# crmorton/Turbo-Whisper-Workspace

Hardware: AMD Instinct MI355X
Metric: real-time factor (audio-sec/wall-sec) Whisper-v3-turbo, 30s chunks, 1/2/4/8 GPU (higher is better)
Workload: dtype bf16; 1 GPU; whisper-large-v3-turbo bf16, batch=24 x 30s windows per GPU, greedy, 128 new tokens/window (EOS suppressed, one seek pass), timestamps on, language detected; collectives=none, global_batch=24, seq_len=3000, parallelism=chunk-dp1

## Files before the change

include/tw_whisper.h:

```cpp
#ifndef TW_WHISPER_H
#define TW_WHISPER_H
#include <stdint.h>

#ifdef __cplusplus
extern "C" {
#endif

#define TW_ABI_VERSION 1

#define TW_EPI_BF16 0
#define TW_EPI_GELU_BF16 1
#define TW_EPI_RESID_F32 2
#define TW_EPI_GELU_POS_F32 3
#define TW_EPI_F32 4
#define TW_EPI_CROSSKV 5
#define TW_EPI_GELU_PACKED 6
#define TW_EPI_GELU_MX 7
#define TW_EPI_GELU_F32 8
#define TW_EPI_PARTIAL_F32 100

#define TW_STATE_STRIDE 8
#define TW_ST_NGEN 0
#define TW_ST_LAST 1
#define TW_ST_PENULT 2
#define TW_ST_LASTTS 3
#define TW_ST_FINISHED 4
#define TW_ST_LANG 5
#define TW_ST_SUMLP 6
#define TW_ST_NOSPEECH 7

#define TW_SELECT_CHUNKS 16
#define TW_SELECT_WS_PER_ROW 128

typedef struct TwSelectParams {
  int32_t V;
  int32_t eos;
  int32_t pad;
  int32_t ts_begin;
  int32_t no_timestamps;
  int32_t max_initial_ts;
  int32_t use_timestamps;
  int32_t max_new;
  int32_t mode;
  int32_t lo, hi;
  int32_t n_begin_suppress;
  int32_t begin_suppress[8];
} TwSelectParams;

int tw_version(void);
const char* tw_last_error(void);

int tw_fill_synth(void* out, long n, uint64_t seed, uint32_t tensor_id, float scale, float offset, int as_f32,
                  void* stream);
int tw_f32_to_bf16(const float* in, uint16_t* out, long n, float scale, void* stream);

int tw_logmel(const float* wave, int n_chunks, const float* basis_cos, const float* basis_sin, const float* mel_fb,
              int n_mels, float* feats, uint32_t* maxkeys, void* stream);

int tw_logmel_long(const float* wave, long n_samples, const float* basis_cos, const float* basis_sin,
                   const float* mel_fb, int n_mels, float* feats, long feats_ld, uint32_t* maxkey, void* stream);

int tw_im2col_conv1(const float* feats, int n_mels, const int* row_map, const int* seek, int R, int kpad,
                    uint16_t* out, void* stream);
int tw_im2col_conv1_long(const float* feats, int n_mels, long ld, const int* max_frames, const int* row_map,
                         const int* seek, int R, int kpad, uint16_t* out, void* stream);
int tw_im2col_conv2(const uint16_t* h1, int R, int D, uint16_t* out, void* stream);
int tw_conv2_gemm(const uint16_t* h1, int R, int D, const uint16_t* W, const float* bias, const float* pos, float* out,
                  void* stream);

int tw_gemm_bf16(const uint16_t* A, const uint16_t* W, int M, int N, int K, int lda, int ldw, int epi, void* out,
                 int ldo, const float* bias, const float* aux, int aux_rows, const int* kv_geom, void* stream);
int tw_gemm_set_variant(int v);
int tw_gemm_bf16_partial(const uint16_t* A, const uint16_t* W, int M, int N, int K, int lda, int ldw, int splits,
                         float* part, int ldp, void* stream);
int tw_resid_layernorm(float* x, const float* parts, int nparts, const float* bias, const float* gamma,
                       const float* beta, int M, int D, float eps, uint16_t* out, void* stream);
int tw_layernorm(const float* x, const float* gamma, const float* beta, int M, int D, float eps, uint16_t* out,
                 void* stream);
int tw_layernorm_set_lds_pad(int kib);

int tw_gemm_mx(const uint8_t* A, const uint8_t* Sa, const uint8_t* W, const uint8_t* Sw, int M, int N, int K, int lda,
               int ldw, int Mp, int Np, int epi, void* out, int ldo, const float* bias, uint8_t* sout, int sout_rows,
               void* stream);
int tw_gemm_mx_set_variant(int v);
int tw_quant_mx(const uint16_t* src, int rows, int K, int ld, uint8_t* dst, uint8_t* scales, int rows_pad,
                void* stream);
int tw_layernorm_mx(const float* x, const float* gamma, const float* beta, int M, int D, float eps, uint8_t* out,
                    uint8_t* scales, int rows_pad, void* stream);

int tw_attn_encoder(const uint16_t* qkv, int B, int S, int H, uint16_t* out, void* stream);
int tw_attn_encoder_mx(const uint16_t* qkv, int B, int S, int H, uint8_t* out, uint8_t* scales, int rows_pad,
                       void* stream);
int tw_attn_set_variant(int variant);
int tw_attn_set_lds_pad(int units);

typedef struct TwBeamParams {
  int32_t num_beams;
  int32_t max_new;
  float length_penalty;
  int32_t ld_tokens;
  int32_t scores_are_logprobs;
} TwBeamParams;
typedef struct TwBeamState {
  float* run_score;
  float* fin_score;
  int32_t* fin_flag;
  int32_t* fin_len;
  int32_t* fin_tokens;
  int32_t* win;
  int32_t* src_rows;
  int32_t* kv_tab;
  int32_t* fin_tab;
  float* run_lp;
  float* fin_lp;
} TwBeamState;
size_t tw_beam_workspace_bytes(int rows);
int tw_beam_step(const float* logits, int W, int ld_logits, const uint32_t* suppress_bits,
                 const TwSelectParams* params, const TwBeamParams* beam, const TwBeamState* bstate, int* state,
                 int* tokens, int* ids, int* pos, void* workspace, void* stream);
int tw_kv_reorder(uint16_t* k_cache, uint16_t* v_cache, uint16_t* k_scratch, uint16_t* v_scratch, int layers,
                  int rows_cap, int H, int T, int R, const int* src_rows, const int* pos, void* stream);

int tw_pack_weight(const uint16_t* W, int N, int K, int ldw, uint16_t* Wp, void* stream);
int tw_gemv_packed(const uint16_t* A, int a_packed, int lda, const uint16_t* Wp, int M, int N, int K, int epi,
                   void* out, int ldo, const float* bias, int splits, void* stream);
int tw_gemv_set_wide_slices(int kw);
int tw_gemv_set_variant(int v);
int tw_gemm_set_epilogue(int tr);
int tw_gemm_set_persistent_grid(int n);
typedef struct TwDecLayerW {
  const uint16_t *wqkv, *wo, *wq_x, *wo_x, *w1, *w2;
  const float *bqkv, *bo, *bq_x, *bo_x, *b1, *b2;
  const float *ln1_g, *ln1_b, *ln2_g, *ln2_b, *ln3_g, *ln3_b;
} TwDecLayerW;
size_t tw_dec_fused_sync_bytes(void);
int tw_dec_fused_supported(int d_model, int heads, int ffn, int rows);
int tw_dec_fused_set_grid(int n);
int tw_dec_fused_set_acquire(int on);
int tw_dec_fused_set_probe(void* buf);
int tw_dec_fused_grid(void);
int tw_dec_fused(const TwDecLayerW* layers, int n_layers, int R, const int* pos, float* x, uint16_t* kc,
                 uint16_t* vc, long kv_layer_stride, int max_pos, const uint16_t* xkv, long xkv_layer_stride,
                 long xkv_v_off, int S, uint16_t* qb, uint16_t* ab, uint16_t* fb, float* slab, float* xpart,
                 const float* lnf_g, const float* lnf_b, uint16_t* hp, float eps, unsigned* sync, unsigned* err,
                 void* stream);
size_t tw_dec_fused_xpart_bytes(int rows);
int tw_resid_layernorm_packed(float* x, const float* parts, int nparts, const float* bias, const float* gamma,
                              const float* beta, int M, int D, float eps, uint16_t* out, void* stream);
int tw_resid_layernorm_packed_to(const float* x, float* x_out, const float* parts, int nparts, const float* bias,
                                 const float* gamma, const float* beta, int M, int D, float eps, uint16_t* out,
                                 void* stream);

int tw_attn_decode_self(const uint16_t* qkv, int B, int H, int max_pos, const int* pos, uint16_t* k_cache,
                        uint16_t* v_cache, uint16_t* out, void* stream);
int tw_attn_decode_self_tab(const uint16_t* qkv, int B, int H, int max_pos, const int* pos, uint16_t* k_cache,
                            uint16_t* v_cache, const int* kv_tab, int row0, uint16_t* out, void* stream);
int tw_attn_decode_self_masked(const uint16_t* qkv, int B, int H, int max_pos, const int* pos, uint16_t* k_cache,
                               uint16_t* v_cache, const int* kv_start, uint16_t* out, void* stream);
int tw_attn_decode_self_tab_masked(const uint16_t* qkv, int B, int H, int max_pos, const int* pos, uint16_t* k_cache,
                                   uint16_t* v_cache, const int* kv_tab, int row0, const int* kv_start, uint16_t* out,
                                   void* stream);
int tw_kv_tab_check(const int* kv_tab, const int* pos, int row0, int B, int max_pos, int* bad, void* stream);
int tw_debug_build(void);
int tw_attn_decode_cross(const uint16_t* q, int B, int H, int S, int Bt, const int* row_map, const uint16_t* cross_kv,
                         uint16_t* out, void* stream);
size_t tw_attn_decode_cross_grouped_ws_bytes(int B, int H);
int tw_attn_decode_cross_grouped(const uint16_t* q, int B, int H, int S, int Bt, const int* row_map, int group,
                                 int first, const uint16_t* cross_kv, float* ws, uint16_t* out, void* stream);
int tw_attn_decode_cross_probs(const uint16_t* q, int B, int H, int S, int Bt, const int* row_map,
                               const uint16_t* cross_kv, uint16_t* out, float* probs, uint32_t head_mask, int slot0,
                               int n_slots, const int* pos, int pos0, int n_steps, void* stream);
int tw_dtw(const double* matrix, int n, int m, int* text_idx, int* time_idx, int* path_len);

int tw_gemm_f32(const float* A, const float* W, int M, int N, int K, int lda, int ldw, int epi, float* out, int ldo,
                const float* bias, const float* aux, int aux_rows, const int* kv_geom, void* stream);
int tw_layernorm_f32(const float* x, const float* gamma, const float* beta, int M, int D, float eps, float* out,
                     void* stream);
int tw_im2col_conv1_f32(const float* feats, int n_mels, long ld, const int* max_frames, const int* row_map,
                        const int* seek, int R, int kpad, float* out, void* stream);
int tw_im2col_conv2_f32(const float* h1, int R, int D, float* out, void* stream);
int tw_embed_decoder_f32(const float* tok_emb, const float* pos_emb, const int* ids, const int* pos, int B, int D,
                         float* x, void* stream);
int tw_attn_encoder_f32(const float* qkv, int B, int S, int H, float* out, void* stream);
int tw_attn_decode_self_f32(const float* qkv, int B, int H, int max_pos, const int* pos, float* k_cache,
                            float* v_cache, const int* kv_tab, int row0, const int* kv_start, float* out,
                            void* stream);
int tw_attn_decode_cross_f32(const float* q, int B, int H, int S, int Bt, const int* row_map, const float* cross_kv,
                             float* out, float* probs, unsigned head_mask, int slot0, int n_slots, const int* pos,
                             int pos0, int n_steps, void* stream);

int tw_embed_decoder(const uint16_t* tok_emb, const uint16_t* pos_emb, const int* ids, const int* pos, int B, int D,
                     float* x, void* stream);
int tw_logits_select(const float* logits, int B, int ld_logits, const uint32_t* suppress_bits,
                     const TwSelectParams* params, int* state, int* tokens_out, int ld_tokens, int* next_ids,
                     int* pos, float* workspace, void* stream);
int tw_logits_select_embed(const float* logits, int B, int ld_logits, const uint32_t* suppress_bits,
                           const TwSelectParams* params, int* state, int* tokens_out, int ld_tokens, int* next_ids,
                           int* pos, float* workspace, const uint16_t* tok_emb, const uint16_t* pos_emb, int D,
                           int max_pos, float* x, const float* gamma, const float* beta, float eps, uint16_t* out,
                           int packed, void* stream);

int tw_logits_sample(const float* logits, int B, int ld_logits, const uint32_t* suppress_bits,
                     const TwSelectParams* params, float temperature, int top_k, uint64_t seed, const int* row_key,
                     int* state, int* tokens_out, int ld_tokens, int* next_ids, int* pos, void* stream);
int tw_token_prob(const float* logits, int B, int ld_logits, int V, int token, int* state, void* stream);

#define TW_HIST_MAX 448
#define TW_HIST_LANG (-1)
int tw_logits_history(float* logits, int R, int ld_logits, int V, const int* prefix, int ld_prefix,
                      const int* prefix_len, const int* tokens, int ld_tokens, const int* state,
                      float repetition_penalty, int no_repeat_ngram, int to_logprobs, void* stream);

#ifdef __cplusplus
}
#endif
#endif
```

turbo-whisper-workspace_amd/csrc/decode.hip:

```cpp
#include "tw_common.h"
#include "../../include/tw_whisper.h"

struct Best {
  float v;
  int i;
};
__device__ inline Best best_of(Best a, Best b) {
  if (b.v > a.v || (b.v == a.v && b.i < a.i)) return b;
  return a;
}
__device__ inline void lse_merge(float& m, float& s, float m2, float s2) {
  if (m2 == -INFINITY) return;
  if (m == -INFINITY) { m = m2; s = s2; return; }
  if (m2 > m) { s = s * __expf(m - m2) + s2; m = m2; }
  else s = s + s2 * __expf(m2 - m);
}

__device__ inline void lse_add1(float& m, float& s, float x) {
  const float d = x - m;
  const float e = (x == -INFINITY) ? 0.f : __expf(-fabsf(d));
  s = (d > 0.f) ? s * e + 1.f : s + e;
  m = fmaxf(m, x);
}

struct SelPart {
  float bt_v; int bt_i;
  float bs_v; int bs_i;
  float m_ts, s_ts;
  float pad0, pad1;
};

struct RowMask {
  int init_step, mask_ts_all, mask_text_lt_eos, ts_hi_block;
};
__device__ inline RowMask row_mask(const int* st, const TwSelectParams& p) {
  const int n_gen = st[TW_ST_NGEN], last = st[TW_ST_LAST], penult = st[TW_ST_PENULT], last_ts = st[TW_ST_LASTTS];
  const int tsb = p.ts_begin;
  RowMask r{n_gen == 0, 0, 0, tsb};
  if (p.mode == 0 && p.use_timestamps) {
    const bool last_was_ts = n_gen >= 1 && last >= tsb;
    const bool penult_was_ts = n_gen < 2 || penult >= tsb;
    if (last_was_ts) {
      if (penult_was_ts) r.mask_ts_all = 1;
      else r.mask_text_lt_eos = 1;
    }
    if (last_ts >= 0) r.ts_hi_block = (last_was_ts && !penult_was_ts) ? last_ts : last_ts + 1;
  }
  return r;
}

template <bool TX>
__device__ inline void sel_chunk(const float* __restrict__ row, const uint32_t* __restrict__ suppress_bits,
                                 const TwSelectParams& p, const RowMask& rm, int v0, int v1, SelPart* sp,
                                 SelPart& out, float& m_tx, float& s_tx) {
  const int tid = threadIdx.x, lane = tid & 63, wid = tid >> 6;
  const int tsb = p.ts_begin;
  Best bt{-INFINITY, 0x7fffffff}, bs{-INFINITY, 0x7fffffff};
  float m_ts = -INFINITY, s_ts = 0.f;
  for (int base = v0 + tid; base < v1; base += 4 * 256) {
    float xs[4];
    uint32_t sb[4];
#pragma unroll
    for (int u = 0; u < 4; ++u) {
      const int v = min(base + 256 * u, v1 - 1);
      xs[u] = row[v];
      sb[u] = suppress_bits ? suppress_bits[v >> 5] : 0u;
    }
#pragma unroll
    for (int u = 0; u < 4; ++u) {
      const int v = base + 256 * u;
      const bool ok = v < v1;
      float x = xs[u];
      bool masked;
      if (p.mode == 1) {
        masked = (v < p.lo || v >= p.hi);
      } else {
        masked = (sb[u] >> (v & 31)) & 1u;
        if (rm.init_step)
          for (int i = 0; i < p.n_begin_suppress; ++i) masked |= (v == p.begin_suppress[i]);
        if (p.use_timestamps) {
          masked |= (v == p.no_timestamps);
          if (v >= tsb) {
            masked |= rm.mask_ts_all || (v < rm.ts_hi_block);
            if (rm.init_step && p.max_initial_ts >= 0) masked |= (v > tsb + p.max_initial_ts);
          } else {
            masked |= (rm.mask_text_lt_eos && v < p.eos) || rm.init_step;
          }
        }
      }
      if (masked) x = -INFINITY;
      if (!ok) continue;
      if (v < tsb || !p.use_timestamps || p.mode == 1) {
        bt = best_of(bt, Best{x, v});
        if (TX && x != -INFINITY) lse_merge(m_tx, s_tx, x, 1.f);
      } else {
        bs = best_of(bs, Best{x, v});
        if (x != -INFINITY) lse_merge(m_ts, s_ts, x, 1.f);
      }
    }
  }
#pragma unroll
  for (int o = 32; o > 0; o >>= 1) {
    Best ot{__shfl_xor(bt.v, o, 64), __shfl_xor(bt.i, o, 64)};
    Best os{__shfl_xor(bs.v, o, 64), __shfl_xor(bs.i, o, 64)};
    bt = best_of(bt, ot);
    bs = best_of(bs, os);
    float m2 = __shfl_xor(m_ts, o, 64), s2 = __shfl_xor(s_ts, o, 64);
    lse_merge(m_ts, s_ts, m2, s2);
  }
  if (lane == 0) sp[wid] = SelPart{bt.v, bt.i, bs.v, bs.i, m_ts, s_ts, 0.f, 0.f};
  __syncthreads();
  if (tid == 0) {
    for (int w = 1; w < 4; ++w) {
      bt = best_of(bt, Best{sp[w].bt_v, sp[w].bt_i});
      bs = best_of(bs, Best{sp[w].bs_v, sp[w].bs_i});
      lse_merge(m_ts, s_ts, sp[w].m_ts, sp[w].s_ts);
    }
    out = SelPart{bt.v, bt.i, bs.v, bs.i, m_ts, s_ts, 0.f, 0.f};
  }
}

__global__ TW_DEC_LB(256, 1) void k_select_partial(const float* __restrict__ logits, int ld_logits,
                                                        const uint32_t* __restrict__ suppress_bits, TwSelectParams p,
                                                        const int* __restrict__ state, SelPart* __restrict__ ws) {
  TW_DEC_PRIO();
  __shared__ SelPart sp[4];
  const int b = blockIdx.x, c = blockIdx.y, NC = gridDim.y;
  const RowMask rm = row_mask(state + b * TW_STATE_STRIDE, p);
  const int V = p.V;
  const int v0 = (int)((long)c * V / NC), v1 = (int)((long)(c + 1) * V / NC);
  SelPart out;
  float m_tx = -INFINITY, s_tx = 0.f;
  sel_chunk<false>(logits + (size_t)b * ld_logits, suppress_bits, p, rm, v0, v1, sp, out, m_tx, s_tx);
  if (threadIdx.x == 0) ws[b * NC + c] = out;
}

__device__ inline void sel_merge(const SelPart* __restrict__ ws, int NC, int b, int lane, Best& bt, Best& bs,
                                 float& m_ts, float& s_ts) {
  bt = Best{-INFINITY, 0x7fffffff};
  bs = Best{-INFINITY, 0x7fffffff};
  m_ts = -INFINITY;
  s_ts = 0.f;
  for (int c = lane; c < NC; c += 64) {
    const SelPart r = ws[b * NC + c];
    bt = best_of(bt, Best{r.bt_v, r.bt_i});
    bs = best_of(bs, Best{r.bs_v, r.bs_i});
    lse_merge(m_ts, s_ts, r.m_ts, r.s_ts);
  }
#pragma unroll
  for (int o = 32; o > 0; o >>= 1) {
    Best ot{__shfl_xor(bt.v, o, 64), __shfl_xor(bt.i, o, 64)};
    Best os{__shfl_xor(bs.v, o, 64), __shfl_xor(bs.i, o, 64)};
    bt = best_of(bt, ot);
    bs = best_of(bs, os);
    float m2 = __shfl_xor(m_ts, o, 64), s2 = __shfl_xor(s_ts, o, 64);
    lse_merge(m_ts, s_ts, m2, s2);
  }
}
__device__ inline bool sel_rule_fires(const TwSelectParams& p, Best bt, float m_ts, float s_ts) {
  if (!p.use_timestamps) return false;
  const float lse_ts = (m_ts == -INFINITY) ? -INFINITY : m_ts + __logf(s_ts);
  return lse_ts > bt.v;
}
__device__ inline int sel_greedy(const TwSelectParams& p, Best bt, Best bs, float m_ts, float s_ts) {
  if (!p.use_timestamps) return bt.i;
  return sel_rule_fires(p, bt, m_ts, s_ts) ? bs.i : best_of(bt, bs).i;
}
__device__ inline int sel_commit(const TwSelectParams& p, int* __restrict__ st, int sel, int* __restrict__ tokens_out,
                                 int ld_tokens, int* __restrict__ next_ids, int b) {
  const int n_gen = st[TW_ST_NGEN], last = st[TW_ST_LAST];
  const int finished = st[TW_ST_FINISHED];
  const int tok = finished ? p.pad : sel;
  if (tokens_out) tokens_out[(size_t)b * ld_tokens + n_gen] = tok;
  if (next_ids) next_ids[b] = tok;
  st[TW_ST_PENULT] = last;
  st[TW_ST_LAST] = tok;
  if (tok >= p.ts_begin && p.use_timestamps) st[TW_ST_LASTTS] = tok;
  st[TW_ST_NGEN] = n_gen + 1;
  if (!finished && (tok == p.eos || n_gen + 1 >= p.max_new)) st[TW_ST_FINISHED] = 1;
  return tok;
}

__device__ inline void select_final_row(const SelPart* __restrict__ ws, int NC, const TwSelectParams& p,
                                        int* __restrict__ state, int* __restrict__ tokens_out, int ld_tokens,
                                        int* __restrict__ next_ids, int* __restrict__ pos, int b, int lane,
                                        int& tok_out, int& npos) {
  Best bt, bs;
  float m_ts, s_ts;
  sel_merge(ws, NC, b, lane, bt, bs, m_ts, s_ts);
  if (lane != 0) return;
  int* st = state + b * TW_STATE_STRIDE;
  npos = 0;
  if (pos) npos = pos[b] += 1;
  if (p.mode == 1) {
    const int sel = bt.i;
    st[TW_ST_LANG] = sel;
    if (next_ids) next_ids[b] = sel;
    tok_out = sel;
    return;
  }
  tok_out = sel_commit(p, st, sel_greedy(p, bt, bs, m_ts, s_ts), tokens_out, ld_tokens, next_ids, b);
}

__global__ __launch_bounds__(64) void k_select_final(const SelPart* __restrict__ ws, int NC, TwSelectParams p,
                                                     int* __restrict__ state, int* __restrict__ tokens_out,
                                                     int ld_tokens, int* __restrict__ next_ids,
                                                     int* __restrict__ pos) {
  TW_DEC_PRIO();
  int tok, npos;
  select_final_row(ws, NC, p, state, tokens_out, ld_tokens, next_ids, pos, blockIdx.x, threadIdx.x, tok, npos);
}

#define SFE_MAXV 4
template <bool PACKED>
__global__ TW_DEC_LB(256, 1) void k_select_final_embed(const SelPart* __restrict__ ws, int NC, TwSelectParams p,
                                                            int* __restrict__ state, int* __restrict__ tokens_out,
                                                            int ld_tokens, int* __restrict__ next_ids,
                                                            int* __restrict__ pos, const bf16_t* __restrict__ tok_emb,
                                                            const bf16_t* __restrict__ pos_emb, int D, int max_pos,
                                                            float* __restrict__ x, const float* __restrict__ g,
                                                            const float* __restrict__ bta, float eps,
                                                            bf16_t* __restrict__ out) {
  TW_DEC_PRIO();
  __shared__ float red[8];
  __shared__ int sh[2];
  const int b = blockIdx.x, tid = threadIdx.x;
  if (tid < 64) {
    int tok = 0, npos = 0;
    select_final_row(ws, NC, p, state, tokens_out, ld_tokens, next_ids, pos, b, tid, tok, npos);
    if (tid == 0) {
      sh[0] = tok;
      sh[1] = min(npos, max_pos - 1);
    }
  }
  __syncthreads();
  const bf16_t* te = tok_emb + (size_t)sh[0] * D;
  const bf16_t* pe = pos_emb + (size_t)sh[1] * D;
  float* xr = x + (size_t)b * D;
  const int nc = D >> 2;
  float4 v[SFE_MAXV];
  float s = 0.f;
#pragma unroll
  for (int i = 0; i < SFE_MAXV; ++i) {
    const int c = min(tid + 256 * i, nc - 1);
    const uint2 t = ((const uint2*)te)[c], q = ((const uint2*)pe)[c];
    float4 a;
    a.x = bf16_to_f32((bf16_t)(t.x & 0xffff)) + bf16_to_f32((bf16_t)(q.x & 0xffff));
    a.y = bf16_to_f32((bf16_t)(t.x >> 16)) + bf16_to_f32((bf16_t)(q.x >> 16));
    a.z = bf16_to_f32((bf16_t)(t.y & 0xffff)) + bf16_to_f32((bf16_t)(q.y & 0xffff));
    a.w = bf16_to_f32((bf16_t)(t.y >> 16)) + bf16_to_f32((bf16_t)(q.y >> 16));
    v[i] = a;
    if (tid + 256 * i < nc) {
      ((float4*)xr)[tid + 256 * i] = a;
      s += (a.x + a.y) + (a.z + a.w);
    }
  }
  tw_row_ln_store<PACKED>(v, s, b, D, eps, g, bta, out, red);
}

extern "C" int tw_logits_select(const float* logits, int B, int ld_logits, const uint32_t* suppress_bits,
                                const TwSelectParams* params, int* state, int* tokens_out, int ld_tokens,
                                int* next_ids, int* pos, float* workspace, void* stream) {
  TW_REQUIRE(logits && params && state && workspace && B > 0, "tw_logits_select: bad args");
  TW_REQUIRE(params->V > 0 && params->V <= ld_logits, "tw_logits_select: V=%d ld=%d", params->V, ld_logits);
  TW_REQUIRE(params->n_begin_suppress >= 0 && params->n_begin_suppress <= 8, "tw_logits_select: begin_suppress");
  static_assert(sizeof(SelPart) * TW_SELECT_CHUNKS == sizeof(float) * TW_SELECT_WS_PER_ROW, "workspace size");
  hipStream_t s = (hipStream_t)stream;
  SelPart* ws = (SelPart*)workspace;
  hipLaunchKernelGGL(k_select_partial, dim3(B, TW_SELECT_CHUNKS), dim3(256), 0, s, logits, ld_logits, suppress_bits,
                     *params, state, ws);
  hipLaunchKernelGGL(k_select_final, dim3(B), dim3(64), 0, s, ws, TW_SELECT_CHUNKS, *params, state, tokens_out,
                     ld_tokens, next_ids, pos);
  return tw_check_launch("tw_logits_select");
}

extern "C" int tw_logits_select_embed(const float* logits, int B, int ld_logits, const uint32_t* suppress_bits,
                                      const TwSelectParams* params, int* state, int* tokens_out, int ld_tokens,
                                      int* next_ids, int* pos, float* workspace, const uint16_t* tok_emb,
                                      const uint16_t* pos_emb, int D, int max_pos, float* x, const float* gamma,
                                      const float* beta, float eps, uint16_t* out, int packed, void* stream) {
  TW_REQUIRE(logits && params && state && workspace && next_ids && pos && B > 0, "tw_logits_select_embed: bad args");
  TW_REQUIRE(params->mode == 0, "tw_logits_select_embed: greedy token selection (mode 0) only");
  TW_REQUIRE(params->V > 0 && params->V <= ld_logits, "tw_logits_select_embed: V=%d ld=%d", params->V, ld_logits);
  TW_REQUIRE(params->n_begin_suppress >= 0 && params->n_begin_suppress <= 8, "tw_logits_select_embed: begin_suppress");
  TW_REQUIRE(tok_emb && pos_emb && x && gamma && beta && out && max_pos > 0, "tw_logits_select_embed: embed/LN args");
  TW_REQUIRE(D > 0 && D % 4 == 0 && D <= 1024 * SFE_MAXV && (!packed || (B <= 64 && D % 32 == 0)),
             "tw_logits_select_embed: D=%d B=%d packed=%d", D, B, packed);
  hipStream_t s = (hipStream_t)stream;
  SelPart* ws = (SelPart*)workspace;
  hipLaunchKernelGGL(k_select_partial, dim3(B, TW_SELECT_CHUNKS), dim3(256), 0, s, logits, ld_logits, suppress_bits,
                     *params, state, ws);
  if (packed)
    hipLaunchKernelGGL(k_select_final_embed<true>, dim3(B), dim3(256), 0, s, ws, TW_SELECT_CHUNKS, *params, state,
                       tokens_out, ld_tokens, next_ids, pos, tok_emb, pos_emb, D, max_pos, x, gamma, beta, eps, out);
  else
    hipLaunchKernelGGL(k_select_final_embed<false>, dim3(B), dim3(256), 0, s, ws, TW_SELECT_CHUNKS, *params, state,
                       tokens_out, ld_tokens, next_ids, pos, tok_emb, pos_emb, D, max_pos, x, gamma, beta, eps, out);
  return tw_check_launch("tw_logits_select_embed");
}

__device__ inline uint64_t tw_mix64(uint64_t z) {
  z += 0x9e3779b97f4a7c15ull;
  z = (z ^ (z >> 30)) * 0xbf58476d1ce4e5b9ull;
  z = (z ^ (z >> 27)) * 0x94d049bb133111ebull;
  return z ^ (z >> 31);
}
__device__ inline float tw_gumbel(uint64_t seed, uint32_t key, uint32_t step, uint32_t v) {
  const uint64_t h = tw_mix64(seed ^ tw_mix64(((uint64_t)key << 32) ^ ((uint64_t)step << 20) ^ (uint64_t)v));
  const float u = ((float)(h >> 40) + 0.5f) * (1.0f / 16777216.0f);
  return -logf(-logf(u));
}
__device__ inline float sel_processed(const float* __restrict__ row, const uint32_t* __restrict__ suppress_bits,
                                      const TwSelectParams& p, const RowMask& rm, int v) {
  const int tsb = p.ts_begin;
  bool masked = suppress_bits ? (suppress_bits[v >> 5] >> (v & 31)) & 1u : false;
  if (rm.init_step)
    for (int i = 0; i < p.n_begin_suppress; ++i) masked |= (v == p.begin_suppress[i]);
  if (p.use_timestamps) {
    masked |= (v == p.no_timestamps);
    if (v >= tsb) {
      masked |= rm.mask_ts_all || (v < rm.ts_hi_block);
      if (rm.init_step && p.max_initial_ts >= 0) masked |= (v > tsb + p.max_initial_ts);
    } else {
      masked |= (rm.mask_text_lt_eos && v < p.eos) || rm.init_step;
    }
  }
  return masked ? -INFINITY : row[v];
}
__device__ inline float block_sum256(float v, float* red) {
  v = wave_sum(v);
  __syncthreads();
  if ((threadIdx.x & 63) == 0) red[threadIdx.x >> 6] = v;
  __syncthreads();
  return (red[0] + red[1]) + (red[2] + red[3]);
}
__device__ inline void block_lse256(float& m, float& s, float* red) {
#pragma unroll
  for (int o = 32; o > 0; o >>= 1) lse_merge(m, s, __shfl_xor(m, o, 64), __shfl_xor(s, o, 64));
  __syncthreads();
  if ((threadIdx.x & 63) == 0) {
    red[2 * (threadIdx.x >> 6)] = m;
    red[2 * (threadIdx.x >> 6) + 1] = s;
  }
  __syncthreads();
  m = red[0];
  s = red[1];
  for (int w = 1; w < 4; ++w) lse_merge(m, s, red[2 * w], red[2 * w + 1]);
}

__global__ __launch_bounds__(256) void k_select_full(const float* __restrict__ logits, int ld_logits,
                                                     const uint32_t* __restrict__ suppress_bits, TwSelectParams p,
                                                     float temperature, int top_k, uint64_t seed,
                                                     const int* __restrict__ row_key, int* __restrict__ state,
                                                     int* __restrict__ tokens_out, int ld_tokens,
                                                     int* __restrict__ next_ids, int* __restrict__ pos) {
  __shared__ SelPart sp[4];
  __shared__ SelPart parts[TW_SELECT_CHUNKS];
  __shared__ float red[8];
  __shared__ uint32_t hist[256];
  __shared__ int bcast[4];
  const int b = blockIdx.x, tid = threadIdx.x, lane = tid & 63;
  int* st = state + b * TW_STATE_STRIDE;
  const RowMask rm = row_mask(st, p);
  const float* row = logits + (size_t)b * ld_logits;
  const int V = p.V, NC = TW_SELECT_CHUNKS, tsb = p.ts_begin;
  float m_tx = -INFINITY, s_tx = 0.f;
  for (int c = 0; c < NC; ++c) {
    SelPart out;
    sel_chunk<true>(row, suppress_bits, p, rm, (int)((long)c * V / NC), (int)((long)(c + 1) * V / NC), sp, out, m_tx,
                    s_tx);
    if (tid == 0) parts[c] = out;
    __syncthreads();
  }
  block_lse256(m_tx, s_tx, red);
  Best bt, bs;
  float m_ts, s_ts;
  sel_merge(parts, NC, 0, lane, bt, bs, m_ts, s_ts);
  const bool fire = sel_rule_fires(p, bt, m_ts, s_ts);
  int sel;
  float lse;
  if (temperature <= 0.f) {
    sel = sel_greedy(p, bt, bs, m_ts, s_ts);
    float m = fire ? -INFINITY : m_tx, sm = fire ? 0.f : s_tx;
    if (p.use_timestamps) lse_merge(m, sm, m_ts, s_ts);
    lse = m + __logf(sm);
  } else {
    const float invT = 1.f / temperature;
    auto elig = [&](int v, float x) { return x != -INFINITY && !(fire && v < tsb); };
    uint32_t prefix = 0u, mask = 0u;
    int n_el = 0;
    for (int v = tid; v < V; v += 256) n_el += elig(v, sel_processed(row, suppress_bits, p, rm, v)) ? 1 : 0;
    n_el = (int)block_sum256((float)n_el, red);
    const bool restrict_k = top_k > 0 && n_el > top_k;
    if (restrict_k) {
      int k_rem = top_k;
      for (int shift = 24; shift >= 0; shift -= 8) {
        hist[tid] = 0u;
        __syncthreads();
        for (int v = tid; v < V; v += 256) {
          const float x = sel_processed(row, suppress_bits, p, rm, v);
          if (!elig(v, x)) continue;
          const uint32_t key = f32_order_key(x);
          if ((key & mask) == prefix) atomicAdd(&hist[(key >> shift) & 255u], 1u);
        }
        __syncthreads();
        if (tid == 0) {
          int cum = 0, d = 255;
          for (; d > 0; --d) {
            if (cum + (int)hist[d] >= k_rem) break;
            cum += (int)hist[d];
          }
          bcast[0] = d;
          bcast[1] = k_rem - cum;
        }
        __syncthreads();
        prefix |= (uint32_t)bcast[0] << shift;
        mask |= 255u << shift;
        k_rem = bcast[1];
        __syncthreads();
      }
    }
    const uint32_t rkey = row_key ? (uint32_t)row_key[b] : (uint32_t)b;
    const uint32_t step = (uint32_t)st[TW_ST_NGEN];
    Best g{-INFINITY, 0x7fffffff};
    float m = -INFINITY, sm = 0.f;
    for (int v = tid; v < V; v += 256) {
      const float x = sel_processed(row, suppress_bits, p, rm, v);
      if (!elig(v, x) || (restrict_k && f32_order_key(x) < prefix)) continue;
      lse_merge(m, sm, x, 1.f);
      g = best_of(g, Best{x * invT + tw_gumbel(seed, rkey, step, (uint32_t)v), v});
    }
#pragma unroll
    for (int o = 32; o > 0; o >>= 1) g = best_of(g, Best{__shfl_xor(g.v, o, 64), __shfl_xor(g.i, o, 64)});
    __syncthreads();
    if (lane == 0) {
      red[tid >> 6] = g.v;
      bcast[tid >> 6] = g.i;
    }
    __syncthreads();
    g = Best{red[0], bcast[0]};
    for (int w = 1; w < 4; ++w) g = best_of(g, Best{red[w], bcast[w]});
    sel = g.i;
    block_lse256(m, sm, red);
    lse = m + __logf(sm);
  }
  if (tid != 0) return;
  if (pos) pos[b] += 1;
  const int was_finished = st[TW_ST_FINISHED];
  const int tok = sel_commit(p, st, sel, tokens_out, ld_tokens, next_ids, b);
  if (!was_finished) {
    const float lp = row[tok] - lse;
    st[TW_ST_SUMLP] = __float_as_int(__int_as_float(st[TW_ST_SUMLP]) + lp);
  }
}

__global__ __launch_bounds__(256) void k_token_prob(const float* __restrict__ logits, int ld_logits, int V, int token,
                                                    int* __restrict__ state) {
  __shared__ float red[8];
  const float* row = logits + (size_t)blockIdx.x * ld_logits;
  float m = -INFINITY, s = 0.f;
  for (int v = threadIdx.x; v < V; v += 256) lse_merge(m, s, row[v], 1.f);
  block_lse256(m, s, red);
  if (threadIdx.x == 0)
    state[blockIdx.x * TW_STATE_STRIDE + TW_ST_NOSPEECH] = __float_as_int(__expf(row[token] - (m + __logf(s))));
}

extern "C" int tw_logits_sample(const float* logits, int B, int ld_logits, const uint32_t* suppress_bits,
                                const TwSelectParams* params, float temperature, int top_k, uint64_t seed,
                                const int* row_key, int* state, int* tokens_out, int ld_tokens, int* next_ids,
                                int* pos, void* stream) {
  TW_REQUIRE(logits && params && state && B > 0, "tw_logits_sample: bad args");
  TW_REQUIRE(params->mode == 0, "tw_logits_sample: generation steps (mode 0) only");
  TW_REQUIRE(params->V > 0 && params->V <= ld_logits, "tw_logits_sample: V=%d ld=%d", params->V, ld_logits);
  TW_REQUIRE(params->n_begin_suppress >= 0 && params->n_begin_suppress <= 8, "tw_logits_sample: begin_suppress");
  TW_REQUIRE(temperature >= 0.f && temperature == temperature, "tw_logits_sample: temperature %f", temperature);
  hipLaunchKernelGGL(k_select_full, dim3(B), dim3(256), 0, (hipStream_t)stream, logits, ld_logits, suppress_bits,
                     *params, temperature, top_k, seed, row_key, state, tokens_out, ld_tokens, next_ids, pos);
  return tw_check_launch("tw_logits_sample");
}

extern "C" int tw_token_prob(const float* logits, int B, int ld_logits, int V, int token, int* state, void* stream) {
  TW_REQUIRE(logits && state && B > 0 && V > 0 && V <= ld_logits && token >= 0 && token < V,
             "tw_token_prob: B=%d V=%d token=%d", B, V, token);
  hipLaunchKernelGGL(k_token_prob, dim3(B), dim3(256), 0, (hipStream_t)stream, logits, ld_logits, V, token, state);
  return tw_check_launch("tw_token_prob");
}

#define TW_HIST_THREADS 1024
#define TW_HIST_INFLIGHT 8
__global__ __launch_bounds__(TW_HIST_THREADS) void k_logits_history(float* __restrict__ logits, int ld_logits, int V,
                                                                    const int* __restrict__ prefix, int ld_prefix,
                                                                    const int* __restrict__ prefix_len,
                                                                    const int* __restrict__ tokens, int ld_tokens,
                                                                    const int* __restrict__ state, float penalty,
                                                                    int ngram, int to_logprobs) {
  TW_DEC_PRIO();
  __shared__ int h[TW_HIST_MAX];
  __shared__ float red[2 * (TW_HIST_THREADS / 64)];
  const int r = blockIdx.x, tid = threadIdx.x;
  const int* st = state + r * TW_STATE_STRIDE;
  if (st[TW_ST_FINISHED]) return;
  float* row = logits + (size_t)r * ld_logits;
  const int pl = prefix ? min(max(prefix_len[r], 0), ld_prefix) : 0;
  const int ng = min(max(st[TW_ST_NGEN], 0), ld_tokens);
  const int L = min(pl + ng, TW_HIST_MAX);
  for (int i = tid; i < L; i += TW_HIST_THREADS) {
    int id = i < pl ? prefix[(size_t)r * ld_prefix + i] : tokens[(size_t)r * ld_tokens + (i - pl)];
    if (id == TW_HIST_LANG) id = st[TW_ST_LANG];
    h[i] = id;
  }
  if (to_logprobs) {
    float m = -INFINITY, s = 0.f;
    for (int base = tid; base < V; base += TW_HIST_INFLIGHT * TW_HIST_THREADS) {
      float xs[TW_HIST_INFLIGHT];
#pragma unroll
      for (int u = 0; u < TW_HIST_INFLIGHT; ++u) {
        const int v = base + u * TW_HIST_THREADS;
        xs[u] = v < V ? row[v] : -INFINITY;
      }
#pragma unroll
      for (int u = 0; u < TW_HIST_INFLIGHT; ++u) {
        const float x = xs[u], d = x - m;
        const float e = (x == -INFINITY) ? 0.f : expf(-fabsf(d));
        s = (d > 0.f) ? s * e + 1.f : s + e;
        m = fmaxf(m, x);
      }
    }
    auto merge = [](float& m, float& s, float m2, float s2) {
      if (m2 == -INFINITY) return;
      if (m == -INFINITY) { m = m2; s = s2; return; }
// ... 657 lines not shown
```

turbo-whisper-workspace_amd/csrc/gemm.hip:

```cpp
#include <algorithm>
#include <type_traits>

#include "tw_common.h"
#include "../../include/tw_whisper.h"

struct EpiArgs {
  void* out;
  int ldo;
  const float* bias;
  const float* aux;
  int aux_rows;
  int kv_S, kv_B, kv_D, kv_H;
  uint8_t* sout;
  int s_rows;
  int group_m;
};

__device__ inline void tw_tile_grouped(int wgid, int ntm, int ntn, int gm, int& tm, int& tn) {
  if (gm <= 1) {
    tm = wgid / ntn;
    tn = wgid - tm * ntn;
    return;
  }
  const int per = gm * ntn, g = wgid / per, first = g * gm;
  const int rows = min(ntm - first, gm), l = wgid - g * per;
  tm = first + l % rows;
  tn = l / rows;
}

template <int EPI>
__device__ inline void epi_store(const EpiArgs& ea, int m, int n, float v) {
  if (ea.bias) v += ea.bias[n];
  if constexpr (EPI == TW_EPI_BF16) {
    ((bf16_t*)ea.out)[(size_t)m * ea.ldo + n] = f32_to_bf16(v);
  } else if constexpr (EPI == TW_EPI_GELU_BF16) {
    ((bf16_t*)ea.out)[(size_t)m * ea.ldo + n] = f32_to_bf16(gelu_erf(v));
  } else if constexpr (EPI == TW_EPI_RESID_F32) {
    float* o = (float*)ea.out + (size_t)m * ea.ldo + n;
    *o = *o + v;
  } else if constexpr (EPI == TW_EPI_GELU_POS_F32) {
    ((float*)ea.out)[(size_t)m * ea.ldo + n] = gelu_erf(v) + ea.aux[(size_t)(m % ea.aux_rows) * ea.ldo + n];
  } else if constexpr (EPI == TW_EPI_F32) {
    ((float*)ea.out)[(size_t)m * ea.ldo + n] = v;
  } else if constexpr (EPI == TW_EPI_CROSSKV) {
    const int D = ea.kv_D, S = ea.kv_S;
    int l = n / (2 * D), rem = n - l * 2 * D;
    int kv = rem / D, hd = rem - kv * D;
    int h = hd >> 6, d = hd & 63;
    int b = m / S, s = m - b * S;
    size_t idx = ((((size_t)(l * 2 + kv) * ea.kv_B + b) * ea.kv_H + h) * S + s) * 64 + d;
    ((bf16_t*)ea.out)[idx] = f32_to_bf16(v);
  }
}

static int tw_gemm_kernel = 1;
static int tw_gemm_tr = 0;
extern "C" int tw_gemm_set_epilogue(int tr) {
  TW_REQUIRE(tr == 0 || tr == 1, "tw_gemm_set_epilogue: %d (0 or 1)", tr);
  tw_gemm_tr = tr;
  return 0;
}
static inline int tw_group_for(int N) { return (N + 255) / 256 >= 10 ? 8 : 1; }
static constexpr int tw_gemv_nt_min_n = 16384;
static int tw_gemv_wide_kw = 1;
extern "C" int tw_gemv_set_wide_slices(int kw) {
  TW_REQUIRE(kw == 1 || kw == 2 || kw == 4, "tw_gemv_set_wide_slices: kw=%d (1, 2 or 4)", kw);
  tw_gemv_wide_kw = kw;
  return 0;
}
static constexpr int tw_gemv_max_kw = 4;
static int tw_gemv_kernel = 0;
extern "C" int tw_gemv_set_variant(int v) {
  TW_REQUIRE(v == 0 || v == 1, "tw_gemv_set_variant: v=%d (0 or 1)", v);
  tw_gemv_kernel = v;
  return 0;
}
extern "C" int tw_gemm_set_variant(int v) {
  tw_gemm_kernel = (v & 15) == 5 ? 5 : (v & 15) == 6 ? 6 : 1;
  return 0;
}
static int tw_pgrid_override = 0;
extern "C" int tw_gemm_set_persistent_grid(int n) {
  TW_REQUIRE(n == 0 || (n >= 8 && n % 8 == 0), "tw_gemm_set_persistent_grid: %d (0 = all CUs, else a multiple of 8)", n);
  tw_pgrid_override = n;
  return 0;
}
static int tw_persistent_grid() {
  static int g = 0;
  if (tw_pgrid_override) return tw_pgrid_override;
  if (!g) {
    int dev = 0, cus = 0;
    if (hipGetDevice(&dev) != hipSuccess ||
        hipDeviceGetAttribute(&cus, hipDeviceAttributeMultiprocessorCount, dev) != hipSuccess || cus < 8)
      cus = 256;
    g = cus / 8 * 8;
  }
  return g;
}

#define GB_BM 256
#define GB_BN 256
#define GB_BK 64
#define GB_EPI_LD 68

typedef __attribute__((address_space(3))) void lds_void_t;

__device__ inline int gb_swz(int r) { return (r >> 1) & 7; }

constexpr int gb_nt_bit(int epi) {
  return epi == TW_EPI_BF16 ? TW_NT_GEMM_BF16 : epi == TW_EPI_GELU_BF16 ? TW_NT_GEMM_GELU
         : epi == TW_EPI_RESID_F32 ? TW_NT_GEMM_RESID : TW_NT_GEMM_OTHER;
}

template <int EPI>
__device__ inline void epi_store4(const EpiArgs& ea, int m, int n, int N, float4 v) {
  if (n + 3 >= N) {
    const float t[4] = {v.x, v.y, v.z, v.w};
    EpiArgs e2 = ea;
    e2.bias = nullptr;
    for (int q = 0; q < 4; ++q)
      if (n + q < N) epi_store<EPI>(e2, m, n + q, t[q]);
    return;
  }
  if constexpr (EPI == TW_EPI_BF16 || EPI == TW_EPI_GELU_BF16) {
    if constexpr (EPI == TW_EPI_GELU_BF16) v = gelu_erf4(v);
    uint2 w;
    w.x = pack_bf16x2(v.x, v.y);
    w.y = pack_bf16x2(v.z, v.w);
    tw_st_enc<gb_nt_bit(EPI)>((bf16_t*)ea.out + (size_t)m * ea.ldo + n, w);
  } else if constexpr (EPI == TW_EPI_RESID_F32) {
    float4* o = (float4*)((float*)ea.out + (size_t)m * ea.ldo + n);
    float4 x = *o;
    x.x += v.x; x.y += v.y; x.z += v.z; x.w += v.w;
    tw_st_enc<gb_nt_bit(EPI)>(o, x);
  } else if constexpr (EPI == TW_EPI_GELU_POS_F32) {
    const float4 a = *(const float4*)(ea.aux + (size_t)(m % ea.aux_rows) * ea.ldo + n);
    float4 o = gelu_erf4(v);
    o.x += a.x; o.y += a.y; o.z += a.z; o.w += a.w;
    tw_st_enc<gb_nt_bit(EPI)>((float*)ea.out + (size_t)m * ea.ldo + n, o);
  } else if constexpr (EPI == TW_EPI_F32) {
    tw_st_enc<gb_nt_bit(EPI)>((float*)ea.out + (size_t)m * ea.ldo + n, v);
  } else if constexpr (EPI == TW_EPI_CROSSKV) {
    const int D = ea.kv_D, S = ea.kv_S;
    int l = n / (2 * D), rem = n - l * 2 * D;
    int kv = rem / D, hd = rem - kv * D;
    int h = hd >> 6, d = hd & 63;
    int b = m / S, s = m - b * S;
    size_t idx = ((((size_t)(l * 2 + kv) * ea.kv_B + b) * ea.kv_H + h) * S + s) * 64 + d;
    uint2 w;
    w.x = pack_bf16x2(v.x, v.y);
    w.y = pack_bf16x2(v.z, v.w);
    tw_st_enc<gb_nt_bit(EPI)>((bf16_t*)ea.out + idx, w);
  }
}

template <int EPI>
__device__ inline float4 epi_addend(const EpiArgs& ea, int m, int n, bool full) {
// ... 857 lines not shown
    for (int a = 0; a < 2; ++a)
#pragma unroll
      for (int b = 0; b < 2; ++b)
#pragma unroll
        for (int i = 0; i < 4; ++i)
#pragma unroll
          for (int j = 0; j < 2; ++j) acc[a][b][i][j] = (f32x4){0.f, 0.f, 0.f, 0.f};
    if (nk == 1) {
      ktile(0, BF{}, BT{});
    } else {
      ktile(0, BT{}, BT{});
      for (int t = 1; t + 1 < nk; ++t) ktile(t, BT{}, BF{});
      ktile(nk - 1, BF{}, BF{});
    }
    if (wr == 0) __builtin_amdgcn_s_barrier();
    __syncthreads();
    const int nlocal = local + S;
    const bool has_next = nlocal < cnt;
    const int cm0 = m0, cn0 = n0;
    if (has_next) {
      set_tile(base + nlocal, m0, n0);
#pragma unroll
      for (int h = 0; h < 4; ++h) stage(0, h, 0);
      stage_bias((it + 1) & 1, n0);
    }
    epilogue(cm0, cn0, bias_sl + 256 * (it & 1));
    if (!has_next) break;
    if (BF16OUT && cm0 + GB_BM <= M && cn0 + GB_BN <= N)
      asm volatile("s_waitcnt vmcnt(16)" ::: "memory");
    else if (PRE && cm0 + GB_BM <= M && cn0 + GB_BN <= N)
      asm volatile("s_waitcnt vmcnt(8)" ::: "memory");
    else
      asm volatile("s_waitcnt vmcnt(0)" ::: "memory");
    __builtin_amdgcn_s_barrier();
    if (wr == 1) __builtin_amdgcn_s_barrier();
    local = nlocal;
  }
}

#define TW_EPI_PARTIAL 100

template <int EPI, int NW, bool TWO>
__global__ __launch_bounds__(NW * 64) void k_gemm_skinny(const bf16_t* __restrict__ A, const bf16_t* __restrict__ W,
                                                         int M, int N, int K, int lda, int ldw, EpiArgs ea) {
  TW_DEC_PRIO();
  __shared__ float red[NW][32][17];
  const int tid = threadIdx.x, lane = tid & 63, wid = tid >> 6;
  const int n0 = blockIdx.x * 16;
  const int nsl = NW * gridDim.y, gw = blockIdx.y * NW + wid;
  const int ns = K >> 5;
  const int s0 = (int)((long)gw * ns / nsl), s1 = (int)((long)(gw + 1) * ns / nsl);
  const int col = min(n0 + (lane & 15), N - 1);
  const int ksub = 8 * (lane >> 4);
  const int ar0 = min(lane & 15, M - 1), ar1 = min(16 + (lane & 15), M - 1);
  const bf16_t* wp = W + (size_t)col * ldw + ksub;
  const bf16_t* ap0 = A + (size_t)ar0 * lda + ksub;
  const bf16_t* ap1 = A + (size_t)ar1 * lda + ksub;
  f32x4 c0 = {0}, c1 = {0};
  int s = s0;
  for (; s + 8 <= s1; s += 8) {
    bf16x8 bw[8], a0[8], a1[8];
#pragma unroll
    for (int u = 0; u < 8; ++u) {
      bw[u] = *(const bf16x8*)(wp + 32 * (s + u));
      a0[u] = *(const bf16x8*)(ap0 + 32 * (s + u));
      if (TWO) a1[u] = *(const bf16x8*)(ap1 + 32 * (s + u));
    }
#pragma unroll
    for (int u = 0; u < 8; ++u) {
      c0 = __builtin_amdgcn_mfma_f32_16x16x32_bf16(a0[u], bw[u], c0, 0, 0, 0);
      if (TWO) c1 = __builtin_amdgcn_mfma_f32_16x16x32_bf16(a1[u], bw[u], c1, 0, 0, 0);
    }
  }
  for (; s < s1; ++s) {
    bf16x8 bw = *(const bf16x8*)(wp + 32 * s);
    bf16x8 a0 = *(const bf16x8*)(ap0 + 32 * s);
    c0 = __builtin_amdgcn_mfma_f32_16x16x32_bf16(a0, bw, c0, 0, 0, 0);
    if (TWO) {
      bf16x8 a1 = *(const bf16x8*)(ap1 + 32 * s);
      c1 = __builtin_amdgcn_mfma_f32_16x16x32_bf16(a1, bw, c1, 0, 0, 0);
    }
  }
  const int cc = lane & 15, rb = (lane >> 4) * 4;
#pragma unroll
  for (int r = 0; r < 4; ++r) {
    red[wid][rb + r][cc] = c0[r];
    if (TWO) red[wid][16 + rb + r][cc] = c1[r];
  }
  __syncthreads();
  const int rows = TWO ? 32 : 16;
  for (int e = tid; e < rows * 16; e += NW * 64) {
    int m = e >> 4, c = e & 15;
    int n = n0 + c;
    if (m < M && n < N) {
      float v = 0.f;
#pragma unroll
      for (int w = 0; w < NW; ++w) v += red[w][m][c];
      if constexpr (EPI == TW_EPI_PARTIAL) {
        ((float*)ea.out)[((size_t)blockIdx.y * M + m) * ea.ldo + n] = v;
      } else {
        epi_store<EPI>(ea, m, n, v);
      }
    }
  }
}

template <int EPI, int NW>
static void launch_skinny_nw(const bf16_t* A, const bf16_t* W, int M, int N, int K, int lda, int ldw,
                             const EpiArgs& ea, int splits, hipStream_t s) {
  dim3 grid(tw_cdiv(N, 16), splits);
  if (M > 16)
    hipLaunchKernelGGL((k_gemm_skinny<EPI, NW, true>), grid, dim3(NW * 64), 0, s, A, W, M, N, K, lda, ldw, ea);
  else
    hipLaunchKernelGGL((k_gemm_skinny<EPI, NW, false>), grid, dim3(NW * 64), 0, s, A, W, M, N, K, lda, ldw, ea);
}

template <int EPI>
static void launch_skinny(const bf16_t* A, const bf16_t* W, int M, int N, int K, int lda, int ldw,
                          const EpiArgs& ea, int splits, hipStream_t s) {
  const long nb = tw_cdiv(N, 16) * (long)splits;
  const int ns = K / 32;
  int nw = 4;
  while (nb * nw < 1024 && nw < 8 && ns >= 2 * 2 * nw * splits) nw *= 2;
  if (nw == 4) launch_skinny_nw<EPI, 4>(A, W, M, N, K, lda, ldw, ea, splits, s);
  else if (nw == 8) launch_skinny_nw<EPI, 8>(A, W, M, N, K, lda, ldw, ea, splits, s);
  else launch_skinny_nw<EPI, 16>(A, W, M, N, K, lda, ldw, ea, splits, s);
}

__global__ __launch_bounds__(256) void k_pack_weight(const bf16_t* __restrict__ W, int N, int K, int ldw,
                                                     bf16_t* __restrict__ Wp, long nchunks) {
  const long c = (long)blockIdx.x * 256 + threadIdx.x;
  if (c >= nchunks) return;
  const int lane = (int)(c & 63);
  const long rest = c >> 6;
  const int ns = K >> 5;
  const int st = (int)(rest % ns), g = (int)(rest / ns);
  const int n = g * 16 + (lane & 15), k = st * 32 + 8 * (lane >> 4);
  uint4 v = make_uint4(0u, 0u, 0u, 0u);
  if (n < N) v = *(const uint4*)(W + (size_t)n * ldw + k);
  *(uint4*)(Wp + c * 8) = v;
}


template <int MT, bool APACK>
__device__ inline const bf16_t* gemv_a_base(const bf16_t* A, int lda, int M, int K, int t, int lane) {
  if constexpr (APACK) return A + (size_t)(t >> 1) * 32 * K + (t & 1) * 512 + lane * 8;
  else return A + (size_t)min(16 * t + (lane & 15), M - 1) * lda + 8 * (lane >> 4);
}
template <bool APACK>
__device__ inline bf16x8 gemv_a_load(const bf16_t* ap, int st) {
  return APACK ? *(const bf16x8*)(ap + (size_t)st * 1024) : *(const bf16x8*)(ap + 32 * st);
}

template <int EPI, int KW, int U, bool APACK, int MT, bool NTW = false>
__global__ TW_DEC_LB(KW > 4 ? 512 : 256, NTW ? 4 : 1) void k_gemv_p(const bf16_t* __restrict__ A, int lda,
                                                               const bf16_t* __restrict__ Wp, int M, int N, int K,
                                                               EpiArgs ea) {
  TW_DEC_PRIO();
  constexpr int NW = KW > 4 ? KW : 4, GPB = NW / KW;
  __shared__ float red[KW > 1 ? NW : 1][KW > 1 ? MT * 16 : 1][17];
  const int tid = threadIdx.x, lane = tid & 63, wid = tid >> 6;
  const int gl = wid / KW, kw = wid - gl * KW;
  const int g = blockIdx.x * GPB + gl;
  const int ngroups = (N + 15) >> 4, ns = K >> 5;
  const int nsl = KW * gridDim.y, sl = blockIdx.y * KW + kw;
  const int s0 = (int)((long)sl * ns / nsl), s1 = (int)((long)(sl + 1) * ns / nsl);
  f32x4 c[MT];
#pragma unroll
  for (int t = 0; t < MT; ++t) c[t] = (f32x4){0.f, 0.f, 0.f, 0.f};
  if (g < ngroups) {
    const bf16_t* wp = Wp + (size_t)g * ns * 512 + lane * 8;
    const bf16_t* ap[MT];
#pragma unroll
    for (int t = 0; t < MT; ++t) ap[t] = gemv_a_base<MT, APACK>(A, lda, M, K, t, lane);
    auto ldW = [&](int st) -> bf16x8 {
      if constexpr (NTW) {
        typedef short s16x8_nt __attribute__((ext_vector_type(8)));
        const s16x8_nt v = __builtin_nontemporal_load((const s16x8_nt*)(wp + (size_t)st * 512));
        return __builtin_bit_cast(bf16x8, v);
      } else {
        return *(const bf16x8*)(wp + (size_t)st * 512);
      }
    };
    auto batch = [&](auto NBc, int st0, int n) {
      constexpr int NB = decltype(NBc)::value;
      bf16x8 bw[NB], a[NB][MT];
#pragma unroll
      for (int u = 0; u < NB; ++u) {
        const int st = min(st0 + u, s1 - 1);
        bw[u] = ldW(st);
#pragma unroll
        for (int t = 0; t < MT; ++t) a[u][t] = gemv_a_load<APACK>(ap[t], st);
      }
      if constexpr (!NTW) __builtin_amdgcn_sched_barrier(0);
#pragma unroll
      for (int u = 0; u < NB; ++u) {
        if (u < n) {
#pragma unroll
          for (int t = 0; t < MT; ++t) c[t] = __builtin_amdgcn_mfma_f32_16x16x32_bf16(a[u][t], bw[u], c[t], 0, 0, 0);
        }
      }
    };
    using IU = std::integral_constant<int, U>;
    int st = s0;
    for (; st + U <= s1; st += U) batch(IU{}, st, U);
    const int rem = s1 - st;
    if (rem > U / 2) batch(IU{}, st, rem);
    else if (rem > U / 4) batch(std::integral_constant<int, (U / 2 > 0 ? U / 2 : 1)>{}, st, rem);
    else if (rem > 0) batch(std::integral_constant<int, (U / 4 > 0 ? U / 4 : 1)>{}, st, rem);
  }
  const int cc = lane & 15, rb = (lane >> 4) * 4;
  auto store = [&](int m, int n, float v) {
    if constexpr (EPI == TW_EPI_PARTIAL) {
      ((float*)ea.out)[((size_t)blockIdx.y * M + m) * ea.ldo + n] = v;
    } else if constexpr (EPI == TW_EPI_GELU_PACKED) {
      if (ea.bias) v += ea.bias[n];
      ((bf16_t*)ea.out)[tw_pack_act_idx(m, n, N)] = f32_to_bf16(gelu_erf(v));
    } else {
      epi_store<EPI>(ea, m, n, v);
    }
  };
  if constexpr (KW == 1) {
    const int n = g * 16 + cc;
    if (g < ngroups && n < N) {
#pragma unroll
      for (int t = 0; t < MT; ++t)
#pragma unroll
        for (int r = 0; r < 4; ++r)
          if (16 * t + rb + r < M) store(16 * t + rb + r, n, c[t][r]);
    }
    return;
  }
#pragma unroll
  for (int t = 0; t < MT; ++t)
#pragma unroll
    for (int r = 0; r < 4; ++r) red[wid][16 * t + rb + r][cc] = c[t][r];
  __syncthreads();
  constexpr int ROWS = MT * 16;
  for (int e = tid; e < GPB * ROWS * 16; e += NW * 64) {
    const int gg = e / (ROWS * 16), rem = e - gg * ROWS * 16;
    const int m = rem >> 4, cl = rem & 15;
    const int n = (blockIdx.x * GPB + gg) * 16 + cl;
    if (m < M && n < N) {
      float v = 0.f;
#pragma unroll
      for (int w = 0; w < KW; ++w) v += red[gg * KW + w][m][cl];
      store(m, n, v);
    }
  }
}

template <int EPI, int KW, int U, bool APACK, int MT, bool NTW = false>
__global__ TW_DEC_LB(256, 1) void k_gemv_pc(const bf16_t* __restrict__ A, int lda, const bf16_t* __restrict__ Wp,
                                            int M, int N, int K, EpiArgs ea) {
  TW_DEC_PRIO();
  static_assert(KW == 1 || KW == 2 || KW == 4, "k_gemv_pc: 1, 2 or 4 K-slices");
  constexpr int NW = 4, GPB = NW / KW;
  constexpr int RT = MT > 2 ? 2 : MT;
  __shared__ float red[KW > 1 ? NW : 1][2][KW > 1 ? RT * 16 : 1][17];
  const int tid = threadIdx.x, lane = tid & 63, wid = tid >> 6;
  const int gl = wid / KW, kw = wid - gl * KW;
  const int g0 = (blockIdx.x * GPB + gl) * 2;
  const int ngroups = (N + 15) >> 4, ns = K >> 5;
  const int nsl = KW * gridDim.y, sl = blockIdx.y * KW + kw;
  const int s0 = (int)((long)sl * ns / nsl), s1 = (int)((long)(sl + 1) * ns / nsl);
  f32x4 c[2][MT];
#pragma unroll
  for (int t = 0; t < MT; ++t) c[0][t] = c[1][t] = (f32x4){0.f, 0.f, 0.f, 0.f};
  if (g0 < ngroups) {
    const bool has1 = g0 + 1 < ngroups;
    const bf16_t* wp0 = Wp + (size_t)g0 * ns * 512 + lane * 8;
    const bf16_t* wp1 = has1 ? wp0 + (size_t)ns * 512 : wp0;
    const bf16_t* ap[MT];
#pragma unroll
    for (int t = 0; t < MT; ++t) ap[t] = gemv_a_base<MT, APACK>(A, lda, M, K, t, lane);
    constexpr int TH = MT > 2 ? 2 : MT;
    auto batch = [&](auto NBc, int st0, int n) {
      constexpr int NB = decltype(NBc)::value;
      bf16x8 b0[NB], b1[NB], a[NB][TH];
#pragma unroll
      for (int u = 0; u < NB; ++u) {
        const int st = min(st0 + u, s1 - 1);
        if constexpr (NTW) {
          typedef short s16x8_nt __attribute__((ext_vector_type(8)));
          b0[u] = __builtin_bit_cast(bf16x8, __builtin_nontemporal_load((const s16x8_nt*)(wp0 + (size_t)st * 512)));
          b1[u] = __builtin_bit_cast(bf16x8, __builtin_nontemporal_load((const s16x8_nt*)(wp1 + (size_t)st * 512)));
        } else {
          b0[u] = *(const bf16x8*)(wp0 + (size_t)st * 512);
          b1[u] = *(const bf16x8*)(wp1 + (size_t)st * 512);
        }
#pragma unroll
        for (int t = 0; t < TH; ++t) a[u][t] = gemv_a_load<APACK>(ap[t], st);
      }
#pragma unroll
      for (int h = 0; h < MT / TH; ++h) {
        if (h) {
#pragma unroll
          for (int u = 0; u < NB; ++u) {
            const int st = min(st0 + u, s1 - 1);
#pragma unroll
            for (int t = 0; t < TH; ++t) a[u][t] = gemv_a_load<APACK>(ap[h * TH + t], st);
          }
        }
        __builtin_amdgcn_sched_barrier(0);
#pragma unroll
        for (int u = 0; u < NB; ++u) {
          if (u < n) {
#pragma unroll
            for (int t = 0; t < TH; ++t) {
              c[0][h * TH + t] = __builtin_amdgcn_mfma_f32_16x16x32_bf16(a[u][t], b0[u], c[0][h * TH + t], 0, 0, 0);
              c[1][h * TH + t] = __builtin_amdgcn_mfma_f32_16x16x32_bf16(a[u][t], b1[u], c[1][h * TH + t], 0, 0, 0);
            }
          }
        }
        if constexpr (MT > TH) __builtin_amdgcn_sched_barrier(0);
      }
    };
    using IU = std::integral_constant<int, U>;
    int st = s0;
    for (; st + U <= s1; st += U) batch(IU{}, st, U);
    const int rem = s1 - st;
    if (rem > U / 2) batch(IU{}, st, rem);
    else if (rem > 0) batch(std::integral_constant<int, (U / 2 > 0 ? U / 2 : 1)>{}, st, rem);
  }
  const int cc = lane & 15, rb = (lane >> 4) * 4;
  auto store = [&](int m, int n, float v) {
    if constexpr (EPI == TW_EPI_PARTIAL) {
      ((float*)ea.out)[((size_t)blockIdx.y * M + m) * ea.ldo + n] = v;
    } else if constexpr (EPI == TW_EPI_GELU_PACKED) {
      if (ea.bias) v += ea.bias[n];
      ((bf16_t*)ea.out)[tw_pack_act_idx(m, n, N)] = f32_to_bf16(gelu_erf(v));
    } else {
      epi_store<EPI>(ea, m, n, v);
    }
  };
  if constexpr (KW == 1) {
    const int n0 = g0 * 16 + cc, n1 = n0 + 16;
#pragma unroll
    for (int t = 0; t < MT; ++t)
#pragma unroll
      for (int r = 0; r < 4; ++r) {
        const int m = 16 * t + rb + r;
        if (m < M && n0 < N) store(m, n0, c[0][t][r]);
        if (m < M && n1 < N) store(m, n1, c[1][t][r]);
      }
    return;
  }
  constexpr int ROWS = RT * 16;
#pragma unroll
  for (int pass = 0; pass < MT / RT; ++pass) {
    if (pass) __syncthreads();
#pragma unroll
    for (int t = 0; t < RT; ++t)
#pragma unroll
      for (int r = 0; r < 4; ++r) {
        red[wid][0][16 * t + rb + r][cc] = c[0][pass * RT + t][r];
        red[wid][1][16 * t + rb + r][cc] = c[1][pass * RT + t][r];
      }
    __syncthreads();
    for (int e = tid; e < GPB * 2 * ROWS * 16; e += NW * 64) {
      const int pg = e / (2 * ROWS * 16), rem = e - pg * 2 * ROWS * 16;
      const int h = rem / (ROWS * 16), r2 = rem - h * ROWS * 16;
      const int m = pass * ROWS + (r2 >> 4), cl = r2 & 15;
      const int n = ((blockIdx.x * GPB + pg) * 2 + h) * 16 + cl;
      if (m < M && n < N) {
        float v = 0.f;
#pragma unroll
        for (int w = 0; w < KW; ++w) v += red[pg * KW + w][h][r2 >> 4][cl];
        store(m, n, v);
      }
    }
  }
}

template <int EPI, int KW, bool APACK, int U = 5, bool NTW = false>
static void launch_gemv_pc(const bf16_t* A, int lda, const bf16_t* Wp, int M, int N, int K, const EpiArgs& ea,
                           int splits, hipStream_t s) {
  constexpr int GPB = 4 / KW;
  dim3 grid(tw_cdiv(tw_cdiv(tw_cdiv(N, 16), 2), GPB), splits);
  if (M > 32)
    hipLaunchKernelGGL((k_gemv_pc<EPI, KW, U, APACK, 4, NTW>), grid, dim3(256), 0, s, A, lda, Wp, M, N, K, ea);
  else if (M > 16)
    hipLaunchKernelGGL((k_gemv_pc<EPI, KW, U, APACK, 2, NTW>), grid, dim3(256), 0, s, A, lda, Wp, M, N, K, ea);
  else
    hipLaunchKernelGGL((k_gemv_pc<EPI, KW, U, APACK, 1, NTW>), grid, dim3(256), 0, s, A, lda, Wp, M, N, K, ea);
}

template <int EPI, int KW, int U, bool APACK, int MT>
__global__ TW_DEC_LB(256, 1) void k_gemv_q(const bf16_t* __restrict__ A, int lda, const bf16_t* __restrict__ Wp,
                                           int M, int N, int K, EpiArgs ea) {
  TW_DEC_PRIO();
  static_assert(KW == 1 || KW == 2 || KW == 4, "k_gemv_q: 1, 2 or 4 K-slices");
  constexpr int NW = 4, GPB = NW / KW;
  __shared__ float red[KW > 1 ? NW : 1][KW > 1 ? MT * 16 : 1][17];
  const int tid = threadIdx.x, lane = tid & 63, wid = tid >> 6;
  const int gl = wid / KW, kw = wid - gl * KW;
  const int g = blockIdx.x * GPB + gl;
  const int ngroups = (N + 15) >> 4, ns = K >> 5;
  const int nsl = KW * gridDim.y, sl = blockIdx.y * KW + kw;
  const int s0 = (int)((long)sl * ns / nsl), s1 = (int)((long)(sl + 1) * ns / nsl);
  const int n = s1 - s0;
  f32x4 c[MT];
#pragma unroll
  for (int t = 0; t < MT; ++t) c[t] = (f32x4){0.f, 0.f, 0.f, 0.f};
  if (g < ngroups) {
    const bf16_t* wp = Wp + ((size_t)g * ns + s0) * 512 + lane * 8;
    const bf16_t* ap[MT];
#pragma unroll
    for (int t = 0; t < MT; ++t) ap[t] = gemv_a_base<MT, APACK>(A, lda, M, K, t, lane);
    bf16x8 w[U];
#pragma unroll
    for (int u = 0; u < U; ++u)
      if (u < n) w[u] = *(const bf16x8*)(wp + (size_t)u * 512);
    bf16x8 a[2][MT];
#pragma unroll
    for (int t = 0; t < MT; ++t) a[0][t] = gemv_a_load<APACK>(ap[t], s0);
    __builtin_amdgcn_sched_barrier(0);
#pragma unroll
    for (int u = 0; u < U; ++u) {
      if (u < n) {
        if (u + 1 < n) {
#pragma unroll
          for (int t = 0; t < MT; ++t) a[(u + 1) & 1][t] = gemv_a_load<APACK>(ap[t], s0 + u + 1);
        }
        __builtin_amdgcn_sched_barrier(0);
#pragma unroll
        for (int t = 0; t < MT; ++t) c[t] = __builtin_amdgcn_mfma_f32_16x16x32_bf16(a[u & 1][t], w[u], c[t], 0, 0, 0);
        __builtin_amdgcn_sched_barrier(0);
      }
    }
  }
  const int cc = lane & 15, rb = (lane >> 4) * 4;
  auto store = [&](int m, int col, float v) {
    if constexpr (EPI == TW_EPI_PARTIAL) {
      ((float*)ea.out)[((size_t)blockIdx.y * M + m) * ea.ldo + col] = v;
    } else if constexpr (EPI == TW_EPI_GELU_PACKED) {
      if (ea.bias) v += ea.bias[col];
      ((bf16_t*)ea.out)[tw_pack_act_idx(m, col, N)] = f32_to_bf16(gelu_erf(v));
    } else {
      epi_store<EPI>(ea, m, col, v);
    }
  };
  if constexpr (KW == 1) {
    const int col = g * 16 + cc;
    if (g < ngroups && col < N) {
#pragma unroll
      for (int t = 0; t < MT; ++t)
#pragma unroll
        for (int r = 0; r < 4; ++r)
          if (16 * t + rb + r < M) store(16 * t + rb + r, col, c[t][r]);
    }
    return;
  }
#pragma unroll
  for (int t = 0; t < MT; ++t)
#pragma unroll
    for (int r = 0; r < 4; ++r) red[wid][16 * t + rb + r][cc] = c[t][r];
  __syncthreads();
  constexpr int ROWS = MT * 16;
  for (int e = tid; e < GPB * ROWS * 16; e += NW * 64) {
    const int gg = e / (ROWS * 16), rem = e - gg * ROWS * 16;
    const int m = rem >> 4, cl = rem & 15;
    const int col = (blockIdx.x * GPB + gg) * 16 + cl;
    if (m < M && col < N) {
      float v = 0.f;
#pragma unroll
      for (int w2 = 0; w2 < KW; ++w2) v += red[gg * KW + w2][m][cl];
      store(m, col, v);
    }
  }
}

template <int EPI, bool APACK, int KW, int MT>
static void launch_gemv_q_mt(const bf16_t* A, int lda, const bf16_t* Wp, int M, int N, int K, const EpiArgs& ea,
                             int splits, hipStream_t s) {
  dim3 grid(tw_cdiv(tw_cdiv(N, 16), 4 / KW), splits);
  hipLaunchKernelGGL((k_gemv_q<EPI, KW, 10, APACK, MT>), grid, dim3(256), 0, s, A, lda, Wp, M, N, K, ea);
}
template <int EPI, bool APACK, int KW>
static void launch_gemv_q_kw(const bf16_t* A, int lda, const bf16_t* Wp, int M, int N, int K, const EpiArgs& ea,
                             int splits, hipStream_t s) {
  if (M > 32) launch_gemv_q_mt<EPI, APACK, KW, 4>(A, lda, Wp, M, N, K, ea, splits, s);
  else if (M > 16) launch_gemv_q_mt<EPI, APACK, KW, 2>(A, lda, Wp, M, N, K, ea, splits, s);
  else launch_gemv_q_mt<EPI, APACK, KW, 1>(A, lda, Wp, M, N, K, ea, splits, s);
}
template <int EPI, bool APACK>
static bool launch_gemv_q(const bf16_t* A, int lda, const bf16_t* Wp, int M, int N, int K, const EpiArgs& ea,
                          int splits, hipStream_t s) {
  const int ns = K / 32;
  const int ngroups = tw_cdiv(N, 16);
  auto longest = [&](int kw) { return tw_cdiv(ns, kw * splits); };
  int kw = 1;
  while (kw < 4 && longest(kw) > 10) kw *= 2;
  if (longest(kw) > 10) return false;
  while (kw < 4 && (long)tw_cdiv(ngroups, 4 / kw) * splits < 256 && longest(2 * kw) >= 5) kw *= 2;
  if (kw == 1) launch_gemv_q_kw<EPI, APACK, 1>(A, lda, Wp, M, N, K, ea, splits, s);
  else if (kw == 2) launch_gemv_q_kw<EPI, APACK, 2>(A, lda, Wp, M, N, K, ea, splits, s);
  else launch_gemv_q_kw<EPI, APACK, 4>(A, lda, Wp, M, N, K, ea, splits, s);
  return true;
}

template <int EPI, int KW, int U, bool APACK, bool NTW = false>
static void launch_gemv_p3(const bf16_t* A, int lda, const bf16_t* Wp, int M, int N, int K, const EpiArgs& ea, int splits,
                           hipStream_t s) {
  constexpr int NW = KW > 4 ? KW : 4, GPB = NW / KW;
  constexpr int U4 = U > 4 ? U / 2 : U;
  dim3 grid(tw_cdiv(tw_cdiv(N, 16), GPB), splits);
  if (M > 32)
    hipLaunchKernelGGL((k_gemv_p<EPI, KW, U4, APACK, 4, NTW>), grid, dim3(NW * 64), 0, s, A, lda, Wp, M, N, K, ea);
  else if (M > 16)
    hipLaunchKernelGGL((k_gemv_p<EPI, KW, U, APACK, 2, NTW>), grid, dim3(NW * 64), 0, s, A, lda, Wp, M, N, K, ea);
  else
    hipLaunchKernelGGL((k_gemv_p<EPI, KW, U, APACK, 1, NTW>), grid, dim3(NW * 64), 0, s, A, lda, Wp, M, N, K, ea);
}

template <int EPI, bool APACK>
static void launch_gemv_p2(const bf16_t* A, int lda, const bf16_t* Wp, int M, int N, int K, const EpiArgs& ea, int splits,
                           hipStream_t s) {
  const long groups = tw_cdiv(N, 16) * (long)splits;
  const int steps = K / 32 / splits;
  int kw = 1;
  while (groups * kw < 1024 && kw < tw_gemv_max_kw && steps >= 8 * kw) kw *= 2;
  const bool wide = N >= tw_gemv_nt_min_n;
  if (wide) {
    if constexpr (EPI == TW_EPI_F32) {
      if (M > 32 && tw_gemv_wide_kw == 1) {
        launch_gemv_pc<EPI, 1, APACK, 5, true>(A, lda, Wp, M, N, K, ea, splits, s);
        return;
      }
    }
    if (tw_gemv_wide_kw == 4 && steps >= 8 * 4) launch_gemv_p3<EPI, 4, 8, APACK, true>(A, lda, Wp, M, N, K, ea, splits, s);
    else if (tw_gemv_wide_kw >= 2 && steps >= 8 * 2) launch_gemv_p3<EPI, 2, 8, APACK, true>(A, lda, Wp, M, N, K, ea, splits, s);
    else launch_gemv_p3<EPI, 1, 16, APACK, true>(A, lda, Wp, M, N, K, ea, splits, s);
    return;
  }
  if constexpr (EPI == TW_EPI_BF16 || EPI == TW_EPI_PARTIAL || EPI == TW_EPI_GELU_PACKED) {
    if (tw_gemv_kernel == 1 && M > 16 && M <= 32 && launch_gemv_q<EPI, APACK>(A, lda, Wp, M, N, K, ea, splits, s)) return;
    const long pairs = tw_cdiv(tw_cdiv(N, 16), 2) * (long)splits;
    if (pairs * 2 < 1024 && steps >= 8 * 4) launch_gemv_pc<EPI, 4, APACK>(A, lda, Wp, M, N, K, ea, splits, s);
    else launch_gemv_pc<EPI, 2, APACK>(A, lda, Wp, M, N, K, ea, splits, s);
    return;
  }
  if (kw == 1) launch_gemv_p3<EPI, 1, 16, APACK>(A, lda, Wp, M, N, K, ea, splits, s);
  else if (kw == 2) launch_gemv_p3<EPI, 2, 8, APACK>(A, lda, Wp, M, N, K, ea, splits, s);
  else launch_gemv_p3<EPI, 4, 8, APACK>(A, lda, Wp, M, N, K, ea, splits, s);
}

template <int EPI>
static void launch_gemv_p(const bf16_t* A, int a_packed, int lda, const bf16_t* Wp, int M, int N, int K,
                          const EpiArgs& ea, int splits, hipStream_t s) {
  if (a_packed) launch_gemv_p2<EPI, true>(A, lda, Wp, M, N, K, ea, splits, s);
  else launch_gemv_p2<EPI, false>(A, lda, Wp, M, N, K, ea, splits, s);
}

template <int EPI>
static int launch_gemm(const bf16_t* A, const bf16_t* W, int M, int N, int K, int lda, int ldw, const EpiArgs& ea,
                       hipStream_t s) {
  if (M <= 32) {
    launch_skinny<EPI>(A, W, M, N, K, lda, ldw, ea, 1, s);
  } else {
    const unsigned nwg = tw_cdiv(M, GB_BM) * tw_cdiv(N, GB_BN);
    if (tw_gemm_kernel == 6 && N % 4 == 0 && N >= 4 && ((uintptr_t)ea.bias & 15) == 0)
      hipLaunchKernelGGL(k_gemm_8pp<EPI>, dim3(std::min<unsigned>(tw_persistent_grid(), (nwg + 7) / 8 * 8)), dim3(512),
                         0, s, A, W, M, N, K, lda, ldw, ea);
    else if (tw_gemm_kernel >= 5 && tw_gemm_tr)
      hipLaunchKernelGGL((k_gemm_8p<EPI, true>), dim3(nwg), dim3(512), 0, s, A, W, M, N, K, lda, ldw, ea);
    else if (tw_gemm_kernel >= 5)
      hipLaunchKernelGGL((k_gemm_8p<EPI, false>), dim3(nwg), dim3(512), 0, s, A, W, M, N, K, lda, ldw, ea);
    else if (tw_gemm_tr)
      hipLaunchKernelGGL((k_gemm_big<EPI, true>), dim3(nwg), dim3(512), 0, s, A, W, M, N, K, lda, ldw, ea);
    else
      hipLaunchKernelGGL((k_gemm_big<EPI, false>), dim3(nwg), dim3(512), 0, s, A, W, M, N, K, lda, ldw, ea);
  }
  return tw_check_launch("tw_gemm_bf16");
}

extern "C" int tw_gemm_bf16(const bf16_t* A, const bf16_t* W, int M, int N, int K, int lda, int ldw, int epi,
                            void* out, int ldo, const float* bias, const float* aux, int aux_rows,
                            const int* kv_geom, void* stream) {
  TW_REQUIRE(A && W && out, "tw_gemm_bf16: null pointer");
  TW_REQUIRE(M > 0 && N > 0 && K > 0 && K % GB_BK == 0, "tw_gemm_bf16: M=%d N=%d K=%d (K %% 64 required)", M, N, K);
  TW_REQUIRE(lda % 8 == 0 && ldw % 8 == 0 && lda >= K && ldw >= K, "tw_gemm_bf16: lda=%d ldw=%d", lda, ldw);
  EpiArgs ea{out, ldo, bias, aux, aux_rows, 0, 0, 0, 0};
  ea.group_m = tw_group_for(N);
  hipStream_t s = (hipStream_t)stream;
  switch (epi) {
    case TW_EPI_BF16: return launch_gemm<TW_EPI_BF16>(A, W, M, N, K, lda, ldw, ea, s);
    case TW_EPI_GELU_BF16: return launch_gemm<TW_EPI_GELU_BF16>(A, W, M, N, K, lda, ldw, ea, s);
    case TW_EPI_RESID_F32: return launch_gemm<TW_EPI_RESID_F32>(A, W, M, N, K, lda, ldw, ea, s);
    case TW_EPI_GELU_POS_F32:
      TW_REQUIRE(aux && aux_rows > 0, "tw_gemm_bf16: GELU_POS needs aux table");
      return launch_gemm<TW_EPI_GELU_POS_F32>(A, W, M, N, K, lda, ldw, ea, s);
    case TW_EPI_F32: return launch_gemm<TW_EPI_F32>(A, W, M, N, K, lda, ldw, ea, s);
    case TW_EPI_CROSSKV:
      TW_REQUIRE(kv_geom != nullptr, "tw_gemm_bf16: CROSSKV needs kv_geom {S,B,D,H}");
      ea.kv_S = kv_geom[0]; ea.kv_B = kv_geom[1]; ea.kv_D = kv_geom[2]; ea.kv_H = kv_geom[3];
      TW_REQUIRE(ea.kv_S * ea.kv_B == M && N % (2 * ea.kv_D) == 0 && ea.kv_H * 64 == ea.kv_D,
                 "tw_gemm_bf16: CROSSKV geometry mismatch");
      return launch_gemm<TW_EPI_CROSSKV>(A, W, M, N, K, lda, ldw, ea, s);
    default: tw_set_error("tw_gemm_bf16: unknown epilogue %d", epi); return TW_ERR_ARG;
  }
}

extern "C" int tw_conv2_gemm(const bf16_t* h1, int R, int D, const bf16_t* W, const float* bias, const float* pos,
                             float* out, void* stream) {
  TW_REQUIRE(h1 && W && bias && pos && out, "tw_conv2_gemm: null pointer");
  TW_REQUIRE(R > 0 && D > 0 && D % 32 == 0, "tw_conv2_gemm: R=%d D=%d (D %% 32 required)", R, D);
  hipStream_t s = (hipStream_t)stream;
  EpiArgs ea{out, D, bias, pos, 1500, 0, 0, 0, 0};
  ea.group_m = tw_group_for(D);
  int rc = launch_gemm<TW_EPI_GELU_POS_F32>(h1 - D, W, R * 1500, D, 3 * D, 2 * D, 3 * D, ea, s);
  if (rc) return rc;
  for (int r0 = 0; r0 < R && !rc; r0 += 32) {
    EpiArgs e0{out + (size_t)r0 * 1500 * D, 1500 * D, bias, pos, 1, 0, 0, 0, 0};
    e0.group_m = 1;
    rc = launch_gemm<TW_EPI_GELU_POS_F32>(h1 + (size_t)r0 * 3000 * D, W + D, std::min(32, R - r0), D, 2 * D,
                                          3000 * D, 3 * D, e0, s);
  }
  return rc;
}

extern "C" int tw_gemm_bf16_partial(const bf16_t* A, const bf16_t* W, int M, int N, int K, int lda, int ldw,
                                    int splits, float* part, int ldp, void* stream) {
  TW_REQUIRE(A && W && part, "tw_gemm_bf16_partial: null pointer");
  TW_REQUIRE(M > 0 && M <= 32 && N > 0 && K > 0 && K % 32 == 0, "tw_gemm_bf16_partial: M=%d N=%d K=%d (M <= 32, K %% 32)",
             M, N, K);
  TW_REQUIRE(splits >= 1 && splits <= 16 && splits <= K / 32, "tw_gemm_bf16_partial: splits=%d", splits);
  TW_REQUIRE(lda % 8 == 0 && ldw % 8 == 0 && lda >= K && ldw >= K && ldp >= N, "tw_gemm_bf16_partial: lda=%d ldw=%d ldp=%d",
             lda, ldw, ldp);
  EpiArgs ea{part, ldp, nullptr, nullptr, 0, 0, 0, 0, 0};
  launch_skinny<TW_EPI_PARTIAL>(A, W, M, N, K, lda, ldw, ea, splits, (hipStream_t)stream);
  return tw_check_launch("tw_gemm_bf16_partial");
}

extern "C" int tw_pack_weight(const bf16_t* W, int N, int K, int ldw, bf16_t* Wp, void* stream) {
  TW_REQUIRE(W && Wp && N > 0 && K > 0 && K % 32 == 0 && ldw >= K && ldw % 8 == 0,
             "tw_pack_weight: N=%d K=%d ldw=%d (K %% 32, ldw %% 8)", N, K, ldw);
  const long nchunks = (long)tw_cdiv(N, 16) * (K / 32) * 64;
  hipLaunchKernelGGL(k_pack_weight, dim3(tw_cdiv(nchunks, 256)), dim3(256), 0, (hipStream_t)stream, W, N, K, ldw, Wp,
                     nchunks);
  return tw_check_launch("tw_pack_weight");
}

extern "C" int tw_gemv_packed(const bf16_t* A, int a_packed, int lda, const bf16_t* Wp, int M, int N, int K, int epi,
                              void* out, int ldo, const float* bias, int splits, void* stream) {
  TW_REQUIRE(A && Wp && out, "tw_gemv_packed: null pointer");
  TW_REQUIRE(M > 0 && M <= 64 && N > 0 && K > 0 && K % 32 == 0, "tw_gemv_packed: M=%d N=%d K=%d (M <= 64, K %% 32)", M,
             N, K);
  TW_REQUIRE(a_packed || (lda >= K && lda % 8 == 0), "tw_gemv_packed: lda=%d", lda);
  TW_REQUIRE(splits >= 1 && splits <= 16 && splits <= K / 32, "tw_gemv_packed: splits=%d", splits);
  TW_REQUIRE(splits == 1 || epi == TW_EPI_PARTIAL_F32, "tw_gemv_packed: split-K needs the PARTIAL epilogue");
  EpiArgs ea{out, ldo, bias, nullptr, 0, 0, 0, 0, 0};
  hipStream_t s = (hipStream_t)stream;
  switch (epi) {
    case TW_EPI_BF16: launch_gemv_p<TW_EPI_BF16>(A, a_packed, lda, Wp, M, N, K, ea, splits, s); break;
    case TW_EPI_F32: launch_gemv_p<TW_EPI_F32>(A, a_packed, lda, Wp, M, N, K, ea, splits, s); break;
    case TW_EPI_GELU_PACKED:
      TW_REQUIRE(N % 32 == 0, "tw_gemv_packed: GELU_PACKED needs N %% 32 (it is the next GEMV's K)");
      launch_gemv_p<TW_EPI_GELU_PACKED>(A, a_packed, lda, Wp, M, N, K, ea, splits, s);
      break;
    case TW_EPI_PARTIAL_F32:
      TW_REQUIRE(ldo >= N, "tw_gemv_packed: ldo=%d < N", ldo);
      ea.bias = nullptr;
      launch_gemv_p<TW_EPI_PARTIAL>(A, a_packed, lda, Wp, M, N, K, ea, splits, s);
      break;
    case TW_EPI_RESID_F32:
      TW_REQUIRE(ldo >= N, "tw_gemv_packed: ldo=%d < N", ldo);
      launch_gemv_p<TW_EPI_RESID_F32>(A, a_packed, lda, Wp, M, N, K, ea, splits, s);
      break;
    default: tw_set_error("tw_gemv_packed: unsupported epilogue %d", epi); return TW_ERR_ARG;
  }
  return tw_check_launch("tw_gemv_packed");
}

typedef __attribute__((ext_vector_type(8))) int i32x8;
#define MX_BK 128
#define MX_TILE (GB_BM * MX_BK)
#define MX_STAGE (2 * MX_TILE + 2 * GB_BM * 4)

template <int EPI>
__global__ __launch_bounds__(512, 1) void k_gemm_mx(const uint8_t* __restrict__ A, const uint8_t* __restrict__ W,
                                                    const uint8_t* __restrict__ Sa, const uint8_t* __restrict__ Sw,
                                                    int M, int N, int K, int lda, int ldw, int Mp, int Np,
                                                    EpiArgs ea) {
  __shared__ __attribute__((aligned(16))) uint8_t smem[8 * 64 * GB_EPI_LD * 4];
  const int tid = threadIdx.x, lane = tid & 63, wid = tid >> 6;
  const int ntm = (M + GB_BM - 1) / GB_BM, ntn = (N + GB_BN - 1) / GB_BN;
  const int nwg = ntm * ntn;
  const int orig = blockIdx.x;
  const int q8 = nwg / 8, r8 = nwg % 8, xcd = orig % 8;
  const int wgid = (xcd < r8 ? xcd * (q8 + 1) : r8 * (q8 + 1) + (xcd - r8) * q8) + orig / 8;
  int tm, tn;
  tw_tile_grouped(wgid, ntm, ntn, ea.group_m, tm, tn);
  const int m0 = tm * GB_BM, n0 = tn * GB_BN;

  const int rows_a = max(0, min(GB_BM, M - m0)), rows_w = max(0, min(GB_BN, N - n0));
  const __amdgpu_buffer_rsrc_t ra = tw_uniform_rsrc(A + (size_t)m0 * lda, rows_a ? (rows_a - 1) * lda + K : 0);
  const __amdgpu_buffer_rsrc_t rw = tw_uniform_rsrc(W + (size_t)n0 * ldw, rows_w ? (rows_w - 1) * ldw + K : 0);
  unsigned va[4], vw[4];
#pragma unroll
  for (int i = 0; i < 4; ++i) {
    const int row = 8 * (4 * wid + i) + (lane >> 3);
    const int ch = (lane & 7) ^ gb_swz(row);
    va[i] = (unsigned)(row * lda + ch * 16);
    vw[i] = (unsigned)(row * ldw + ch * 16);
  }
  const int wu = __builtin_amdgcn_readfirstlane(wid);
  const unsigned gs_step = (unsigned)(wu == 0 ? Mp : Np) * 4u;
  const __amdgpu_buffer_rsrc_t rsc =
      tw_uniform_rsrc(wu == 0 ? Sa + (size_t)m0 * 4 : Sw + (size_t)n0 * 4, (int)((K / MX_BK - 1) * gs_step + 1024u));
  auto stage = [&](int buf, int kt) {
    uint8_t* As = smem + buf * MX_STAGE;
    uint8_t* Ws = As + MX_TILE;
    const unsigned k0 = (unsigned)(kt * MX_BK);
#pragma unroll
    for (int i = 0; i < 4; ++i) {
      const int rb = 8 * (4 * wid + i) * MX_BK;
      __builtin_amdgcn_raw_ptr_buffer_load_lds(ra, (lds_void_t*)(As + rb), 16, va[i], k0, 0, 0);
      __builtin_amdgcn_raw_ptr_buffer_load_lds(rw, (lds_void_t*)(Ws + rb), 16, vw[i], k0, 0, 0);
    }
    if (wu < 2)
      __builtin_amdgcn_raw_ptr_buffer_load_lds(rsc, (lds_void_t*)(As + 2 * MX_TILE + wu * 1024), 16,
                                               (unsigned)lane * 16u, (unsigned)kt * gs_step, 0, 0);
  };

  const int wr = wid >> 2, wc = wid & 3;
  const int fr = lane & 15, fq = lane >> 4;
  const int lane_lo = fr * MX_BK + ((fq ^ ((fr >> 1) & 7)) << 4), lane_hi = fr * MX_BK + (((fq + 4) ^ ((fr >> 1) & 7)) << 4);
  f32x4 acc[8][4];
#pragma unroll
  for (int i = 0; i < 8; ++i)
#pragma unroll
    for (int j = 0; j < 4; ++j) acc[i][j] = (f32x4){0.f, 0.f, 0.f, 0.f};

  const int nk = K / MX_BK;
  stage(0, 0);
  __syncthreads();
  for (int kt = 0; kt < nk; ++kt) {
    const int cur = kt & 1;
    if (kt + 1 < nk) stage(cur ^ 1, kt + 1);
    const uint8_t* As = smem + cur * MX_STAGE;
    const uint8_t* Ws = As + MX_TILE;
    const uint8_t* SAs = As + 2 * MX_TILE;
    const uint8_t* SWs = SAs + 1024;
    auto frag = [&](const uint8_t* p, int r) {
      (void)r;
      const bf16x8 lo8 = *(const bf16x8*)(p + lane_lo);
      const bf16x8 hi8 = *(const bf16x8*)(p + lane_hi);
      const int4 lo = __builtin_bit_cast(int4, lo8), hi = __builtin_bit_cast(int4, hi8);
      return (i32x8){lo.x, lo.y, lo.z, lo.w, hi.x, hi.y, hi.z, hi.w};
    };
    uint32_t sbp = 0;
#pragma unroll
    for (int j = 0; j < 4; ++j) sbp |= (uint32_t)SWs[(wc * 64 + j * 16 + fr) * 4 + fq] << (8 * j);
    auto pass = [&](auto JH) {
      constexpr int jh = decltype(JH)::value;
      i32x8 bfr[2];
#pragma unroll
      for (int jj = 0; jj < 2; ++jj) {
        bfr[jj] = frag(Ws + (wc * 64 + (2 * jh + jj) * 16) * MX_BK, 0);
      }
#pragma unroll
      for (int i = 0; i < 8; ++i) {
        const i32x8 af = frag(As + (wr * 128 + i * 16) * MX_BK, 0);
        const int sa = SAs[(wr * 128 + i * 16 + fr) * 4 + fq];
        acc[i][2 * jh] = __builtin_amdgcn_mfma_scale_f32_16x16x128_f8f6f4(af, bfr[0], acc[i][2 * jh], 0, 0, 0, sa,
                                                                          2 * jh, (int)sbp);
        acc[i][2 * jh + 1] = __builtin_amdgcn_mfma_scale_f32_16x16x128_f8f6f4(af, bfr[1], acc[i][2 * jh + 1], 0, 0, 0,
                                                                              sa, 2 * jh + 1, (int)sbp);
        __builtin_amdgcn_sched_barrier(0);
      }
    };
    pass(std::integral_constant<int, 0>{});
    pass(std::integral_constant<int, 1>{});
    __syncthreads();
  }

  const int ncol0 = n0 + wc * 64;
  const int rc = (lane & 15) * 4;
  float4 bias4 = make_float4(0.f, 0.f, 0.f, 0.f);
  if (ea.bias) {
    const int n = ncol0 + rc;
    bias4.x = ea.bias[min(n, N - 1)];
    bias4.y = ea.bias[min(n + 1, N - 1)];
    bias4.z = ea.bias[min(n + 2, N - 1)];
    bias4.w = ea.bias[min(n + 3, N - 1)];
  }
  float* wimg = (float*)smem + wid * (64 * GB_EPI_LD);
#pragma unroll
  for (int half = 0; half < 2; ++half) {
    const int ib = 4 * half;
    if (half) __syncthreads();
#pragma unroll
    for (int ii = 0; ii < 4; ++ii)
#pragma unroll
      for (int j = 0; j < 4; ++j)
#pragma unroll
        for (int r = 0; r < 4; ++r) wimg[(ii * 16 + fq * 4 + r) * GB_EPI_LD + j * 16 + fr] = acc[ib + ii][j][r];
    __syncthreads();
    const int mrow0 = m0 + wr * 128 + ib * 16;
#pragma unroll 4
    for (int rr = 0; rr < 16; ++rr) {
      const int lr = rr * 4 + (lane >> 4);
      const int m = mrow0 + lr;
      float4 v = *(const float4*)(wimg + lr * GB_EPI_LD + rc);
      v.x += bias4.x; v.y += bias4.y; v.z += bias4.z; v.w += bias4.w;
      if constexpr (EPI == TW_EPI_GELU_MX) {
        v = gelu_erf4(v);
        const uint32_t sbyte = mx_scale_byte(mx_group8_max(abs4max(v.x, v.y, v.z, v.w)));
        const uint32_t w = mx_pack4(v.x, v.y, v.z, v.w, mx_inv_scale(sbyte));
        if (m < M) {
          *(uint32_t*)((uint8_t*)ea.out + (size_t)m * ea.ldo + ncol0 + rc) = w;
          if ((lane & 7) == 0) ea.sout[tw_mx_sidx(m, (ncol0 + rc) >> 5, ea.s_rows)] = (uint8_t)sbyte;
        }
      } else {
        if (m < M && ncol0 + rc < N) epi_store4<EPI>(ea, m, ncol0 + rc, N, v);
      }
    }
  }
}

#define MX8_SC (8 * 128 * MX_BK)
template <int EPI>
__global__ __launch_bounds__(512, 1) void k_gemm_8p_mx(const uint8_t* __restrict__ A, const uint8_t* __restrict__ W,
                                                       const uint8_t* __restrict__ Sa, const uint8_t* __restrict__ Sw,
// ... 259 lines not shown
```

turbo-whisper-workspace_amd/twamd/_lib.py:

```python
from __future__ import annotations

import ctypes
import os

import torch

LIB_PATH = os.path.join(os.path.dirname(os.path.abspath(__file__)), "libtwhip.so")
DEBUG_LIB_PATH = os.path.join(os.path.dirname(os.path.abspath(__file__)), "libtwhip_dbg.so")

TW_EPI_BF16 = 0
TW_EPI_GELU_BF16 = 1
TW_EPI_RESID_F32 = 2
TW_EPI_GELU_POS_F32 = 3
TW_EPI_F32 = 4
TW_EPI_CROSSKV = 5
TW_EPI_GELU_PACKED = 6
TW_EPI_GELU_MX = 7
TW_EPI_GELU_F32 = 8
TW_EPI_PARTIAL_F32 = 100

TW_SELECT_CHUNKS = 16
TW_SELECT_WS_PER_ROW = 128
TW_STATE_STRIDE = 8
TW_ST_NGEN, TW_ST_LAST, TW_ST_PENULT, TW_ST_LASTTS, TW_ST_FINISHED, TW_ST_LANG = 0, 1, 2, 3, 4, 5
TW_ST_SUMLP, TW_ST_NOSPEECH = 6, 7
TW_HIST_MAX = 448
TW_HIST_LANG = -1

EXPORTED = (
    "tw_version", "tw_last_error", "tw_fill_synth", "tw_f32_to_bf16", "tw_logmel", "tw_im2col_conv1",
    "tw_im2col_conv2", "tw_gemm_bf16", "tw_layernorm", "tw_attn_encoder", "tw_attn_decode_self",
    "tw_attn_decode_cross", "tw_embed_decoder", "tw_logits_select", "tw_gemm_bf16_partial", "tw_resid_layernorm",
    "tw_gemm_set_variant", "tw_attn_set_variant",
    "tw_dtw", "tw_attn_decode_cross_probs", "tw_attn_decode_cross_grouped", "tw_attn_decode_cross_grouped_ws_bytes", "tw_attn_decode_self_tab", "tw_beam_workspace_bytes", "tw_beam_step", "tw_kv_reorder", "tw_pack_weight", "tw_gemv_packed", "tw_resid_layernorm_packed", "tw_flac_probe", "tw_flac_decode", "tw_resample_pcm_i32", "tw_resample_pcm_f32",
    "tw_gemm_mx", "tw_quant_mx", "tw_layernorm_mx", "tw_attn_encoder_mx", "tw_gemm_mx_set_variant", "tw_logits_select_embed",
    "tw_attn_set_lds_pad", "tw_logits_sample", "tw_token_prob", "tw_g711_decode", "tw_ima_adpcm_wav_decode",
    "tw_ms_adpcm_wav_decode", "tw_ima_qt_decode", "tw_alac_parse_cookie", "tw_alac_decode",
    "tw_kv_tab_check", "tw_debug_build", "tw_resid_layernorm_packed_to", "tw_conv2_gemm",
    "tw_logmel_long", "tw_im2col_conv1_long", "tw_attn_decode_self_masked", "tw_attn_decode_self_tab_masked",
    "tw_gemv_set_wide_slices", "tw_vorbis_probe", "tw_vorbis_decode", "tw_vorbis_imdct",
    "tw_layernorm_set_lds_pad", "tw_gemv_set_variant",
    "tw_gemm_f32", "tw_layernorm_f32", "tw_im2col_conv1_f32", "tw_im2col_conv2_f32", "tw_embed_decoder_f32",
    "tw_attn_encoder_f32", "tw_attn_decode_self_f32", "tw_attn_decode_cross_f32", "tw_gemm_set_epilogue",
    "tw_gemm_set_persistent_grid", "tw_mp3_probe", "tw_mp3_decode", "tw_aac_parse_asc", "tw_aac_decode_raw",
    "tw_aac_adts_probe", "tw_aac_adts_decode", "tw_dec_fused", "tw_dec_fused_sync_bytes", "tw_dec_fused_supported",
    "tw_dec_fused_set_grid", "tw_dec_fused_set_acquire", "tw_dec_fused_set_probe", "tw_dec_fused_grid",
    "tw_dec_fused_xpart_bytes", "tw_logits_history",
)


class TwSelectParams(ctypes.Structure):
    _fields_ = [
        ("V", ctypes.c_int32), ("eos", ctypes.c_int32), ("pad", ctypes.c_int32), ("ts_begin", ctypes.c_int32),
        ("no_timestamps", ctypes.c_int32), ("max_initial_ts", ctypes.c_int32), ("use_timestamps", ctypes.c_int32),
        ("max_new", ctypes.c_int32), ("mode", ctypes.c_int32), ("lo", ctypes.c_int32), ("hi", ctypes.c_int32),
        ("n_begin_suppress", ctypes.c_int32), ("begin_suppress", ctypes.c_int32 * 8),
    ]


class TwBeamParams(ctypes.Structure):
    _fields_ = [("num_beams", ctypes.c_int32), ("max_new", ctypes.c_int32), ("length_penalty", ctypes.c_float),
                ("ld_tokens", ctypes.c_int32), ("scores_are_logprobs", ctypes.c_int32)]


class TwBeamState(ctypes.Structure):
    _fields_ = [("run_score", ctypes.c_void_p), ("fin_score", ctypes.c_void_p), ("fin_flag", ctypes.c_void_p),
                ("fin_len", ctypes.c_void_p), ("fin_tokens", ctypes.c_void_p), ("win", ctypes.c_void_p),
                ("src_rows", ctypes.c_void_p), ("kv_tab", ctypes.c_void_p), ("fin_tab", ctypes.c_void_p),
                ("run_lp", ctypes.c_void_p), ("fin_lp", ctypes.c_void_p)]


class TwFlacInfo(ctypes.Structure):
    _fields_ = [
        ("sample_rate", ctypes.c_int32), ("channels", ctypes.c_int32), ("bits_per_sample", ctypes.c_int32),
        ("min_blocksize", ctypes.c_int32), ("max_blocksize", ctypes.c_int32), ("total_from_frames", ctypes.c_int32),
        ("total_samples", ctypes.c_int64), ("audio_offset", ctypes.c_int64), ("md5", ctypes.c_uint8 * 16),
    ]


class TwVorbisInfo(ctypes.Structure):
    _fields_ = [
        ("sample_rate", ctypes.c_int32), ("channels", ctypes.c_int32), ("blocksize0", ctypes.c_int32),
        ("blocksize1", ctypes.c_int32), ("total_samples", ctypes.c_int64),
    ]


class TwMp3Info(ctypes.Structure):
    _fields_ = [
        ("sample_rate", ctypes.c_int32), ("channels", ctypes.c_int32), ("version", ctypes.c_int32),
        ("bitrate_kbps", ctypes.c_int32), ("total_samples", ctypes.c_int64), ("n_frames", ctypes.c_int64),
        ("skip_samples", ctypes.c_int64), ("samples_per_frame", ctypes.c_int32), ("enc_delay", ctypes.c_int32),
        ("enc_padding", ctypes.c_int32), ("flags", ctypes.c_int32), ("layer", ctypes.c_int32),
    ]


class TwAlacInfo(ctypes.Structure):
    _fields_ = [
        ("sample_rate", ctypes.c_int32), ("channels", ctypes.c_int32), ("bit_depth", ctypes.c_int32),
        ("frame_length", ctypes.c_int32), ("pb", ctypes.c_int32), ("mb", ctypes.c_int32), ("kb", ctypes.c_int32),
    ]


class TwAacInfo(ctypes.Structure):
    _fields_ = [
        ("sample_rate", ctypes.c_int32), ("channels", ctypes.c_int32), ("object_type", ctypes.c_int32),
        ("frame_length", ctypes.c_int32), ("n_frames", ctypes.c_int64), ("total_samples", ctypes.c_int64),
    ]


class TwError(RuntimeError):
    pass


_P = ctypes.c_void_p
_I = ctypes.c_int
_L = ctypes.c_long
_F = ctypes.c_float
_U64 = ctypes.c_uint64
_U32 = ctypes.c_uint32

_SIGS = {
    "tw_version": ([], _I),
    "tw_last_error": ([], ctypes.c_char_p),
    "tw_fill_synth": ([_P, _L, _U64, _U32, _F, _F, _I, _P], _I),
    "tw_f32_to_bf16": ([_P, _P, _L, _F, _P], _I),
    "tw_logmel": ([_P, _I, _P, _P, _P, _I, _P, _P, _P], _I),
    "tw_im2col_conv1": ([_P, _I, _P, _P, _I, _I, _P, _P], _I),
    "tw_im2col_conv1_long": ([_P, _I, _L, _P, _P, _P, _I, _I, _P, _P], _I),
    "tw_logmel_long": ([_P, _L, _P, _P, _P, _I, _P, _L, _P, _P], _I),
    "tw_im2col_conv2": ([_P, _I, _I, _P, _P], _I),
    "tw_conv2_gemm": ([_P, _I, _I, _P, _P, _P, _P, _P], _I),
    "tw_gemm_bf16": ([_P, _P, _I, _I, _I, _I, _I, _I, _P, _I, _P, _P, _I, _P, _P], _I),
    "tw_layernorm": ([_P, _P, _P, _I, _I, _F, _P, _P], _I),
    "tw_gemm_set_epilogue": ([_I], _I),
    "tw_gemm_set_persistent_grid": ([_I], _I),
    "tw_gemm_f32": ([_P, _P, _I, _I, _I, _I, _I, _I, _P, _I, _P, _P, _I, _P, _P], _I),
    "tw_layernorm_f32": ([_P, _P, _P, _I, _I, _F, _P, _P], _I),
    "tw_im2col_conv1_f32": ([_P, _I, _L, _P, _P, _P, _I, _I, _P, _P], _I),
    "tw_im2col_conv2_f32": ([_P, _I, _I, _P, _P], _I),
    "tw_embed_decoder_f32": ([_P, _P, _P, _P, _I, _I, _P, _P], _I),
    "tw_attn_encoder_f32": ([_P, _I, _I, _I, _P, _P], _I),
    "tw_attn_decode_self_f32": ([_P, _I, _I, _I, _P, _P, _P, _P, _I, _P, _P, _P], _I),
    "tw_attn_decode_cross_f32": ([_P, _I, _I, _I, _I, _P, _P, _P, _P, _U32, _I, _I, _P, _I, _I, _P], _I),
    "tw_gemm_mx": ([_P, _P, _P, _P, _I, _I, _I, _I, _I, _I, _I, _I, _P, _I, _P, _P, _I, _P], _I),
    "tw_quant_mx": ([_P, _I, _I, _I, _P, _P, _I, _P], _I),
    "tw_attn_encoder_mx": ([_P, _I, _I, _I, _P, _P, _I, _P], _I),
    "tw_layernorm_mx": ([_P, _P, _P, _I, _I, _F, _P, _P, _I, _P], _I),
    "tw_attn_encoder": ([_P, _I, _I, _I, _P, _P], _I),
    "tw_attn_decode_self": ([_P, _I, _I, _I, _P, _P, _P, _P, _P], _I),
    "tw_attn_decode_self_masked": ([_P, _I, _I, _I, _P, _P, _P, _P, _P, _P], _I),
    "tw_attn_decode_cross": ([_P, _I, _I, _I, _I, _P, _P, _P, _P], _I),
    "tw_attn_decode_cross_grouped": ([_P, _I, _I, _I, _I, _P, _I, _I, _P, _P, _P, _P], _I),
    "tw_embed_decoder": ([_P, _P, _P, _P, _I, _I, _P, _P], _I),
    "tw_logits_select": ([_P, _I, _I, _P, ctypes.POINTER(TwSelectParams), _P, _P, _I, _P, _P, _P, _P], _I),
    "tw_logits_sample": ([_P, _I, _I, _P, ctypes.POINTER(TwSelectParams), ctypes.c_float, _I, ctypes.c_uint64, _P, _P,
                          _P, _I, _P, _P, _P], _I),
    "tw_token_prob": ([_P, _I, _I, _I, _I, _P, _P], _I),
    "tw_logits_history": ([_P, _I, _I, _I, _P, _I, _P, _P, _I, _P, _F, _I, _I, _P], _I),
    "tw_gemm_bf16_partial": ([_P, _P, _I, _I, _I, _I, _I, _I, _P, _I, _P], _I),
    "tw_gemv_set_wide_slices": ([_I], _I),
    "tw_gemv_set_variant": ([_I], _I),
    "tw_gemm_set_variant": ([_I], _I),
    "tw_gemm_mx_set_variant": ([_I], _I),
    "tw_logits_select_embed": ([_P, _I, _I, _P, ctypes.POINTER(TwSelectParams), _P, _P, _I, _P, _P, _P, _P, _P, _I,
                                _I, _P, _P, _P, _F, _P, _I, _P], _I),
    "tw_attn_set_variant": ([_I], _I),
    "tw_attn_set_lds_pad": ([_I], _I),
    "tw_resid_layernorm": ([_P, _P, _I, _P, _P, _P, _I, _I, _F, _P, _P], _I),
    "tw_dtw": ([_P, _I, _I, _P, _P, _P], _I),
    "tw_attn_decode_cross_probs": ([_P, _I, _I, _I, _I, _P, _P, _P, _P, _U32, _I, _I, _P, _I, _I, _P], _I),
    "tw_beam_workspace_bytes": ([_I], ctypes.c_size_t),
    "tw_attn_decode_cross_grouped_ws_bytes": ([_I, _I], ctypes.c_size_t),
    "tw_attn_decode_self_tab": ([_P, _I, _I, _I, _P, _P, _P, _P, _I, _P, _P], _I),
    "tw_attn_decode_self_tab_masked": ([_P, _I, _I, _I, _P, _P, _P, _P, _I, _P, _P, _P], _I),
    "tw_kv_tab_check": ([_P, _P, _I, _I, _I, _P, _P], _I),
    "tw_debug_build": ([], _I),
    "tw_beam_step": ([_P, _I, _I, _P, ctypes.POINTER(TwSelectParams), ctypes.POINTER(TwBeamParams),
                      ctypes.POINTER(TwBeamState), _P, _P, _P, _P, _P, _P], _I),
    "tw_kv_reorder": ([_P, _P, _P, _P, _I, _I, _I, _I, _I, _P, _P, _P], _I),
    "tw_pack_weight": ([_P, _I, _I, _I, _P, _P], _I),
    "tw_gemv_packed": ([_P, _I, _I, _P, _I, _I, _I, _I, _P, _I, _P, _I, _P], _I),
    "tw_resid_layernorm_packed": ([_P, _P, _I, _P, _P, _P, _I, _I, _F, _P, _P], _I),
    "tw_resid_layernorm_packed_to": ([_P, _P, _P, _I, _P, _P, _P, _I, _I, _F, _P, _P], _I),
    "tw_flac_probe": ([_P, ctypes.c_int64, ctypes.POINTER(TwFlacInfo)], _I),
    "tw_flac_decode": ([_P, ctypes.c_int64, _P, ctypes.c_int64, _I, ctypes.POINTER(ctypes.c_int64)], _I),
    "tw_g711_decode": ([_P, ctypes.c_int64, _I, _P], _I),
    "tw_vorbis_probe": ([_P, ctypes.c_int64, ctypes.POINTER(TwVorbisInfo)], _I),
    "tw_vorbis_decode": ([_P, ctypes.c_int64, _P, ctypes.c_int64, _I, ctypes.POINTER(ctypes.c_int64)], _I),
    "tw_vorbis_imdct": ([_P, _I, _P], _I),
    "tw_mp3_probe": ([_P, ctypes.c_int64, ctypes.POINTER(TwMp3Info)], _I),
    "tw_mp3_decode": ([_P, ctypes.c_int64, _P, ctypes.c_int64, _I, ctypes.POINTER(ctypes.c_int64)], _I),
    "tw_aac_parse_asc": ([_P, _I, ctypes.POINTER(TwAacInfo)], _I),
    "tw_aac_decode_raw": ([_P, _I, _P, ctypes.c_int64, _P, _P, ctypes.c_int64, _P, ctypes.c_int64, _I,
                           ctypes.POINTER(ctypes.c_int64)], _I),
    "tw_aac_adts_probe": ([_P, ctypes.c_int64, ctypes.POINTER(TwAacInfo)], _I),
    "tw_aac_adts_decode": ([_P, ctypes.c_int64, _P, ctypes.c_int64, _I, ctypes.POINTER(ctypes.c_int64)], _I),
    "tw_layernorm_set_lds_pad": ([_I], _I),
    "tw_ima_adpcm_wav_decode": ([_P, ctypes.c_int64, _I, _I, _P, ctypes.c_int64, ctypes.POINTER(ctypes.c_int64)], _I),
    "tw_ms_adpcm_wav_decode": ([_P, ctypes.c_int64, _I, _I, _P, ctypes.c_int64, ctypes.POINTER(ctypes.c_int64)], _I),
    "tw_ima_qt_decode": ([_P, ctypes.c_int64, _I, _P, ctypes.c_int64, ctypes.POINTER(ctypes.c_int64)], _I),
    "tw_alac_parse_cookie": ([_P, ctypes.c_int64, _P], _I),
    "tw_alac_decode": ([_P, ctypes.c_int64, _P, ctypes.c_int64, _P, _P, ctypes.c_int64, _P, ctypes.c_int64, _I,
                        ctypes.POINTER(ctypes.c_int64)], _I),
    "tw_resample_pcm_i32": ([_P, ctypes.c_int64, _I, _F, _I, _I, _P, _I, _P, ctypes.c_int64, _P], _I),
    "tw_resample_pcm_f32": ([_P, ctypes.c_int64, _I, _I, _I, _P, _I, _P, ctypes.c_int64, _P], _I),
    "tw_dec_fused": ([_P, _I, _I, _P, _P, _P, _P, _L, _I, _P, _L, _L, _I, _P, _P, _P, _P, _P, _P, _P, _P, _F, _P, _P,
                      _P], _I),
    "tw_dec_fused_xpart_bytes": ([_I], ctypes.c_size_t),
    "tw_dec_fused_sync_bytes": ([], ctypes.c_size_t),
    "tw_dec_fused_supported": ([_I, _I, _I, _I], _I),
    "tw_dec_fused_set_grid": ([_I], _I),
    "tw_dec_fused_set_acquire": ([_I], _I),
    "tw_dec_fused_set_probe": ([_P], _I),
    "tw_dec_fused_grid": ([], _I),
}

_lib = None
_dbg = None


def _open(path: str) -> ctypes.CDLL:
    if not os.path.exists(path):
        raise TwError(f"HIP library not built: {path} (run `make -C turbo-whisper-workspace_amd/csrc`)")
    lib = ctypes.CDLL(path)
    for name, (args, res) in _SIGS.items():
        fn = getattr(lib, name)
        fn.argtypes = args
        fn.restype = res
    return lib


def load(path: str = LIB_PATH) -> ctypes.CDLL:
    global _lib
    if _lib is not None:
        return _lib
    if os.environ.get("TW_LIB"):
        raise TwError("TW_LIB is no longer read: A/B builds load their library explicitly (_lib.load_debug or a "
                      "separate process over another in-tree build)")
    _lib = _open(path)
    return _lib


def load_debug() -> ctypes.CDLL:
    global _dbg
    if _dbg is None:
        _dbg = _open(DEBUG_LIB_PATH)
        if _dbg.tw_debug_build() != 1:
            raise TwError(f"{DEBUG_LIB_PATH} is not a TW_DEBUG build")
    return _dbg


def call(name: str, *args) -> None:
    lib = load()
    rc = getattr(lib, name)(*args)
    if rc != 0:
        raise TwError(f"{name} failed ({rc}): {lib.tw_last_error().decode(errors='replace')}")


def ptr(t) -> int:
    return 0 if t is None else t.data_ptr()


def stream_handle(stream=None) -> int:
    s = stream if stream is not None else torch.cuda.current_stream()
    return s.cuda_stream
```

turbo-whisper-workspace_amd/twamd/engine.py:

```python
from __future__ import annotations

import contextlib
import ctypes
import dataclasses
import gc
import os
import time
from typing import Dict, List, Optional, Sequence

import numpy as np
import torch

from . import _lib, _ops, alignment
from .config import GenerationSettings, WhisperDims
from .frontend import CHUNK_SAMPLES, N_FRAMES, dft_basis, mel_table, pack_k8
from .segments import (FallbackConfig, condition_prefixes, fallback_sequence, need_fallback, retrieve_segment,
                       segment_slices, strip_generated)
from .weights import PackedWeights

import functools

LN_EPS = 1e-5
S_ENC = 1500

# ... 47 lines not shown
                return fn(self, *args, **kwargs)
        finally:
            cur.wait_stream(self.stream)

    return wrapper


@dataclasses.dataclass
class DecView:
    r0: int
    n: int
    stream: torch.cuda.Stream
    xd: torch.Tensor
    qkvd: torch.Tensor
    qd: torch.Tensor
    attd: torch.Tensor
    logits: torch.Tensor
    parts: torch.Tensor
    sel_ws: torch.Tensor
    state: torch.Tensor
    tokens: torch.Tensor
    ids: torch.Tensor
    pos: torch.Tensor
    hp: torch.Tensor
    fp: torch.Tensor
    fsync: Optional[torch.Tensor] = None


class _EncoderPump:

    def __init__(self, eng: "WhisperEngine", steps, ahead: int = 2):
        self.eng, self.steps, self.ahead = eng, steps, ahead
        self.pending: List[torch.cuda.Event] = []
        self.done = False

    def __call__(self) -> bool:
        queued = False
        while not self.done:
            while self.pending and self.pending[0].query():
                self.pending.pop(0)
            if len(self.pending) >= self.ahead:
                break
            self._one()
            queued = True
        return queued

    def _one(self) -> None:
        try:
            next(self.steps)
        except StopIteration:
            self.done = True
            return
        ev = torch.cuda.Event()
        ev.record(self.eng.enc_stream)
        self.pending.append(ev)

    def drain(self) -> None:
        while not self.done:
            self._one()
        self.pending.clear()


def fallback_row_key(window: int, pass_no: int, fi: int) -> int:
    if not (0 <= int(pass_no) < 1024 and 0 <= int(fi) < 16):
        raise ValueError(f"sampler key fields out of range: pass {pass_no} (< 1024), temperature index {fi} (< 16)")
    key = (int(window) * 1024 + int(pass_no)) * 16 + int(fi)
    if not 0 <= key < 2 ** 31:
        raise ValueError(f"sampler key out of range: window {window}, pass {pass_no}")
    return key


@dataclasses.dataclass
class PassResult:
    tokens: List[List[int]]
    lang_ids: Optional[List[int]]
    token_ts: Optional[List[np.ndarray]] = None
    sum_logprob: Optional[List[float]] = None
    no_speech_prob: Optional[List[float]] = None


class WhisperEngine:
    def __init__(self, weights: PackedWeights, gen: GenerationSettings, max_batch: int = 24,
                 device: str = "cuda", use_graphs: bool = True, max_beams: int = 1,
                 enc_fp8: Optional[bool] = None):
        _lib.load()
        self.ops = _ops.load()
        self.enc_via_ops = True
        d = weights.dims
        d.validate()
        if self.F32 != (weights.conv1_w.dtype == torch.float32):
            raise ValueError(f"{type(self).__name__} needs {'f32' if self.F32 else 'bf16'} weights "
                             "(build_weights(..., dtype=...))")
        self.d, self.w, self.gen = d, weights, gen
        self.max_batch = max_batch
        self.max_beams = max(1, int(max_beams))
        self.max_rows = max_batch * self.max_beams
        self.device = torch.device(device)
        self.use_graphs = use_graphs
        self.stream = torch.cuda.Stream(self.device, priority=-1)
        self.enc_stream = torch.cuda.Stream(self.device, priority=0)
        self._enc_ev = [torch.cuda.Event(), torch.cuda.Event()]
        D, F, H, V, B = d.d_model, d.ffn, d.heads, d.vocab, max_batch
        dev, bf, f32, i32 = self.device, torch.bfloat16, torch.float32, torch.int32
        act = f32 if self.F32 else bf
        c, s = dft_basis()
        self.basis_cos = torch.from_numpy(pack_k8(c)).to(dev)
        self.basis_sin = torch.from_numpy(pack_k8(s)).to(dev)
        self.mel_fb = torch.from_numpy(pack_k8(mel_table(d.n_mels))).to(dev)
        self.wave = torch.zeros(B, CHUNK_SAMPLES, dtype=f32, device=dev)
        self.feats_buf = torch.zeros(2, B, d.n_mels, N_FRAMES, dtype=f32, device=dev)
        self.feats = self.feats_buf[0]
        self.maxkeys = torch.zeros(B, dtype=torch.int32, device=dev)
        M3, M15 = B * N_FRAMES, B * S_ENC
        self.a1 = torch.empty(M3, weights.kpad1, dtype=act, device=dev)
        self._h1_rows = torch.zeros(M3 + 1, D, dtype=act, device=dev)
        self.h1 = self._h1_rows[1:]
        self._conv2_im2col = False
        self.a2 = torch.empty(M15, 3 * D, dtype=act, device=dev) if self._conv2_im2col or self.F32 else None
        self.x = torch.empty(M15, D, dtype=f32, device=dev)
        self.hln = torch.empty(M15, D, dtype=act, device=dev)
        self.qkv = torch.empty(M15, 3 * D, dtype=act, device=dev)
        self.att = torch.empty(M15, D, dtype=act, device=dev)
        self.ffn = torch.empty(M15, F, dtype=act, device=dev)
        self.enc_fp8 = (os.environ.get("TW_ENC_FP8", "0") == "1") if enc_fp8 is None else bool(enc_fp8)
        if self.F32 and self.enc_fp8:
            raise ValueError("the fp32 path has no MX fp8 encoder")
        self.enc_mx: List[Dict[str, tuple]] = []
        if self.enc_fp8:
            u8 = torch.uint8
            self.m15p = _pad256(M15)
            self.hq = torch.empty(M15, D, dtype=u8, device=dev)
            self.hq_s = torch.zeros(D // 128, self.m15p, 4, dtype=u8, device=dev)
            self.attq = torch.empty(M15, D, dtype=u8, device=dev)
            self.attq_s = torch.zeros(D // 128, self.m15p, 4, dtype=u8, device=dev)
            self.ffnq = torch.empty(M15, F, dtype=u8, device=dev)
            self.ffnq_s = torch.zeros(F // 128, self.m15p, 4, dtype=u8, device=dev)
            with torch.cuda.device(self.device):
                self.enc_mx = [{k: self._quant_weight(getattr(L, k)) for k in ("wqkv", "wo", "w1", "w2")}
                               for L in weights.enc]
                torch.cuda.synchronize(self.device)
        self.cross_kv_buf = torch.empty(2, d.decoder_layers, 2, B, H, S_ENC, 64, dtype=act, device=dev)
        self.cross_kv = self.cross_kv_buf[0]
        self._slot = 0
        T = d.max_target_positions
        B = self.max_rows
        self.kcache = torch.zeros(d.decoder_layers, B, H, T, 64, dtype=act, device=dev)
        self.vcache = torch.zeros(d.decoder_layers, B, H, T, 64, dtype=act, device=dev)
        self.xd = torch.empty(B, D, dtype=f32, device=dev)
        self.qkvd = torch.empty(B, 3 * D, dtype=act, device=dev)
        self.qd = torch.empty(B, D, dtype=act, device=dev)
        self.attd = torch.empty(B, D, dtype=act, device=dev)
        self.logits = torch.empty(B, V, dtype=f32, device=dev)
        self.parts = torch.empty(DEC_SPLITS, B, D, dtype=f32, device=dev)
        self.sel_ws = torch.empty(B, _lib.TW_SELECT_WS_PER_ROW, dtype=f32, device=dev)
        self.state = torch.zeros(B, _lib.TW_STATE_STRIDE, dtype=i32, device=dev)
        self.tokens = torch.zeros(B, T, dtype=i32, device=dev)
        self.ids = torch.zeros(B, dtype=i32, device=dev)
        self.pos = torch.zeros(B, dtype=i32, device=dev)
        self.row_map = torch.zeros(max_batch, dtype=i32, device=dev)
        self.seek = torch.zeros(max_batch, dtype=i32, device=dev)
        self.dec_row_map = torch.zeros(B, dtype=i32, device=dev)
        self._use_dec_row_map = False
        self._row_group = 1
        self._xws: Optional[torch.Tensor] = None
        self._kv_tab: Optional[torch.Tensor] = None
        self._long: Optional[dict] = None
        self._kv_start = torch.zeros(self.max_rows, dtype=torch.int32, device=dev)
        self._masked = False
        self._hist_prefix = torch.zeros(self.max_rows, T, dtype=i32, device=dev)
        self._hist_len = torch.zeros(self.max_rows, dtype=i32, device=dev)
        self._hist: Optional[tuple] = None
        self._dec_ctx = (1, 0, False)
        self._fused_dims = (not self.F32 and bool(_lib.load().tw_dec_fused_supported(D, H, d.ffn, 1)))
        self._fused_tab: Optional[torch.Tensor] = None
        self._fused_err = torch.zeros(4, dtype=torch.int32, device=dev)
        self._fused_xpart = (torch.empty(int(_lib.load().tw_dec_fused_xpart_bytes(32)) // 4, dtype=torch.float32,
                                         device=dev) if self._fused_dims else None)
        self._beam: Optional[dict] = None
        self._align: Optional[dict] = None
        self._align_buf: Optional[torch.Tensor] = None
        self.suppress_bits = torch.zeros((V + 31) // 32, dtype=torch.int32, device=dev)
        self.set_suppress_tokens(gen.suppress_tokens)
        self.n_chains = 1
        self._chain_streams = [torch.cuda.Stream(self.device, priority=-1) for _ in range(self.n_chains)]
        self._own_streams = {x.cuda_stream for x in [self.stream, self.enc_stream] + self._chain_streams}
        self._graphs: Dict[tuple, torch.cuda.CUDAGraph] = {}
        self._chain_cache: Dict[tuple, List[DecView]] = {}
        self._pump: Optional[_EncoderPump] = None
        self.dec_ahead = 1
        self.pump_ahead = 2
        self.fused_select = not self.F32
        self.graph_steps_alone = 1
        self.graph_steps_beside = 1
        self.prompt_graph = True
        self.attn_kernel = (32, 32)
        self.attn_pad = (0, 4)
        self.ln_pad = (0, 0)
        self.overlap = True
        self.dec_p: List[Dict[str, torch.Tensor]] = []
        self.emb_p: Optional[torch.Tensor] = None
        if not self.F32:
            with torch.cuda.device(self.device):
                self.dec_p = [{k: self._pack(getattr(L, k)) for k in ("wqkv", "wo", "wq_x", "wo_x", "w1", "w2")}
                              for L in weights.dec]
                self.emb_p = self._pack(weights.emb)
                if self._fused_dims:
                    self._fused_tab = self._fused_table()
                torch.cuda.synchronize(self.device)

    closed = False
    F32 = False

    def close(self) -> None:
        if self.closed:
            return
        for st in [self.stream, self.enc_stream] + list(getattr(self, "_chain_streams", [])):
            st.synchronize()
        for key in reversed(list(self._graphs)):
            self._graphs.pop(key).reset()
        self._graphs.clear()
        self._pump = None
        self.step_hook = None
        self.pass_events = None
        self.replay_host = None
        self.timers = None
        self._enc_ev = []
        self._chain_cache.clear()
        keep = {"d", "gen", "max_batch", "max_beams", "max_rows", "device", "closed", "_own_streams"}
        for name in list(vars(self)):
            if name not in keep and isinstance(getattr(self, name), (torch.Tensor, list, dict, tuple)):
                setattr(self, name, None)
        self.w = None
        self.closed = True

    def __enter__(self) -> "WhisperEngine":
        return self

    def __exit__(self, *exc) -> None:
        self.close()

    def _quant_weight(self, W: torch.Tensor) -> tuple:
        N, K = W.shape
        Np = _pad256(N)
        q = torch.empty(N, K, dtype=torch.uint8, device=self.device)
        sc = torch.zeros(K // 128, Np, 4, dtype=torch.uint8, device=self.device)
        _lib.call("tw_quant_mx", W.data_ptr(), N, K, K, q.data_ptr(), sc.data_ptr(), Np,
                  torch.cuda.current_stream(self.device).cuda_stream)
        return q, sc, Np

    def _gemm_mx(self, A, As, Wt, M, N, K, epi, out, bias=None, sout=None, stream=None):
        st = stream or self.stream
        Wq, Ws, Np = Wt
        rec = self._begin_timer(("gemm_mx", epi), 2.0 * M * N * K, st)
        _lib.call("tw_gemm_mx", A.data_ptr(), As.data_ptr(), Wq.data_ptr(), Ws.data_ptr(), M, N, K, K, K, self.m15p,
                  Np, epi, out.data_ptr(), N, _lib.ptr(bias), _lib.ptr(sout), self.m15p if sout is not None else 0,
                  st.cuda_stream)
        self._end_timer(rec, st)

    def _pack(self, W: torch.Tensor) -> torch.Tensor:
        N, K = W.shape
        Wp = torch.empty((N + 15) // 16 * 16 * K, dtype=torch.bfloat16, device=self.device)
        _lib.call("tw_pack_weight", W.data_ptr(), N, K, K, Wp.data_ptr(), torch.cuda.current_stream().cuda_stream)
        return Wp

    def _gemv(self, A, a_packed: bool, Wp, M, N, K, epi, out, v: DecView, bias=None, splits=1, ldo=None):
        rec = self._begin_timer(("gemv_packed", epi), 2.0 * M * N * K, v.stream)
        _lib.call("tw_gemv_packed", A.data_ptr(), int(a_packed), K, Wp.data_ptr(), M, N, K, epi, out.data_ptr(),
                  ldo if ldo is not None else N, _lib.ptr(bias), splits, v.stream.cuda_stream)
        self._end_timer(rec, v.stream)

    def _resid_ln_p(self, R, nparts, bias, g, b, v: DecView):
        _lib.call("tw_resid_layernorm_packed", v.xd.data_ptr(), v.parts.data_ptr() if nparts else None, nparts,
                  _lib.ptr(bias), _lib.ptr(g), _lib.ptr(b), R, self.d.d_model, LN_EPS, v.hp.data_ptr(),
                  v.stream.cuda_stream)

    def set_suppress_tokens(self, tokens: Sequence[int]) -> None:
        V = self.d.vocab
        bits = np.zeros((V + 31) // 32, np.uint32)
        for t in tokens:
            if 0 <= t < V:
                bits[t >> 5] |= np.uint32(1 << (t & 31))
        self.suppress_bits.copy_(torch.from_numpy(bits.view(np.int32)))
        self.gen.suppress_tokens = list(tokens)

    @property
    def _s(self) -> int:
        return self.stream.cuda_stream

    _enc_cur = None

    def _on(self, st):
        if self._enc_cur == st.cuda_stream or torch.cuda.current_stream(self.device).cuda_stream == st.cuda_stream:
            return contextlib.nullcontext()
        return torch.cuda.stream(st)

    @contextlib.contextmanager
    def _enc_chunk_ctx(self, st):
        with torch.cuda.stream(st):
            self._enc_cur = st.cuda_stream
            try:
                yield
            finally:
                self._enc_cur = None

    @staticmethod
    def _rows(t, M):
        return t if t.shape[0] == M else t[:M]

    def _gemm(self, A, W, M, N, K, epi, out, bias=None, aux=None, aux_rows=0, kv_geom=None, stream=None):
        st = stream or self.stream
        rec = self._begin_timer(("gemm_skinny" if M <= 32 else "gemm_big", epi), 2.0 * M * N * K, st)
        assert A.shape[1] == K and W.shape[0] == N and W.shape[1] == K
        if self.enc_via_ops:
            with self._on(st):
                self.ops.gemm_bf16_out(self._rows(A, M), W, epi, out if epi == _lib.TW_EPI_CROSSKV else
                                       self._rows(out, M), bias, aux, aux_rows,
                                       list(kv_geom) if kv_geom is not None else None)
        else:
            _lib.call("tw_gemm_bf16", A.data_ptr(), W.data_ptr(), M, N, K, K, K, epi, out.data_ptr(), N,
                      _lib.ptr(bias), _lib.ptr(aux), aux_rows,
                      None if kv_geom is None else (ctypes.c_int * 4)(*kv_geom), st.cuda_stream)
        self._end_timer(rec, st)

    timers: Optional[dict] = None
    timer_families: Optional[set] = None
# ... 62 lines not shown
        return DecView(r0, n, stream or self.stream, self.xd[sl], self.qkvd[sl], self.qd[sl], self.attd[sl],
                       self.logits[sl], self.parts if parts is None else parts, self.sel_ws[sl], self.state[sl],
                       self.tokens[sl], self.ids[sl], self.pos[sl], hp, fp, fsync)

    @on_engine_streams
    def set_long_input(self, wave: Optional[torch.Tensor]) -> int:
        if wave is None:
            self._long = None
            return 0
        wave = wave.to(self.device, torch.float32).contiguous()
        n = int(wave.numel())
        T = n // 160
        ld = max(T, N_FRAMES)
        feats = torch.zeros(self.d.n_mels, ld, dtype=torch.float32, device=self.device)
        key = torch.zeros(1, dtype=torch.int32, device=self.device)
        _lib.call("tw_logmel_long", wave.data_ptr(), n, self.basis_cos.data_ptr(), self.basis_sin.data_ptr(),
                  self.mel_fb.data_ptr(), self.d.n_mels, feats.data_ptr(), ld, key.data_ptr(),
                  torch.cuda.current_stream(self.device).cuda_stream)
        mf = torch.tensor([T], dtype=torch.int32, device=self.device)
        self.stream.wait_stream(torch.cuda.current_stream(self.device))
        self.enc_stream.wait_stream(torch.cuda.current_stream(self.device))
        self._long = {"feats": feats, "ld": ld, "max_frames": mf, "T": T, "wave": wave}
        return T

    def use_slot(self, slot: int) -> None:
        self._slot = slot
        self.cross_kv = self.cross_kv_buf[slot]
        self.feats = self.feats_buf[slot]

    @on_engine_streams
    def logmel(self, n: int, slot: Optional[int] = None, sync: bool = True) -> None:
        slot = self._slot if slot is None else slot
        st = self._enc_begin(sync)
        with self._on(st):
            self.ops.logmel_out(self.wave[:n], self.basis_cos, self.basis_sin, self.mel_fb, self.d.n_mels,
                                self.feats_buf[slot][:n], self.maxkeys)
        self._enc_end(sync, slot)

    @on_engine_streams
    def encode(self, R: int, row_map=True, seek=True, slot: Optional[int] = None, sync: bool = True,
               alone: bool = True) -> None:
        self._pump_drain()
        for _ in self._encode_steps(R, row_map, seek, slot, sync, alone=alone):
            pass

    gemm_alone = 6
    gemm_beside = 1
    gemm_beside_cus = 224
    mx_alone = 0
    mx_beside = 0

    def _set_gemm_context(self, alone: bool) -> None:
        _lib.call("tw_gemm_set_variant", self.gemm_alone if alone else self.gemm_beside)
        _lib.call("tw_gemm_set_persistent_grid", 0 if alone else self.gemm_beside_cus)
        _lib.call("tw_attn_set_variant", self.attn_kernel[0 if alone else 1])
        _lib.call("tw_attn_set_lds_pad", self.attn_pad[0 if alone else 1])
        _lib.call("tw_layernorm_set_lds_pad", self.ln_pad[0 if alone else 1])
        if self.enc_fp8:
            _lib.call("tw_gemm_mx_set_variant", self.mx_alone if alone else self.mx_beside)

    def _encode_steps(self, R: int, row_map=True, seek=True, slot: Optional[int] = None, sync: bool = True,
                      alone: bool = True):
        chunks = self._encode_chunks(R, row_map, seek, slot, sync)
        while True:
            self._set_gemm_context(alone)
            try:
                next(chunks)
            except StopIteration:
                break
            yield
        self._set_gemm_context(True)

    def _encode_chunks(self, R: int, row_map=True, seek=True, slot: Optional[int] = None, sync: bool = True):
        d, w = self.d, self.w
        slot = self._slot if slot is None else slot
        D, F, H = d.d_model, d.ffn, d.heads
        M3, M15 = R * N_FRAMES, R * S_ENC
        st = self._enc_begin(sync)
        s = st.cuda_stream
        with self._enc_chunk_ctx(st):
            if self._long is not None:
                lf = self._long
                _lib.call("tw_im2col_conv1_long", lf["feats"].data_ptr(), d.n_mels, lf["ld"],
                          lf["max_frames"].data_ptr(), self.row_map.data_ptr() if row_map else None,
                          self.seek.data_ptr(), R, w.kpad1, self.a1.data_ptr(), s)
            else:
                _lib.call("tw_im2col_conv1", self.feats_buf[slot].data_ptr(), d.n_mels,
                          self.row_map.data_ptr() if row_map else None, self.seek.data_ptr() if seek else None, R,
                          w.kpad1, self.a1.data_ptr(), s)
            self._gemm(self.a1, w.conv1_w, M3, D, w.kpad1, _lib.TW_EPI_GELU_BF16, self.h1, bias=w.conv1_b, stream=st)
            if self._conv2_im2col:
                _lib.call("tw_im2col_conv2", self.h1.data_ptr(), R, D, self.a2.data_ptr(), s)
                self._gemm(self.a2, w.conv2_w, M15, D, 3 * D, _lib.TW_EPI_GELU_POS_F32, self.x, bias=w.conv2_b,
                           aux=w.pos_enc, aux_rows=S_ENC, stream=st)
            else:
                rec = self._begin_timer(("gemm_big", _lib.TW_EPI_GELU_POS_F32), 2.0 * M15 * D * 3 * D, st)
                _lib.call("tw_conv2_gemm", self.h1.data_ptr(), R, D, w.conv2_w.data_ptr(), w.conv2_b.data_ptr(),
                          w.pos_enc.data_ptr(), self.x.data_ptr(), s)
                self._end_timer(rec, st)
        yield
        if self.enc_fp8:
            yield from self._encode_layers_mx(R, st)
        for L in ([] if self.enc_fp8 else w.enc):
            with self._enc_chunk_ctx(st):
                self._ln(self.x, L.ln1_g, L.ln1_b, M15, self.hln, stream=st)
                self._gemm(self.hln, L.wqkv, M15, 3 * D, D, _lib.TW_EPI_BF16, self.qkv, bias=L.bqkv, stream=st)
                rec = self._begin_timer(("attn_encoder", 0), 4.0 * S_ENC * S_ENC * 64 * H * R, st)
                if self.enc_via_ops:
                    with self._on(st):
                        self.ops.attn_encoder_out(self._rows(self.qkv, M15), R, H, self._rows(self.att, M15))
                else:
                    _lib.call("tw_attn_encoder", self.qkv.data_ptr(), R, S_ENC, H, self.att.data_ptr(), s)
                self._end_timer(rec, st)
                self._gemm(self.att, L.wo, M15, D, D, _lib.TW_EPI_RESID_F32, self.x, bias=L.bo, stream=st)
                self._ln(self.x, L.ln2_g, L.ln2_b, M15, self.hln, stream=st)
                self._gemm(self.hln, L.w1, M15, F, D, _lib.TW_EPI_GELU_BF16, self.ffn, bias=L.b1, stream=st)
                self._gemm(self.ffn, L.w2, M15, D, F, _lib.TW_EPI_RESID_F32, self.x, bias=L.b2, stream=st)
            yield
        with self._enc_chunk_ctx(st):
            self._ln(self.x, w.enc_ln_g, w.enc_ln_b, M15, self.hln, stream=st)
            geom = (S_ENC, R, D, H)
            self._gemm(self.hln, w.wkv_x, M15, d.decoder_layers * 2 * D, D, _lib.TW_EPI_CROSSKV,
                       self.cross_kv_buf[slot], bias=w.bkv_x, kv_geom=geom, stream=st)
        self._enc_end(sync, slot)

    def _encode_layers_mx(self, R: int, st):
        d, w = self.d, self.w
        D, F, H = d.d_model, d.ffn, d.heads
        M15, s = R * S_ENC, st.cuda_stream
        for L, Q in zip(w.enc, self.enc_mx):
            _lib.call("tw_layernorm_mx", self.x.data_ptr(), L.ln1_g.data_ptr(), L.ln1_b.data_ptr(), M15, D, LN_EPS,
                      self.hq.data_ptr(), self.hq_s.data_ptr(), self.m15p, s)
            self._gemm_mx(self.hq, self.hq_s, Q["wqkv"], M15, 3 * D, D, _lib.TW_EPI_BF16, self.qkv, bias=L.bqkv,
                          stream=st)
            rec = self._begin_timer(("attn_encoder", 0), 4.0 * S_ENC * S_ENC * 64 * H * R, st)
            _lib.call("tw_attn_encoder_mx", self.qkv.data_ptr(), R, S_ENC, H, self.attq.data_ptr(),
                      self.attq_s.data_ptr(), self.m15p, s)
            self._end_timer(rec, st)
            self._gemm_mx(self.attq, self.attq_s, Q["wo"], M15, D, D, _lib.TW_EPI_RESID_F32, self.x, bias=L.bo,
                          stream=st)
            _lib.call("tw_layernorm_mx", self.x.data_ptr(), L.ln2_g.data_ptr(), L.ln2_b.data_ptr(), M15, D, LN_EPS,
                      self.hq.data_ptr(), self.hq_s.data_ptr(), self.m15p, s)
            self._gemm_mx(self.hq, self.hq_s, Q["w1"], M15, F, D, _lib.TW_EPI_GELU_MX, self.ffnq, bias=L.b1,
                          sout=self.ffnq_s, stream=st)
            self._gemm_mx(self.ffnq, self.ffnq_s, Q["w2"], M15, D, F, _lib.TW_EPI_RESID_F32, self.x, bias=L.b2,
                          stream=st)
            yield

    def encoder_output(self, R: int) -> torch.Tensor:
        return self.hln[: R * S_ENC].view(R, S_ENC, self.d.d_model)

    @on_engine_streams
    def decoder_step(self, R: int, with_logits: bool = True, v: Optional[DecView] = None, r_enc: Optional[int] = None,
                     pre_embedded: bool = False) -> None:
        if v is None and R > VIEW_ROWS:
            r_enc = R if r_enc is None else r_enc
            for r0 in range(0, R, VIEW_ROWS):
                n = min(VIEW_ROWS, R - r0)
                self.decoder_step(n, with_logits, self._view(r0, n), r_enc, pre_embedded)
            return
        v = v or self._view(0, R)
        r_enc = R if r_enc is None else r_enc
        d, w = self.d, self.w
        D, F, H, T = d.d_model, d.ffn, d.heads, d.max_target_positions
        st = v.stream
        s = st.cuda_stream
        if not pre_embedded:
            _lib.call("tw_embed_decoder", w.emb.data_ptr(), w.pos_dec.data_ptr(), v.ids.data_ptr(), v.pos.data_ptr(), R,
                      D, v.xd.data_ptr(), s)
        if self._fused_ok(R):
            self._fused_layers(R, r_enc, v)
            if with_logits:
                self._gemv(v.hp, True, self.emb_p, R, d.vocab, D, _lib.TW_EPI_F32, v.logits, v)
            return
        xkv_stride = 2 * r_enc * H * S_ENC * 64
        nparts, pbias = 0, None
        PART, K4 = _lib.TW_EPI_PARTIAL_F32, DEC_SPLITS
        for li, L in enumerate(w.dec):
            P = self.dec_p[li]
            kc, vc = self.kcache[li, v.r0:].data_ptr(), self.vcache[li, v.r0:].data_ptr()
            if li or not pre_embedded:
                self._resid_ln_p(R, nparts, pbias, L.ln1_g, L.ln1_b, v)
            self._gemv(v.hp, True, P["wqkv"], R, 3 * D, D, _lib.TW_EPI_BF16, v.qkvd, v, bias=L.bqkv)
            ks = self._kv_start[v.r0:].data_ptr() if self._masked else None
            if self._kv_tab is not None:
                if ks is not None:
                    _lib.call("tw_attn_decode_self_tab_masked", v.qkvd.data_ptr(), R, H, T, v.pos.data_ptr(), kc, vc,
                              self._kv_tab.data_ptr(), v.r0, ks, v.attd.data_ptr(), s)
                else:
                    _lib.call("tw_attn_decode_self_tab", v.qkvd.data_ptr(), R, H, T, v.pos.data_ptr(), kc, vc,
                              self._kv_tab.data_ptr(), v.r0, v.attd.data_ptr(), s)
            elif ks is not None:
                _lib.call("tw_attn_decode_self_masked", v.qkvd.data_ptr(), R, H, T, v.pos.data_ptr(), kc, vc, ks,
                          v.attd.data_ptr(), s)
            else:
                _lib.call("tw_attn_decode_self", v.qkvd.data_ptr(), R, H, T, v.pos.data_ptr(), kc, vc,
                          v.attd.data_ptr(), s)
            self._gemv(v.attd, False, P["wo"], R, D, D, PART, v.parts, v, splits=K4)
            self._resid_ln_p(R, K4, L.bo, L.ln2_g, L.ln2_b, v)
            self._gemv(v.hp, True, P["wq_x"], R, D, D, _lib.TW_EPI_BF16, v.qd, v, bias=L.bq_x)
            ckv, rmap = self._cross_ptrs(li, xkv_stride, v)
            rec = self._begin_timer(("attn_decode_cross", 0), 2.0 * R * H * S_ENC * 64 * 2, st)
            self._cross_attend(li, R, r_enc, rmap, ckv, v)
            self._end_timer(rec, st)
            self._gemv(v.attd, False, P["wo_x"], R, D, D, PART, v.parts, v, splits=K4)
            self._resid_ln_p(R, K4, L.bo_x, L.ln3_g, L.ln3_b, v)
            self._gemv(v.hp, True, P["w1"], R, F, D, _lib.TW_EPI_GELU_PACKED, v.fp, v, bias=L.b1)
            self._gemv(v.fp, True, P["w2"], R, D, F, PART, v.parts, v, splits=K4)
            nparts, pbias = K4, L.b2
        if with_logits:
            self._resid_ln_p(R, nparts, pbias, w.dec_ln_g, w.dec_ln_b, v)
            self._gemv(v.hp, True, self.emb_p, R, d.vocab, D, _lib.TW_EPI_F32, v.logits, v)

    def _cross_attend(self, li: int, R: int, r_enc: int, rmap, ckv, v: DecView) -> None:
        H, s = self.d.heads, v.stream.cuda_stream
        al = self._align
        if al is not None and li in al["layers"]:
            mask, slot0 = al["layers"][li]
            row_stride = al["n_steps"] * al["n_slots"] * S_ENC * 4
            _lib.call("tw_attn_decode_cross_probs", v.qd.data_ptr(), R, H, S_ENC, r_enc, rmap, ckv, v.attd.data_ptr(),
                      al["buf"].data_ptr() + v.r0 * row_stride, mask, slot0, al["n_slots"], v.pos.data_ptr(),
                      al["pos0"], al["n_steps"], s)
        elif self._row_group > 1 and rmap is not None:
            g = self._row_group
            if self._xws is None:
                nbytes = int(_lib.load().tw_attn_decode_cross_grouped_ws_bytes(self.max_rows, H))
                self._xws = torch.empty(nbytes // 4, dtype=torch.float32, device=self.device)
            row_bytes = self._xws.numel() * 4 // self.max_rows
            _lib.call("tw_attn_decode_cross_grouped", v.qd.data_ptr(), R, H, S_ENC, r_enc, rmap, g, (g - v.r0 % g) % g,
                      ckv, self._xws.data_ptr() + v.r0 * row_bytes, v.attd.data_ptr(), s)
        else:
            _lib.call("tw_attn_decode_cross", v.qd.data_ptr(), R, H, S_ENC, r_enc, rmap, ckv, v.attd.data_ptr(), s)

    def _align_setup(self, R: int, pos0: int, n_steps: int) -> None:
        heads = self.gen.alignment_heads
        if not heads:
            raise ValueError("token-level timestamps need generation alignment_heads")
        layers: Dict[int, tuple] = {}
        slot = 0
        for li in sorted({l for l, _ in heads}):
            hs = sorted({h for l, h in heads if l == li})
            layers[li] = (sum(1 << h for h in hs), slot)
            slot += len(hs)
        order = [(l, h) for l in sorted(layers) for h in sorted({hh for ll, hh in heads if ll == l})]
        shape = (self.max_rows, n_steps, slot, S_ENC)
        buf = self._align_buf if getattr(self, "_align_buf", None) is not None else None
        if buf is None or buf.numel() < int(np.prod(shape)):
            buf = torch.empty(int(np.prod(shape)), dtype=torch.float32, device=self.device)
            self._align_buf = buf
        perm = [order.index((l, h)) for l, h in heads]
        self._align = {"layers": layers, "n_slots": slot, "pos0": pos0, "n_steps": n_steps, "buf": buf, "perm": perm}

    def _align_weights(self, R: int, n_rows: int) -> np.ndarray:
        al = self._align
        b = al["buf"][: R * al["n_steps"] * al["n_slots"] * S_ENC].view(R, al["n_steps"], al["n_slots"], S_ENC)
        w = b[:, :n_rows].permute(0, 2, 1, 3)[:, al["perm"]].float().cpu().numpy()
        return w

    def _cross_ptrs(self, li: int, xkv_stride: int, v: DecView):
        H, esz = self.d.heads, self.cross_kv.element_size()
        base = self.cross_kv.data_ptr() + li * xkv_stride * esz
        if self._use_dec_row_map:
            return base, self.dec_row_map.data_ptr() + 4 * v.r0
        return base + v.r0 * H * S_ENC * 64 * esz, None

    def _select_params(self, mode: int, max_new: int, use_timestamps: bool = True) -> _lib.TwSelectParams:
        st, g = self.gen.special, self.gen
        p = _lib.TwSelectParams()
        p.V, p.eos, p.pad = self.d.vocab, st.eot, st.eot
        p.ts_begin, p.no_timestamps = st.timestamp_begin, st.notimestamps
        p.max_initial_ts = -1 if g.max_initial_timestamp_index is None else g.max_initial_timestamp_index
        p.use_timestamps = int(use_timestamps)
        p.max_new, p.mode = max_new, mode
        p.lo, p.hi = st.lang_begin, st.lang_end
        bs = list(g.begin_suppress_tokens or [])
        p.n_begin_suppress = len(bs)
        for i, t in enumerate(bs):
            p.begin_suppress[i] = t
        return p

    def _select(self, R: int, params: _lib.TwSelectParams, tokens: bool = True, v: Optional[DecView] = None,
                embed_next: bool = False) -> None:
        if v is None and R > VIEW_ROWS:
            for r0 in range(0, R, VIEW_ROWS):
                self._select(min(VIEW_ROWS, R - r0), params, tokens, self._view(r0, min(VIEW_ROWS, R - r0)), embed_next)
            return
        v = v or self._view(0, R)
        if params.mode == 0:
            self._history(v.r0, R, v.stream)
        if embed_next:
            L0 = self.w.dec[0]
            _lib.call("tw_logits_select_embed", v.logits.data_ptr(), R, self.d.vocab, self.suppress_bits.data_ptr(),
                      ctypes.byref(params), v.state.data_ptr(), v.tokens.data_ptr() if tokens else None,
                      v.tokens.shape[1], v.ids.data_ptr(), v.pos.data_ptr(), v.sel_ws.data_ptr(),
                      self.w.emb.data_ptr(), self.w.pos_dec.data_ptr(), self.d.d_model, self.d.max_target_positions,
                      v.xd.data_ptr(), L0.ln1_g.data_ptr(), L0.ln1_b.data_ptr(), LN_EPS,
                      v.hp.data_ptr(), 1, v.stream.cuda_stream)
            return
        _lib.call("tw_logits_select", v.logits.data_ptr(), R, self.d.vocab, self.suppress_bits.data_ptr(),
                  ctypes.byref(params), v.state.data_ptr(), v.tokens.data_ptr() if tokens else None,
                  v.tokens.shape[1], v.ids.data_ptr(), v.pos.data_ptr(), v.sel_ws.data_ptr(), v.stream.cuda_stream)

    def _hist_begin(self, R: int, repetition_penalty: float, no_repeat_ngram_size: int, tail: Sequence[int],
                    lang_ids: Optional[Sequence[int]], prefix=None) -> None:
        p, n = float(repetition_penalty or 1.0), int(no_repeat_ngram_size or 0)
        if p == 1.0 and n == 0:
            self._hist = None
            return
        st = self.gen.special
        rows = []
        for r in range(R):
            h = [int(t) for t in prefix[0][r]] if prefix is not None and prefix[0] else []
            h.append(st.sot)
            if st.is_multilingual:
                h.append(_lib.TW_HIST_LANG if lang_ids is None else int(lang_ids[r]))
            h.extend(int(t) for t in tail)
            rows.append(h)
        L = len(rows[0])
        if L > self._hist_prefix.shape[1]:
            raise ValueError(f"decoder prompt of {L} tokens exceeds {self._hist_prefix.shape[1]} positions")
        self._hist_prefix[:R, :L] = torch.as_tensor(rows, dtype=torch.int32, device=self.device)
        self._hist_len[:R] = L
        self._hist = (p, n)

    def _history(self, r0: int, R: int, stream, to_logprobs: bool = False) -> None:
        if self._hist is None:
            return
        p, n = self._hist
        _lib.call("tw_logits_history", self.logits[r0:].data_ptr(), R, self.logits.stride(0), self.d.vocab,
                  self._hist_prefix[r0:].data_ptr(), self._hist_prefix.stride(0), self._hist_len[r0:].data_ptr(),
                  self.tokens[r0:].data_ptr(), self.tokens.stride(0), self.state[r0:].data_ptr(), p, n,
                  int(to_logprobs), stream.cuda_stream)

    step_hook = None
    pass_events: Optional[list] = None
    replay_host: Optional[list] = None

    def embed_head(self, v: Optional[DecView] = None, R: Optional[int] = None) -> None:
        if v is not None:
            self._embed_head(v)
            return
        for r0 in range(0, R, VIEW_ROWS):
            self._embed_head(self._view(r0, min(VIEW_ROWS, R - r0)))

    def _embed_head(self, v: DecView) -> None:
        L0 = self.w.dec[0]
        _lib.call("tw_embed_decoder", self.w.emb.data_ptr(), self.w.pos_dec.data_ptr(), v.ids.data_ptr(),
                  v.pos.data_ptr(), v.n, self.d.d_model, v.xd.data_ptr(), v.stream.cuda_stream)
        self._resid_ln_p(v.n, 0, None, L0.ln1_g, L0.ln1_b, v)

    def _gen_step(self, R: int, params, v: Optional[DecView] = None, r_enc: Optional[int] = None,
                  fused: bool = False) -> None:
        self.decoder_step(R, v=v, r_enc=r_enc, pre_embedded=fused)
        self._select(R, params, v=v, embed_next=fused)

    dec_alone_wide_kw = 1
    dec_beside_wide_kw = 1

    dec_alone_gemv = 1
    dec_beside_gemv = 0

    dec_fused_alone = False
    dec_fused_max_rows = 4

    @property
    def _wide_kw(self) -> int:
        return self._dec_ctx[0]

    def _dec_context(self) -> tuple:
        beside = self._pump is not None
        ctx = ((self.dec_beside_wide_kw, self.dec_beside_gemv, False) if beside
               else (self.dec_alone_wide_kw, self.dec_alone_gemv, bool(self.dec_fused_alone and self._fused_dims)))
        if ctx[:2] != self._dec_ctx[:2]:
            _lib.call("tw_gemv_set_wide_slices", ctx[0])
            _lib.call("tw_gemv_set_variant", ctx[1])
        self._dec_ctx = ctx
        return ctx

    def _fused_ok(self, R: int) -> bool:
        return (self._dec_ctx[2] and R <= min(32, self.dec_fused_max_rows) and self._kv_tab is None
                and not self._masked and self._align is None and not self._use_dec_row_map)

    def _fused_layers(self, R: int, r_enc: int, v: DecView) -> None:
        d, w = self.d, self.w
        H, T = d.heads, d.max_target_positions
        esz = self.cross_kv.element_size()
        xkv = self.cross_kv.data_ptr() + v.r0 * H * S_ENC * 64 * esz
        _lib.call("tw_dec_fused", self._fused_tab.data_ptr(), d.decoder_layers, R, v.pos.data_ptr(), v.xd.data_ptr(),
                  self.kcache[0, v.r0].data_ptr(), self.vcache[0, v.r0].data_ptr(), self.kcache.stride(0), T, xkv,
                  2 * r_enc * H * S_ENC * 64, r_enc * H * S_ENC * 64, S_ENC, v.qd.data_ptr(), v.attd.data_ptr(),
                  v.fp.data_ptr(), v.parts.data_ptr(), self._fused_xpart.data_ptr(), w.dec_ln_g.data_ptr(),
                  w.dec_ln_b.data_ptr(), v.hp.data_ptr(),
                  LN_EPS, v.fsync.data_ptr(), self._fused_err.data_ptr(), v.stream.cuda_stream)

    def _fused_table(self) -> torch.Tensor:
        names_w = ("wqkv", "wo", "wq_x", "wo_x", "w1", "w2")
        names_f = ("bqkv", "bo", "bq_x", "bo_x", "b1", "b2", "ln1_g", "ln1_b", "ln2_g", "ln2_b", "ln3_g", "ln3_b")
        rows = []
        for L, P in zip(self.w.dec, self.dec_p):
            for k in names_f:
                t = getattr(L, k)
                if t.dtype != torch.float32 or not t.is_contiguous():
                    raise ValueError(f"tw_dec_fused: decoder {k} must be contiguous f32")
            rows.append([P[k].data_ptr() for k in names_w] + [getattr(L, k).data_ptr() for k in names_f])
        return torch.tensor(rows, dtype=torch.int64, device=self.device)

    def check_fused(self) -> None:
        e = int(self._fused_err[0].item())
        if e:
            self._fused_err.zero_()
            raise _lib.TwError(f"tw_dec_fused: a phase wait timed out (code {e:#x}); the decode pass is void")

    def _prompt_len(self, tail: Sequence[int], prefix=None) -> int:
        L = len(prefix[0][0]) if prefix is not None and prefix[0] else 0
        return L + 1 + (1 if self.gen.special.is_multilingual else 0) + len(tail)

    def _token_ts(self, R: int, P: int, res: PassResult, num_frames: Optional[Sequence[int]]) -> None:
        st = self.gen.special
        real = [(t.index(st.eot) + 1) if st.eot in t else len(t) for t in res.tokens]
        rows = max(real) - 1 if real else 0
        w = self._align_weights(R, rows) if rows > 0 else None
        res.token_ts = []
        for r in range(R):
            nf = None if num_frames is None else int(num_frames[r])
            ts = (alignment.token_timestamps(w[r], 0, nf, self.gen.median_filter_width) if w is not None
                  else np.zeros(1, np.float32))
            res.token_ts.append(np.concatenate([np.zeros(P, np.float32), ts]))

    def _prefill(self, R: int, prefix, r_enc: Optional[int] = None) -> int:
        if prefix is None:
            return 0
        rows, pads = prefix
        L = len(rows[0]) if rows else 0
        if L == 0:
            return 0
        if len(rows) != R or any(len(r) != L for r in rows):
            raise ValueError("prefix: one left-padded row of equal length per decoder row")
        dev = self.device
        cols = torch.as_tensor(rows, dtype=torch.int32, device=dev)
        self._kv_start[:R] = torch.as_tensor(list(pads), dtype=torch.int32, device=dev)
        self._masked = True
        for k in range(L):
            self.ids[:R] = cols[:, k]
            self.pos[:R] = k
            self.decoder_step(R, with_logits=False, r_enc=r_enc)
        return L

    @on_engine_streams
    def _detect_languages(self, R: int) -> List[int]:
        st = self.gen.special
        self._dec_context()
        self.stream.wait_event(self._enc_ev[self._slot])
        with torch.cuda.stream(self.stream):
            self.state[:R].zero_()
            self.state[:R, _lib.TW_ST_LAST:_lib.TW_ST_LASTTS + 1] = -1
            self.pos[:R] = 0
            self.ids[:R] = st.sot
            self.decoder_step(R)
            self._select(R, self._select_params(1, 1), tokens=False)
            out = self.ids[:R].tolist()
        return [int(x) for x in out]

    @on_engine_streams
    def decode_pass(self, R: int, tail: Sequence[int], lang_ids: Optional[Sequence[int]], max_new: int,
                    check_every: int = 8, use_timestamps: bool = True, align: bool = False,
                    num_frames: Optional[Sequence[int]] = None, prefix=None, repetition_penalty: float = 1.0,
                    no_repeat_ngram_size: int = 0) -> PassResult:
        if align:
            P = self._prompt_len(tail, prefix)
            self._align_setup(R, P, max_new)
            try:
                res = self.decode_pass(R, tail, lang_ids, max_new, check_every, use_timestamps, prefix=prefix,
                                       repetition_penalty=repetition_penalty,
                                       no_repeat_ngram_size=no_repeat_ngram_size)
                self._token_ts(R, P, res, num_frames)
                return res
            finally:
                self._align = None
        st = self.gen.special
        dev = self.device
        self._dec_context()
        self.stream.wait_event(self._enc_ev[self._slot])
        detect = st.is_multilingual and lang_ids is None
        params = self._select_params(0, max_new, use_timestamps)
        base = self._prefill(R, prefix)
        self._hist_begin(R, repetition_penalty, no_repeat_ngram_size, tail, lang_ids, prefix)

        def prompt() -> None:
            self.state[:R].zero_()
            self.state[:R, _lib.TW_ST_LAST:_lib.TW_ST_LASTTS + 1] = -1
            self.pos[:R] = base
            self.ids[:R] = st.sot
            prompt_rest: List = []
            if st.is_multilingual:
                prompt_rest.append(None if lang_ids is None else list(lang_ids))
            prompt_rest.extend(int(t) for t in tail)
            for k, tok in enumerate(prompt_rest):
                if k == 0 and detect:
                    self.decoder_step(R)
                    self._select(R, self._select_params(1, max_new), tokens=False)
                    continue
                self.decoder_step(R, with_logits=False)
                if isinstance(tok, list):
                    self.ids[:R] = torch.as_tensor(tok, dtype=torch.int32, device=dev)
                else:
                    self.ids[:R] = tok
                self.pos[:R] = base + k + 1
            self._gen_step(R, params)

        if self.use_graphs and self.prompt_graph and (detect or not st.is_multilingual) and not base:
            al = self._align
            key = ("prompt", R, tuple(int(t) for t in tail), max_new, use_timestamps, self._slot,
                   None if al is None else (al["pos0"], al["n_steps"], al["buf"].data_ptr()), self._dec_ctx,
                   self._hist)
            g = self._graphs.get(key)
            if g is None:
                g = torch.cuda.CUDAGraph()
                with _capture(g, self.stream):
                    prompt()
                self._graphs[key] = g
            g.replay()
        else:
            prompt()
        steps = 1
        chains = self._chains(R)
# ... 696 lines not shown
```

Baseline: 8185 audio-s/wall-s.

## Fold greedy token-selection partial reduction into vocab projection GEMV epilogue

Adds a packed GEMV variant for the output vocabulary projection that computes per-16-column masked best-text, best-timestamp and timestamp log-sum-exp records in its epilogue, writing them to the selection workspace. A new final-select kernel, optionally fused with the next-token embed and layernorm, then merges these records, so the separate k_select_partial pass that re-reads the full fp32 logits is skipped. It is enabled by default for greedy decoding with at most 32 rows and no history penalties. The trade-off is extra epilogue work and register pressure in the GEMV, plus many more partial records to merge in the final kernel.

```diff
diff --git a/include/tw_whisper.h b/include/tw_whisper.h
--- a/include/tw_whisper.h
+++ b/include/tw_whisper.h
@@ -31,6 +31,7 @@
 
 #define TW_SELECT_CHUNKS 16
 #define TW_SELECT_WS_PER_ROW 128
+#define TW_SELECT_REC_WORDS 8
 
 typedef struct TwSelectParams {
   int32_t V;
@@ -124,6 +125,10 @@
 int tw_pack_weight(const uint16_t* W, int N, int K, int ldw, uint16_t* Wp, void* stream);
 int tw_gemv_packed(const uint16_t* A, int a_packed, int lda, const uint16_t* Wp, int M, int N, int K, int epi,
                    void* out, int ldo, const float* bias, int splits, void* stream);
+int tw_gemv_packed_select(const uint16_t* A, const uint16_t* Wp, int M, int N, int K, float* logits, int ldo,
+                          const uint32_t* suppress_bits, const TwSelectParams* params, const int* state,
+                          float* workspace, void* stream);
+int tw_gemv_packed_select_records(int N);
 int tw_gemv_set_wide_slices(int kw);
 int tw_gemv_set_variant(int v);
 int tw_gemm_set_epilogue(int tr);
@@ -200,6 +205,13 @@
                            int max_pos, float* x, const float* gamma, const float* beta, float eps, uint16_t* out,
                            int packed, void* stream);
 
+int tw_select_final(const float* workspace, int n_records, int B, const TwSelectParams* params, int* state,
+                    int* tokens_out, int ld_tokens, int* next_ids, int* pos, void* stream);
+int tw_select_final_embed(const float* workspace, int n_records, int B, const TwSelectParams* params, int* state,
+                          int* tokens_out, int ld_tokens, int* next_ids, int* pos, const uint16_t* tok_emb,
+                          const uint16_t* pos_emb, int D, int max_pos, float* x, const float* gamma, const float* beta,
+                          float eps, uint16_t* out, int packed, void* stream);
+
 int tw_logits_sample(const float* logits, int B, int ld_logits, const uint32_t* suppress_bits,
                      const TwSelectParams* params, float temperature, int top_k, uint64_t seed, const int* row_key,
                      int* state, int* tokens_out, int ld_tokens, int* next_ids, int* pos, void* stream);
diff --git a/turbo-whisper-workspace_amd/csrc/decode.hip b/turbo-whisper-workspace_amd/csrc/decode.hip
--- a/turbo-whisper-workspace_amd/csrc/decode.hip
+++ b/turbo-whisper-workspace_amd/csrc/decode.hip
@@ -1,20 +1,6 @@
 #include "tw_common.h"
 #include "../../include/tw_whisper.h"
-
-struct Best {
-  float v;
-  int i;
-};
-__device__ inline Best best_of(Best a, Best b) {
-  if (b.v > a.v || (b.v == a.v && b.i < a.i)) return b;
-  return a;
-}
-__device__ inline void lse_merge(float& m, float& s, float m2, float s2) {
-  if (m2 == -INFINITY) return;
-  if (m == -INFINITY) { m = m2; s = s2; return; }
-  if (m2 > m) { s = s * __expf(m - m2) + s2; m = m2; }
-  else s = s + s2 * __expf(m2 - m);
-}
+#include "tw_select.h"
 
 __device__ inline void lse_add1(float& m, float& s, float x) {
   const float d = x - m;
@@ -23,38 +9,11 @@
   m = fmaxf(m, x);
 }
 
-struct SelPart {
-  float bt_v; int bt_i;
-  float bs_v; int bs_i;
-  float m_ts, s_ts;
-  float pad0, pad1;
-};
-
-struct RowMask {
-  int init_step, mask_ts_all, mask_text_lt_eos, ts_hi_block;
-};
-__device__ inline RowMask row_mask(const int* st, const TwSelectParams& p) {
-  const int n_gen = st[TW_ST_NGEN], last = st[TW_ST_LAST], penult = st[TW_ST_PENULT], last_ts = st[TW_ST_LASTTS];
-  const int tsb = p.ts_begin;
-  RowMask r{n_gen == 0, 0, 0, tsb};
-  if (p.mode == 0 && p.use_timestamps) {
-    const bool last_was_ts = n_gen >= 1 && last >= tsb;
-    const bool penult_was_ts = n_gen < 2 || penult >= tsb;
-    if (last_was_ts) {
-      if (penult_was_ts) r.mask_ts_all = 1;
-      else r.mask_text_lt_eos = 1;
-    }
-    if (last_ts >= 0) r.ts_hi_block = (last_was_ts && !penult_was_ts) ? last_ts : last_ts + 1;
-  }
-  return r;
-}
-
 template <bool TX>
 __device__ inline void sel_chunk(const float* __restrict__ row, const uint32_t* __restrict__ suppress_bits,
                                  const TwSelectParams& p, const RowMask& rm, int v0, int v1, SelPart* sp,
                                  SelPart& out, float& m_tx, float& s_tx) {
   const int tid = threadIdx.x, lane = tid & 63, wid = tid >> 6;
-  const int tsb = p.ts_begin;
   Best bt{-INFINITY, 0x7fffffff}, bs{-INFINITY, 0x7fffffff};
   float m_ts = -INFINITY, s_ts = 0.f;
   for (int base = v0 + tid; base < v1; base += 4 * 256) {
@@ -71,26 +30,10 @@
       const int v = base + 256 * u;
       const bool ok = v < v1;
       float x = xs[u];
-      bool masked;
-      if (p.mode == 1) {
-        masked = (v < p.lo || v >= p.hi);
-      } else {
-        masked = (sb[u] >> (v & 31)) & 1u;
-        if (rm.init_step)
-          for (int i = 0; i < p.n_begin_suppress; ++i) masked |= (v == p.begin_suppress[i]);
-        if (p.use_timestamps) {
-          masked |= (v == p.no_timestamps);
-          if (v >= tsb) {
-            masked |= rm.mask_ts_all || (v < rm.ts_hi_block);
-            if (rm.init_step && p.max_initial_ts >= 0) masked |= (v > tsb + p.max_initial_ts);
-          } else {
-            masked |= (rm.mask_text_lt_eos && v < p.eos) || rm.init_step;
-          }
-        }
-      }
+      const bool masked = sel_masked(p, rm, sel_col_bits(p, sb[u], v, rm.init_step), v);
       if (masked) x = -INFINITY;
       if (!ok) continue;
-      if (v < tsb || !p.use_timestamps || p.mode == 1) {
+      if (sel_is_text(p, v)) {
         bt = best_of(bt, Best{x, v});
         if (TX && x != -INFINITY) lse_merge(m_tx, s_tx, x, 1.f);
       } else {
@@ -135,17 +78,31 @@
   if (threadIdx.x == 0) ws[b * NC + c] = out;
 }
 
-__device__ inline void sel_merge(const SelPart* __restrict__ ws, int NC, int b, int lane, Best& bt, Best& bs,
-                                 float& m_ts, float& s_ts) {
+#define SEL_MERGE_NB 7
+__device__ inline void sel_merge(const SelPart* __restrict__ ws, int NC, int b, int idx, int stride, Best& bt,
+                                 Best& bs, float& m_ts, float& s_ts) {
   bt = Best{-INFINITY, 0x7fffffff};
   bs = Best{-INFINITY, 0x7fffffff};
   m_ts = -INFINITY;
   s_ts = 0.f;
-  for (int c = lane; c < NC; c += 64) {
-    const SelPart r = ws[b * NC + c];
-    bt = best_of(bt, Best{r.bt_v, r.bt_i});
-    bs = best_of(bs, Best{r.bs_v, r.bs_i});
-    lse_merge(m_ts, s_ts, r.m_ts, r.s_ts);
+  const SelPart* row = ws + (size_t)b * NC;
+  for (int c0 = idx; c0 < NC; c0 += stride * SEL_MERGE_NB) {
+    float4 ra[SEL_MERGE_NB];
+    float2 rb[SEL_MERGE_NB];
+#pragma unroll
+    for (int u = 0; u < SEL_MERGE_NB; ++u) {
+      const SelPart* r = row + min(c0 + stride * u, NC - 1);
+      ra[u] = *(const float4*)r;
+      rb[u] = *(const float2*)&r->m_ts;
+    }
+#pragma unroll
+    for (int u = 0; u < SEL_MERGE_NB; ++u) {
+      if (c0 + stride * u < NC) {
+        bt = best_of(bt, Best{ra[u].x, __float_as_int(ra[u].y)});
+        bs = best_of(bs, Best{ra[u].z, __float_as_int(ra[u].w)});
+        lse_merge(m_ts, s_ts, rb[u].x, rb[u].y);
+      }
+    }
   }
 #pragma unroll
   for (int o = 32; o > 0; o >>= 1) {
@@ -181,14 +138,26 @@
   return tok;
 }
 
+template <int NW>
 __device__ inline void select_final_row(const SelPart* __restrict__ ws, int NC, const TwSelectParams& p,
                                         int* __restrict__ state, int* __restrict__ tokens_out, int ld_tokens,
-                                        int* __restrict__ next_ids, int* __restrict__ pos, int b, int lane,
-                                        int& tok_out, int& npos) {
+                                        int* __restrict__ next_ids, int* __restrict__ pos, int b, int tid,
+                                        int& tok_out, int& npos, SelPart* xw) {
   Best bt, bs;
   float m_ts, s_ts;
-  sel_merge(ws, NC, b, lane, bt, bs, m_ts, s_ts);
-  if (lane != 0) return;
+  sel_merge(ws, NC, b, tid, 64 * NW, bt, bs, m_ts, s_ts);
+  if constexpr (NW > 1) {
+    if ((tid & 63) == 0) xw[tid >> 6] = SelPart{bt.v, bt.i, bs.v, bs.i, m_ts, s_ts, 0.f, 0.f};
+    __syncthreads();
+    if (tid == 0) {
+      for (int w = 1; w < NW; ++w) {
+        bt = best_of(bt, Best{xw[w].bt_v, xw[w].bt_i});
+        bs = best_of(bs, Best{xw[w].bs_v, xw[w].bs_i});
+        lse_merge(m_ts, s_ts, xw[w].m_ts, xw[w].s_ts);
+      }
+    }
+  }
+  if (tid != 0) return;
   int* st = state + b * TW_STATE_STRIDE;
   npos = 0;
   if (pos) npos = pos[b] += 1;
@@ -208,11 +177,12 @@
                                                      int* __restrict__ pos) {
   TW_DEC_PRIO();
   int tok, npos;
-  select_final_row(ws, NC, p, state, tokens_out, ld_tokens, next_ids, pos, blockIdx.x, threadIdx.x, tok, npos);
+  select_final_row<1>(ws, NC, p, state, tokens_out, ld_tokens, next_ids, pos, blockIdx.x, threadIdx.x, tok, npos,
+                      nullptr);
 }
 
 #define SFE_MAXV 4
-template <bool PACKED>
+template <bool PACKED, int NW>
 __global__ TW_DEC_LB(256, 1) void k_select_final_embed(const SelPart* __restrict__ ws, int NC, TwSelectParams p,
                                                             int* __restrict__ state, int* __restrict__ tokens_out,
                                                             int ld_tokens, int* __restrict__ next_ids,
@@ -224,10 +194,11 @@
   TW_DEC_PRIO();
   __shared__ float red[8];
   __shared__ int sh[2];
+  __shared__ SelPart xw[NW];
   const int b = blockIdx.x, tid = threadIdx.x;
-  if (tid < 64) {
+  if (tid < 64 * NW) {
     int tok = 0, npos = 0;
-    select_final_row(ws, NC, p, state, tokens_out, ld_tokens, next_ids, pos, b, tid, tok, npos);
+    select_final_row<NW>(ws, NC, p, state, tokens_out, ld_tokens, next_ids, pos, b, tid, tok, npos, xw);
     if (tid == 0) {
       sh[0] = tok;
       sh[1] = min(npos, max_pos - 1);
@@ -291,12 +262,44 @@
   hipLaunchKernelGGL(k_select_partial, dim3(B, TW_SELECT_CHUNKS), dim3(256), 0, s, logits, ld_logits, suppress_bits,
                      *params, state, ws);
   if (packed)
-    hipLaunchKernelGGL(k_select_final_embed<true>, dim3(B), dim3(256), 0, s, ws, TW_SELECT_CHUNKS, *params, state,
+    hipLaunchKernelGGL((k_select_final_embed<true, 1>), dim3(B), dim3(256), 0, s, ws, TW_SELECT_CHUNKS, *params, state,
                        tokens_out, ld_tokens, next_ids, pos, tok_emb, pos_emb, D, max_pos, x, gamma, beta, eps, out);
   else
-    hipLaunchKernelGGL(k_select_final_embed<false>, dim3(B), dim3(256), 0, s, ws, TW_SELECT_CHUNKS, *params, state,
+    hipLaunchKernelGGL((k_select_final_embed<false, 1>), dim3(B), dim3(256), 0, s, ws, TW_SELECT_CHUNKS, *params, state,
                        tokens_out, ld_tokens, next_ids, pos, tok_emb, pos_emb, D, max_pos, x, gamma, beta, eps, out);
   return tw_check_launch("tw_logits_select_embed");
+}
+
+extern "C" int tw_select_final(const float* workspace, int n_records, int B, const TwSelectParams* params, int* state,
+                               int* tokens_out, int ld_tokens, int* next_ids, int* pos, void* stream) {
+  TW_REQUIRE(workspace && params && state && B > 0 && n_records > 0, "tw_select_final: bad args");
+  TW_REQUIRE(((uintptr_t)workspace & 15) == 0, "tw_select_final: workspace must be 16-byte aligned");
+  hipLaunchKernelGGL(k_select_final, dim3(B), dim3(64), 0, (hipStream_t)stream, (const SelPart*)workspace, n_records,
+                     *params, state, tokens_out, ld_tokens, next_ids, pos);
+  return tw_check_launch("tw_select_final");
+}
+
+extern "C" int tw_select_final_embed(const float* workspace, int n_records, int B, const TwSelectParams* params,
+                                     int* state, int* tokens_out, int ld_tokens, int* next_ids, int* pos,
+                                     const uint16_t* tok_emb, const uint16_t* pos_emb, int D, int max_pos, float* x,
+                                     const float* gamma, const float* beta, float eps, uint16_t* out, int packed,
+                                     void* stream) {
+  TW_REQUIRE(workspace && params && state && next_ids && pos && B > 0 && n_records > 0,
+             "tw_select_final_embed: bad args");
+  TW_REQUIRE(((uintptr_t)workspace & 15) == 0, "tw_select_final_embed: workspace must be 16-byte aligned");
+  TW_REQUIRE(params->mode == 0, "tw_select_final_embed: greedy token selection (mode 0) only");
+  TW_REQUIRE(tok_emb && pos_emb && x && gamma && beta && out && max_pos > 0, "tw_select_final_embed: embed/LN args");
+  TW_REQUIRE(D > 0 && D % 4 == 0 && D <= 1024 * SFE_MAXV && (!packed || (B <= 64 && D % 32 == 0)),
+             "tw_select_final_embed: D=%d B=%d packed=%d", D, B, packed);
+  hipStream_t s = (hipStream_t)stream;
+  const SelPart* ws = (const SelPart*)workspace;
+  auto launch = [&](auto kernel) {
+    hipLaunchKernelGGL(kernel, dim3(B), dim3(256), 0, s, ws, n_records, *params, state, tokens_out, ld_tokens, next_ids,
+                       pos, tok_emb, pos_emb, D, max_pos, x, gamma, beta, eps, out);
+  };
+  if (n_records > 64) packed ? launch(k_select_final_embed<true, 4>) : launch(k_select_final_embed<false, 4>);
+  else packed ? launch(k_select_final_embed<true, 1>) : launch(k_select_final_embed<false, 1>);
+  return tw_check_launch("tw_select_final_embed");
 }
 
 __device__ inline uint64_t tw_mix64(uint64_t z) {
@@ -375,7 +378,7 @@
   block_lse256(m_tx, s_tx, red);
   Best bt, bs;
   float m_ts, s_ts;
-  sel_merge(parts, NC, 0, lane, bt, bs, m_ts, s_ts);
+  sel_merge(parts, NC, 0, lane, 64, bt, bs, m_ts, s_ts);
   const bool fire = sel_rule_fires(p, bt, m_ts, s_ts);
   int sel;
   float lse;
diff --git a/turbo-whisper-workspace_amd/csrc/gemm.hip b/turbo-whisper-workspace_amd/csrc/gemm.hip
--- a/turbo-whisper-workspace_amd/csrc/gemm.hip
+++ b/turbo-whisper-workspace_amd/csrc/gemm.hip
@@ -3,6 +3,7 @@
 
 #include "tw_common.h"
 #include "../../include/tw_whisper.h"
+#include "tw_select.h"
 
 struct EpiArgs {
   void* out;
@@ -1166,13 +1167,105 @@
   return APACK ? *(const bf16x8*)(ap + (size_t)st * 1024) : *(const bf16x8*)(ap + 32 * st);
 }
 
-template <int EPI, int KW, int U, bool APACK, int MT, bool NTW = false>
+struct SelArgs {
+  const uint32_t* suppress_bits;
+  const int* state;
+  SelPart* ws;
+  TwSelectParams p;
+};
+struct SelRec {
+  float bt_v; int bt_i;
+  float bs_v; int bs_i;
+  float m_ts, s_ts;
+};
+
+template <int CTRL>
+__device__ __forceinline__ float row16_dpp(float v) {
+  return __int_as_float(__builtin_amdgcn_update_dpp(0, __float_as_int(v), CTRL, 0xF, 0xF, false));
+}
+__device__ __forceinline__ float row16_max(float v) {
+  v = fmaxf(v, row16_dpp<0xB1>(v));
+  v = fmaxf(v, row16_dpp<0x4E>(v));
+  v = fmaxf(v, row16_dpp<0x141>(v));
+  v = fmaxf(v, row16_dpp<0x140>(v));
+  return v;
+}
+__device__ __forceinline__ float row16_sum(float v) {
+  v += row16_dpp<0xB1>(v);
+  v += row16_dpp<0x4E>(v);
+  v += row16_dpp<0x141>(v);
+  v += row16_dpp<0x140>(v);
+  return v;
+}
+__device__ __forceinline__ Best row16_best(float x, bool elig, int n0, int lane, float& mx) {
+  const float xe = elig ? x : -INFINITY;
+  mx = row16_max(xe);
+  const uint32_t seg = (uint32_t)(__ballot(elig && xe == mx) >> (lane & 48)) & 0xffffu;
+  return seg ? Best{mx, n0 + __ffs(seg) - 1} : Best{-INFINITY, 0x7fffffff};
+}
+
+template <int MT>
+__device__ inline void gemv_sel_prologue(int g, int ngroups, int M, int N, const SelArgs& sa, uint32_t& rmw,
+                                         uint32_t& col) {
+  const int lane = threadIdx.x & 63;
+  const int row = min(lane & (MT * 16 - 1), M - 1), n = g * 16 + (lane & 15);
+  rmw = row_mask_pack(row_mask(sa.state + (size_t)row * TW_STATE_STRIDE, sa.p));
+  col = (g < ngroups && n < N) ? sel_col_bits(sa.p, sa.suppress_bits ? sa.suppress_bits[n >> 5] : 0u, n, true) : 0u;
+  asm volatile("" : "+v"(rmw), "+v"(col));
+}
+template <int MT>
+__device__ inline void gemv_sel_epilogue(const f32x4 (&c)[MT], int g, int ngroups, int M, int N, const SelArgs& sa,
+                                         uint32_t rmw, uint32_t col, SelRec (*rec)[MT * 16]) {
+  const int tid = threadIdx.x, lane = tid & 63, wid = tid >> 6;
+  const int cc = lane & 15, rb = (lane >> 4) * 4;
+  const TwSelectParams& p = sa.p;
+  const int n = g * 16 + cc;
+  const bool colok = g < ngroups && n < N;
+  const bool text = colok && sel_is_text(p, n), ts = colok && !sel_is_text(p, n);
+  const bool any_tx = g < ngroups && sel_is_text(p, g * 16);
+  const bool any_ts = g < ngroups && !sel_is_text(p, min(g * 16 + 15, N - 1));
+#pragma unroll
+  for (int t = 0; t < MT; ++t) {
+#pragma unroll
+    for (int r = 0; r < 4; ++r) {
+      const int m = 16 * t + rb + r;
+      const RowMask rm = row_mask_unpack((uint32_t)__shfl((int)rmw, m, 64));
+      const float x = sel_masked(p, rm, col, n) ? -INFINITY : c[t][r];
+      Best bt{-INFINITY, 0x7fffffff}, bs{-INFINITY, 0x7fffffff};
+      float m_ts = -INFINITY, s_ts = 0.f, mx;
+      if (any_tx) bt = row16_best(x, text, g * 16, lane, mx);
+      if (any_ts) {
+        bs = row16_best(x, ts, g * 16, lane, m_ts);
+        s_ts = row16_sum((ts && x != -INFINITY) ? __expf(x - m_ts) : 0.f);
+      }
+      if (cc == 0) rec[wid][m] = SelRec{bt.v, bt.i, bs.v, bs.i, m_ts, s_ts};
+    }
+  }
+  __syncthreads();
+  if (tid < MT * 16 && tid < M) {
+    const SelRec r0 = rec[0][tid];
+    Best bt{r0.bt_v, r0.bt_i}, bs{r0.bs_v, r0.bs_i};
+    float m_ts = r0.m_ts, s_ts = r0.s_ts;
+#pragma unroll
+    for (int w = 1; w < 4; ++w) {
+      const SelRec r = rec[w][tid];
+      bt = best_of(bt, Best{r.bt_v, r.bt_i});
+      bs = best_of(bs, Best{r.bs_v, r.bs_i});
+      lse_merge(m_ts, s_ts, r.m_ts, r.s_ts);
+    }
+    sa.ws[(size_t)tid * gridDim.x + blockIdx.x] = SelPart{bt.v, bt.i, bs.v, bs.i, m_ts, s_ts, 0.f, 0.f};
+  }
+}
+
+template <int EPI, int KW, int U, bool APACK, int MT, bool NTW = false, bool SEL = false>
 __global__ TW_DEC_LB(KW > 4 ? 512 : 256, NTW ? 4 : 1) void k_gemv_p(const bf16_t* __restrict__ A, int lda,
                                                                const bf16_t* __restrict__ Wp, int M, int N, int K,
-                                                               EpiArgs ea) {
+                                                               EpiArgs ea, SelArgs sa) {
   TW_DEC_PRIO();
+  static_assert(!SEL || (KW == 1 && EPI == TW_EPI_F32 && MT <= 2), "k_gemv_p: SEL is proj_out's one-slice f32 form");
   constexpr int NW = KW > 4 ? KW : 4, GPB = NW / KW;
   __shared__ float red[KW > 1 ? NW : 1][KW > 1 ? MT * 16 : 1][17];
+  __shared__ SelRec rec[SEL ? 4 : 1][SEL ? MT * 16 : 1];
   const int tid = threadIdx.x, lane = tid & 63, wid = tid >> 6;
   const int gl = wid / KW, kw = wid - gl * KW;
   const int g = blockIdx.x * GPB + gl;
@@ -1182,6 +1275,8 @@
   f32x4 c[MT];
 #pragma unroll
   for (int t = 0; t < MT; ++t) c[t] = (f32x4){0.f, 0.f, 0.f, 0.f};
+  uint32_t sel_rmw = 0, sel_col = 0;
+  if constexpr (SEL) gemv_sel_prologue<MT>(g, ngroups, M, N, sa, sel_rmw, sel_col);
   if (g < ngroups) {
     const bf16_t* wp = Wp + (size_t)g * ns * 512 + lane * 8;
     const bf16_t* ap[MT];
@@ -1243,6 +1338,7 @@
         for (int r = 0; r < 4; ++r)
           if (16 * t + rb + r < M) store(16 * t + rb + r, n, c[t][r]);
     }
+    if constexpr (SEL) gemv_sel_epilogue<MT>(c, g, ngroups, M, N, sa, sel_rmw, sel_col, rec);
     return;
   }
 #pragma unroll
@@ -1521,11 +1617,14 @@
   constexpr int U4 = U > 4 ? U / 2 : U;
   dim3 grid(tw_cdiv(tw_cdiv(N, 16), GPB), splits);
   if (M > 32)
-    hipLaunchKernelGGL((k_gemv_p<EPI, KW, U4, APACK, 4, NTW>), grid, dim3(NW * 64), 0, s, A, lda, Wp, M, N, K, ea);
+    hipLaunchKernelGGL((k_gemv_p<EPI, KW, U4, APACK, 4, NTW>), grid, dim3(NW * 64), 0, s, A, lda, Wp, M, N, K, ea,
+                       SelArgs{});
   else if (M > 16)
-    hipLaunchKernelGGL((k_gemv_p<EPI, KW, U, APACK, 2, NTW>), grid, dim3(NW * 64), 0, s, A, lda, Wp, M, N, K, ea);
+    hipLaunchKernelGGL((k_gemv_p<EPI, KW, U, APACK, 2, NTW>), grid, dim3(NW * 64), 0, s, A, lda, Wp, M, N, K, ea,
+                       SelArgs{});
   else
-    hipLaunchKernelGGL((k_gemv_p<EPI, KW, U, APACK, 1, NTW>), grid, dim3(NW * 64), 0, s, A, lda, Wp, M, N, K, ea);
+    hipLaunchKernelGGL((k_gemv_p<EPI, KW, U, APACK, 1, NTW>), grid, dim3(NW * 64), 0, s, A, lda, Wp, M, N, K, ea,
+                       SelArgs{});
 }
 
 template <int EPI, bool APACK>
@@ -1685,6 +1784,33 @@
     default: tw_set_error("tw_gemv_packed: unsupported epilogue %d", epi); return TW_ERR_ARG;
   }
   return tw_check_launch("tw_gemv_packed");
+}
+
+extern "C" int tw_gemv_packed_select_records(int N) { return N > 0 ? (int)tw_cdiv(tw_cdiv(N, 16), 4) : 0; }
+
+extern "C" int tw_gemv_packed_select(const bf16_t* A, const bf16_t* Wp, int M, int N, int K, float* logits, int ldo,
+                                     const uint32_t* suppress_bits, const TwSelectParams* params, const int* state,
+                                     float* workspace, void* stream) {
+  TW_REQUIRE(A && Wp && logits && params && state && workspace, "tw_gemv_packed_select: null pointer");
+  TW_REQUIRE(M > 0 && M <= 32 && N > 0 && K > 0 && K % 32 == 0,
+             "tw_gemv_packed_select: M=%d N=%d K=%d (M <= 32, K %% 32)", M, N, K);
+  TW_REQUIRE(ldo >= N, "tw_gemv_packed_select: ldo=%d < N", ldo);
+  TW_REQUIRE(params->mode == 0 && params->V == N, "tw_gemv_packed_select: mode=%d V=%d N=%d (mode 0, V == N)",
+             params->mode, params->V, N);
+  TW_REQUIRE(params->n_begin_suppress >= 0 && params->n_begin_suppress <= 8, "tw_gemv_packed_select: begin_suppress");
+  TW_REQUIRE(((uintptr_t)workspace & 15) == 0 && ((uintptr_t)state & 15) == 0,
+             "tw_gemv_packed_select: workspace and state must be 16-byte aligned");
+  EpiArgs ea{logits, ldo, nullptr, nullptr, 0, 0, 0, 0, 0};
+  SelArgs sa{suppress_bits, state, (SelPart*)workspace, *params};
+  dim3 grid(tw_gemv_packed_select_records(N), 1);
+  hipStream_t s = (hipStream_t)stream;
+  if (M > 16)
+    hipLaunchKernelGGL((k_gemv_p<TW_EPI_F32, 1, 16, true, 2, true, true>), grid, dim3(256), 0, s, A, K, Wp, M, N, K, ea,
+                       sa);
+  else
+    hipLaunchKernelGGL((k_gemv_p<TW_EPI_F32, 1, 16, true, 1, true, true>), grid, dim3(256), 0, s, A, K, Wp, M, N, K, ea,
+                       sa);
+  return tw_check_launch("tw_gemv_packed_select");
 }
 
 typedef __attribute__((ext_vector_type(8))) int i32x8;
diff --git a/turbo-whisper-workspace_amd/csrc/tw_select.h b/turbo-whisper-workspace_amd/csrc/tw_select.h
--- /dev/null
+++ b/turbo-whisper-workspace_amd/csrc/tw_select.h
@@ -0,0 +1,78 @@
+#pragma once
+#include "tw_common.h"
+#include "../../include/tw_whisper.h"
+
+struct Best {
+  float v;
+  int i;
+};
+__device__ inline Best best_of(Best a, Best b) {
+  if (b.v > a.v || (b.v == a.v && b.i < a.i)) return b;
+  return a;
+}
+__device__ inline void lse_merge(float& m, float& s, float m2, float s2) {
+  if (m2 == -INFINITY) return;
+  if (m == -INFINITY) { m = m2; s = s2; return; }
+  if (m2 > m) { s = s * __expf(m - m2) + s2; m = m2; }
+  else s = s + s2 * __expf(m2 - m);
+}
+
+struct alignas(16) SelPart {
+  float bt_v; int bt_i;
+  float bs_v; int bs_i;
+  float m_ts, s_ts;
+  float pad0, pad1;
+};
+static_assert(sizeof(SelPart) == sizeof(float) * TW_SELECT_REC_WORDS, "record size");
+
+struct RowMask {
+  int init_step, mask_ts_all, mask_text_lt_eos, ts_hi_block;
+};
+__device__ inline RowMask row_mask(const int* st, const TwSelectParams& p) {
+  const int n_gen = st[TW_ST_NGEN], last = st[TW_ST_LAST], penult = st[TW_ST_PENULT], last_ts = st[TW_ST_LASTTS];
+  const int tsb = p.ts_begin;
+  RowMask r{n_gen == 0, 0, 0, tsb};
+  if (p.mode == 0 && p.use_timestamps) {
+    const bool last_was_ts = n_gen >= 1 && last >= tsb;
+    const bool penult_was_ts = n_gen < 2 || penult >= tsb;
+    if (last_was_ts) {
+      if (penult_was_ts) r.mask_ts_all = 1;
+      else r.mask_text_lt_eos = 1;
+    }
+    if (last_ts >= 0) r.ts_hi_block = (last_was_ts && !penult_was_ts) ? last_ts : last_ts + 1;
+  }
+  return r;
+}
+
+__device__ inline uint32_t row_mask_pack(const RowMask& r) {
+  return (uint32_t)r.init_step | ((uint32_t)r.mask_ts_all << 1) | ((uint32_t)r.mask_text_lt_eos << 2) |
+         ((uint32_t)r.ts_hi_block << 3);
+}
+__device__ inline RowMask row_mask_unpack(uint32_t w) {
+  return RowMask{(int)(w & 1u), (int)((w >> 1) & 1u), (int)((w >> 2) & 1u), (int)(w >> 3)};
+}
+
+__device__ inline uint32_t sel_col_bits(const TwSelectParams& p, uint32_t sbw, int v, bool with_begin) {
+  uint32_t c = (sbw >> (v & 31)) & 1u;
+  if (p.use_timestamps) c |= (uint32_t)(v == p.no_timestamps);
+  uint32_t b = 0;
+  if (with_begin)
+    for (int i = 0; i < p.n_begin_suppress; ++i) b |= (uint32_t)(v == p.begin_suppress[i]);
+  return c | (b << 1);
+}
+__device__ inline bool sel_masked(const TwSelectParams& p, const RowMask& rm, uint32_t col, int v) {
+  if (p.mode == 1) return v < p.lo || v >= p.hi;
+  bool masked = (col & 1u) || (rm.init_step && (col & 2u));
+  if (p.use_timestamps) {
+    if (v >= p.ts_begin) {
+      masked |= rm.mask_ts_all || (v < rm.ts_hi_block);
+      if (rm.init_step && p.max_initial_ts >= 0) masked |= (v > p.ts_begin + p.max_initial_ts);
+    } else {
+      masked |= (rm.mask_text_lt_eos && v < p.eos) || rm.init_step;
+    }
+  }
+  return masked;
+}
+__device__ inline bool sel_is_text(const TwSelectParams& p, int v) {
+  return v < p.ts_begin || !p.use_timestamps || p.mode == 1;
+}
diff --git a/turbo-whisper-workspace_amd/twamd/_lib.py b/turbo-whisper-workspace_amd/twamd/_lib.py
--- a/turbo-whisper-workspace_amd/twamd/_lib.py
+++ b/turbo-whisper-workspace_amd/twamd/_lib.py
@@ -21,6 +21,7 @@
 
 TW_SELECT_CHUNKS = 16
 TW_SELECT_WS_PER_ROW = 128
+TW_SELECT_REC_WORDS = 8
 TW_STATE_STRIDE = 8
 TW_ST_NGEN, TW_ST_LAST, TW_ST_PENULT, TW_ST_LASTTS, TW_ST_FINISHED, TW_ST_LANG = 0, 1, 2, 3, 4, 5
 TW_ST_SUMLP, TW_ST_NOSPEECH = 6, 7
@@ -45,7 +46,8 @@
     "tw_gemm_set_persistent_grid", "tw_mp3_probe", "tw_mp3_decode", "tw_aac_parse_asc", "tw_aac_decode_raw",
     "tw_aac_adts_probe", "tw_aac_adts_decode", "tw_dec_fused", "tw_dec_fused_sync_bytes", "tw_dec_fused_supported",
     "tw_dec_fused_set_grid", "tw_dec_fused_set_acquire", "tw_dec_fused_set_probe", "tw_dec_fused_grid",
-    "tw_dec_fused_xpart_bytes", "tw_logits_history",
+    "tw_dec_fused_xpart_bytes", "tw_logits_history", "tw_gemv_packed_select", "tw_gemv_packed_select_records",
+    "tw_select_final", "tw_select_final_embed",
 )
 
 
@@ -213,6 +215,11 @@
     "tw_dec_fused_set_acquire": ([_I], _I),
     "tw_dec_fused_set_probe": ([_P], _I),
     "tw_dec_fused_grid": ([], _I),
+    "tw_gemv_packed_select": ([_P, _P, _I, _I, _I, _P, _I, _P, ctypes.POINTER(TwSelectParams), _P, _P, _P], _I),
+    "tw_gemv_packed_select_records": ([_I], _I),
+    "tw_select_final": ([_P, _I, _I, ctypes.POINTER(TwSelectParams), _P, _P, _I, _P, _P, _P], _I),
+    "tw_select_final_embed": ([_P, _I, _I, ctypes.POINTER(TwSelectParams), _P, _P, _I, _P, _P, _P, _P, _I, _I, _P, _P,
+                               _P, _F, _P, _I, _P], _I),
 }
 
 _lib = None
diff --git a/turbo-whisper-workspace_amd/twamd/engine.py b/turbo-whisper-workspace_amd/twamd/engine.py
--- a/turbo-whisper-workspace_amd/twamd/engine.py
+++ b/turbo-whisper-workspace_amd/twamd/engine.py
@@ -223,7 +223,9 @@
         self.attd = torch.empty(B, D, dtype=act, device=dev)
         self.logits = torch.empty(B, V, dtype=f32, device=dev)
         self.parts = torch.empty(DEC_SPLITS, B, D, dtype=f32, device=dev)
-        self.sel_ws = torch.empty(B, _lib.TW_SELECT_WS_PER_ROW, dtype=f32, device=dev)
+        self._sel_records = int(_lib.load().tw_gemv_packed_select_records(V))
+        self.sel_ws = torch.empty(B, max(_lib.TW_SELECT_WS_PER_ROW, self._sel_records * _lib.TW_SELECT_REC_WORDS),
+                                  dtype=f32, device=dev)
         self.state = torch.zeros(B, _lib.TW_STATE_STRIDE, dtype=i32, device=dev)
         self.tokens = torch.zeros(B, T, dtype=i32, device=dev)
         self.ids = torch.zeros(B, dtype=i32, device=dev)
@@ -241,7 +243,7 @@
         self._hist_prefix = torch.zeros(self.max_rows, T, dtype=i32, device=dev)
         self._hist_len = torch.zeros(self.max_rows, dtype=i32, device=dev)
         self._hist: Optional[tuple] = None
-        self._dec_ctx = (1, 0, False)
+        self._dec_ctx = (1, 0, False, False)
         self._fused_dims = (not self.F32 and bool(_lib.load().tw_dec_fused_supported(D, H, d.ffn, 1)))
         self._fused_tab: Optional[torch.Tensor] = None
         self._fused_err = torch.zeros(4, dtype=torch.int32, device=dev)
@@ -610,12 +612,12 @@
 
     @on_engine_streams
     def decoder_step(self, R: int, with_logits: bool = True, v: Optional[DecView] = None, r_enc: Optional[int] = None,
-                     pre_embedded: bool = False) -> None:
+                     pre_embedded: bool = False, sel_params=None) -> None:
         if v is None and R > VIEW_ROWS:
             r_enc = R if r_enc is None else r_enc
             for r0 in range(0, R, VIEW_ROWS):
                 n = min(VIEW_ROWS, R - r0)
-                self.decoder_step(n, with_logits, self._view(r0, n), r_enc, pre_embedded)
+                self.decoder_step(n, with_logits, self._view(r0, n), r_enc, pre_embedded, sel_params)
             return
         v = v or self._view(0, R)
         r_enc = R if r_enc is None else r_enc
@@ -629,7 +631,7 @@
         if self._fused_ok(R):
             self._fused_layers(R, r_enc, v)
             if with_logits:
-                self._gemv(v.hp, True, self.emb_p, R, d.vocab, D, _lib.TW_EPI_F32, v.logits, v)
+                self._proj_out(R, v, sel_params)
             return
         xkv_stride = 2 * r_enc * H * S_ENC * 64
         nparts, pbias = 0, None
@@ -668,7 +670,18 @@
             nparts, pbias = K4, L.b2
         if with_logits:
             self._resid_ln_p(R, nparts, pbias, w.dec_ln_g, w.dec_ln_b, v)
-            self._gemv(v.hp, True, self.emb_p, R, d.vocab, D, _lib.TW_EPI_F32, v.logits, v)
+            self._proj_out(R, v, sel_params)
+
+    def _proj_out(self, R: int, v: DecView, sel_params=None) -> None:
+        d = self.d
+        if sel_params is None:
+            self._gemv(v.hp, True, self.emb_p, R, d.vocab, d.d_model, _lib.TW_EPI_F32, v.logits, v)
+            return
+        rec = self._begin_timer(("gemv_packed", _lib.TW_EPI_F32), 2.0 * R * d.vocab * d.d_model, v.stream)
+        _lib.call("tw_gemv_packed_select", v.hp.data_ptr(), self.emb_p.data_ptr(), R, d.vocab, d.d_model,
+                  v.logits.data_ptr(), d.vocab, self.suppress_bits.data_ptr(), ctypes.byref(sel_params),
+                  v.state.data_ptr(), v.sel_ws.data_ptr(), v.stream.cuda_stream)
+        self._end_timer(rec, v.stream)
 
     def _cross_attend(self, li: int, R: int, r_enc: int, rmap, ckv, v: DecView) -> None:
         H, s = self.d.heads, v.stream.cuda_stream
@@ -738,12 +751,23 @@
         return p
 
     def _select(self, R: int, params: _lib.TwSelectParams, tokens: bool = True, v: Optional[DecView] = None,
-                embed_next: bool = False) -> None:
+                embed_next: bool = False, folded: bool = False) -> None:
         if v is None and R > VIEW_ROWS:
             for r0 in range(0, R, VIEW_ROWS):
                 self._select(min(VIEW_ROWS, R - r0), params, tokens, self._view(r0, min(VIEW_ROWS, R - r0)), embed_next)
             return
         v = v or self._view(0, R)
+        if folded:
+            head = (v.sel_ws.data_ptr(), self._sel_records, R, ctypes.byref(params), v.state.data_ptr(),
+                    v.tokens.data_ptr() if tokens else None, v.tokens.shape[1], v.ids.data_ptr(), v.pos.data_ptr())
+            if embed_next:
+                L0 = self.w.dec[0]
+                _lib.call("tw_select_final_embed", *head, self.w.emb.data_ptr(), self.w.pos_dec.data_ptr(),
+                          self.d.d_model, self.d.max_target_positions, v.xd.data_ptr(), L0.ln1_g.data_ptr(),
+                          L0.ln1_b.data_ptr(), LN_EPS, v.hp.data_ptr(), 1, v.stream.cuda_stream)
+            else:
+                _lib.call("tw_select_final", *head, v.stream.cuda_stream)
+            return
         if params.mode == 0:
             self._history(v.r0, R, v.stream)
         if embed_next:
@@ -809,9 +833,17 @@
 
     def _gen_step(self, R: int, params, v: Optional[DecView] = None, r_enc: Optional[int] = None,
                   fused: bool = False) -> None:
+        if self._fold_ok(R if v is None else v.n, params):
+            self.decoder_step(R, v=v, r_enc=r_enc, pre_embedded=fused, sel_params=params)
+            self._select(R, params, v=v, embed_next=fused, folded=True)
+            return
         self.decoder_step(R, v=v, r_enc=r_enc, pre_embedded=fused)
         self._select(R, params, v=v, embed_next=fused)
 
+    def _fold_ok(self, R: int, params) -> bool:
+        return bool(self._dec_ctx[3] and not self.F32 and params.mode == 0 and self._hist is None and R <= 32
+                    and self._wide_kw == 1)
+
     dec_alone_wide_kw = 1
     dec_beside_wide_kw = 1
 
@@ -820,6 +852,9 @@
 
     dec_fused_alone = False
     dec_fused_max_rows = 4
+
+    dec_alone_fold_select = True
+    dec_beside_fold_select = False
 
     @property
     def _wide_kw(self) -> int:
@@ -827,8 +862,9 @@
 
     def _dec_context(self) -> tuple:
         beside = self._pump is not None
-        ctx = ((self.dec_beside_wide_kw, self.dec_beside_gemv, False) if beside
-               else (self.dec_alone_wide_kw, self.dec_alone_gemv, bool(self.dec_fused_alone and self._fused_dims)))
+        ctx = ((self.dec_beside_wide_kw, self.dec_beside_gemv, False, bool(self.dec_beside_fold_select)) if beside
+               else (self.dec_alone_wide_kw, self.dec_alone_gemv, bool(self.dec_fused_alone and self._fused_dims),
+                     bool(self.dec_alone_fold_select)))
         if ctx[:2] != self._dec_ctx[:2]:
             _lib.call("tw_gemv_set_wide_slices", ctx[0])
             _lib.call("tw_gemv_set_variant", ctx[1])
```

New measurement: 8184 audio-s/wall-s. No clear change (-0.0%).
